# pierre-haessig/stodynprog

Measured on AMD Instinct MI355X. Metric: vi_sweeps_per_sec, higher is better.
Workload: dtype f64

## Files before the change

__graft_entry__.py:

```python
import os
import sys

ROOT = os.path.dirname(os.path.abspath(__file__))
if ROOT not in sys.path:
    sys.path.insert(0, ROOT)


def _prebuild_models(verbose=False):
    import numpy as np
    from stodynprog_amd import models, DPSolver, _native as nat
    sources = []
    specs = [
        ('inventory', {}, np.float64),
        ('nas_demo', {}, np.float64),
        ('storage_ar1', {}, np.float64),
        ('storage_ar1', dict(n_E=200, n_P=200, steps=(8. / 49, 0.1)), np.float64),
        ('searev', {}, np.float64),
        ('searev', dict(n_E=128, n_S=128, n_A=128, step=2.2 / 31), np.float64),
        ('synthetic3d', dict(N=20), np.float64),
        ('synthetic3d', dict(N=20), np.float32),
        ('synthetic3d', dict(N=48), np.float64),
        ('synthetic3d', dict(N=256), np.float64),
        ('synthetic3d', dict(N=256), np.float32),
        ('synthetic3d', dict(N=512), np.float32),
        ('synthetic3d', dict(N=256, stock_noise=0.07), np.float64),
        ('synthetic3d', dict(N=256, stock_noise=0.07, nested=True), np.float64),
        ('inventory_markov', {}, np.float64),
        ('inventory_fine', {}, np.float64),
        ('inventory_fine', dict(n_x=65536, n_u=4097, n_w=16), np.float64),
        ('two_reservoirs', dict(n_a=128, n_b=128, n_y=64, n_w=16, steps=(1. / 15, 1. / 15)), np.float64),
        ('synthetic3d_coupled', dict(N=256), np.float64),
        ('synthetic3d_coupled', dict(N=24), np.float64),
    ]
    for name, kw, dt in specs:
        sysd, ref = getattr(models, name)(**kw)
        for kernel in ('auto', 'staged', 'generic', 'long way'):
            solver = DPSolver(sysd, dtype=dt)
            solver.state_grid, solver.perturb_grid = ref.state_grid, ref.perturb_grid
            solver.perturb_proba, solver.control_steps = ref.perturb_proba, ref.control_steps
            if kernel == 'long way':
                solver.certified_filter = False
            else:
                solver.kernel = kernel
            sources.append(solver._kernel_plan()['source'])
    import importlib.util
    dont_write = sys.dont_write_bytecode
    sys.dont_write_bytecode = True
    try:
        spec = importlib.util.spec_from_file_location('column_forms', os.path.join(ROOT, 'tests', 'column_forms.py'))
        forms = importlib.util.module_from_spec(spec)
        spec.loader.exec_module(forms)
    finally:
        sys.dont_write_bytecode = dont_write
    saved = DPSolver.debug_defines
    try:
        for case, geometry in forms.PAIRS:
            DPSolver.debug_defines = dict(case.debug) or None
            for kw in (dict(), dict(certified_filter=False), dict(kernel='generic')):
                sources.append(case.solver(geometry, **kw)._kernel_plan()['source'])
    finally:
        DPSolver.debug_defines = saved
    sys.dont_write_bytecode = True
    sys.path.insert(0, os.path.join(ROOT, 'tests'))
    try:
        import policies
        import test_gpu_simulate_forms as simulate_forms
        for fam in policies.FAMILIES:
            for kernel in (None, 'generic'):
                sources.append(fam.solver(kernel)._kernel_plan()['source'])
        for make, _ in simulate_forms.UNITS.values():
            sources.append(make()._kernel_plan()['source'])
        sources.append(simulate_forms._deterministic(np.float32)._kernel_plan()['source'])
        sources.append(simulate_forms._deterministic(np.float64)._kernel_plan()['source'])
        for dt in (np.float64, np.float32):
            _, fh = models.finite_horizon()
            fh = policies.as_dtype(fh, dt)
            sources += [fh._kernel_plan(t0, fh._trace_now(t0))['source'] for t0 in (3, 11)]
        _, wec = models.searev(n_E=9, n_S=11, n_A=10)
        sources.append(policies.as_dtype(wec, np.float32)._kernel_plan()['source'])
        import test_horizon_plan
        sources += list(test_horizon_plan.units())
        import fp32_cases
        for case in fp32_cases.CASES + [fp32_cases.CONFIG5]:
            for run in case.runs:
                sources.append(fp32_cases.plan_of(case.solver(run))['source'])
        _, fh = models.finite_horizon()
        fh = policies.as_dtype(fh, np.float32)
        sources += [fh._kernel_plan(t, fh._trace_now(t))['source'] for T in (3, 11) for t in range(T)]
        import device_ops
        for dtkey in device_ops.DTYPES:
            for unit in device_ops.units(dtkey):
                sources.append(device_ops.unit_source(device_ops.unit_solver(unit, dtkey)))
        for seed in device_ops.WIDE_SEEDS:
            sources.append(device_ops.wide_model(seed)[0]._kernel_plan()['source'])
    finally:
        sys.path.remove(os.path.join(ROOT, 'tests'))
        sys.dont_write_bytecode = dont_write
    for kw in (dict(), dict(T=14 * 48, N_E=100)):
        _, pv = models.pv_storage(**kw)
        sources.append(pv._kernel_plan(0, pv._trace_now(0))['source'])
    from concurrent.futures import ThreadPoolExecutor
    unique = list(dict.fromkeys(sources))
    with ThreadPoolExecutor(max_workers=min(6, os.cpu_count() or 1)) as pool:
        return list(pool.map(lambda src: nat.compile_model(src, verbose=verbose), unique))


def build():
    from stodynprog_amd import _native as nat
    nat.build_library(verbose=True)
    from stodynprog_amd import codegen
    if os.path.isdir(nat.KCACHE):
        keep = set()
        for fn in os.listdir(nat.KCACHE):
            if fn.endswith('.hip'):
                try:
                    with open(os.path.join(nat.KCACHE, fn)) as f:
                        if codegen.source_key(f.read()) == fn[:-4]:
                            keep.add(fn[:-4])
                except OSError:
                    pass
        for fn in os.listdir(nat.KCACHE):
            stem = fn.split('.')[0]
            if '.tmp.' in fn or (fn.endswith(('.hsaco', '.hip')) and stem not in keep):
                os.unlink(os.path.join(nat.KCACHE, fn))
    import stodynprog_amd
    lib = nat.lib()
    assert lib is not None and nat.EXPORTS
    mods = _prebuild_models()
    print('built {} and {} model code objects'.format(nat.LIB_PATH, len(set(mods))))
    from oracle import c_oracle
    print('built', c_oracle.build())


def smoke():
    import numpy as np
    from stodynprog_amd import models, _native as nat
    nat.require_gpu()
    nat.check(nat.lib().sdp_set_device(0))
    print('device:', nat.device_info(0))
    _, solver = models.synthetic3d(N=20)
    V0 = models.synthetic3d_V0(solver.state_grid)
    J, pol = solver.value_iteration(V0, report_time=False)
    idx = solver.last_policy_index
    from oracle import c_oracle
    Jo, io, mo = c_oracle.vi_synth3d(solver.state_grid, V0, models.SYNTH_PAR, -1., 1., 64,
                                     solver.perturb_grid[0], solver.perturb_proba[0],
                                     n_nodes=V0.size)
    Jo = Jo.reshape(V0.shape)
    io = io.reshape(V0.shape)
    err = np.abs(J - Jo).max() / np.abs(Jo).max()
    print('smoke: max rel err J = {:.3e}; index mismatches = {}'.format(
        err, int((idx != io).sum())))
    assert err < 1e-12, err
    assert np.array_equal(idx, io)
    _, inv = models.inventory()
    J1, u1 = inv.value_iteration(np.zeros(10), report_time=False)
    assert np.allclose(J1, [9, 6, 3, 0, 0.5, 1, 1.5, 2, 2.5, 3], rtol=0, atol=1e-12), J1
    mcr = inv.monte_carlo(u1, np.zeros(1), 50, seed=1, n_burn=5, n_traj=100)
    _, w = inv.monte_carlo_draws(1, 100, 50)
    _, _, g = inv.simulate(u1, np.zeros((100, 1)), w)
    acc = np.zeros(100)
    for k in range(5, 50):
        acc = acc + g[k]
    assert np.array_equal(mcr.cost_sum, acc), (mcr.cost_sum, acc)
    print('smoke: Monte Carlo mean cost {:.4f} +- {:.4f}, same bits as the replay'.format(mcr.mean, mcr.stderr))
    print('smoke OK')


if __name__ == '__main__':
    build()
    if len(sys.argv) > 1 and sys.argv[1] == 'smoke':
        smoke()
```

stodynprog_amd/codegen.py:

```python
import hashlib
import re
import math
import os

import numpy as np

from .trace import TracedModel, DEP_X

CSRC = os.path.join(os.path.dirname(os.path.abspath(__file__)), 'csrc')


DEBUG_INT_MACROS = ('SDP_COL_MIN_WAVES', 'SDP_COL_BATCH', 'SDP_COL_UNROLL_U', 'SDP_COL_UNROLL_W',
                    'SDP_COL_A_GROUP', 'SDP_COL_FILTER_UNROLL', 'SDP_COL_FILTER_TOP2', 'SDP_COL_FILTER_RUNROLL',
                    'SDP_COL_A_WIDE_LOADS', 'SDP_COLU_WIDE_LOADS', 'SDP_COLU_A_GROUP',
                    'SDP_COL_TAIL_HOLD', 'SDP_SHORT_GROUP', 'SDP_BNB_CHUNK')
DEBUG_NAMES = frozenset(DEBUG_INT_MACROS + (
    'SDP_STAMP', 'SDP_NO_POW2', 'SDP_EXTRA_DEFINES', 'SDP_COL_FILTER_SCALE', 'SDP_LEAD_FILTER_SCALE',
    'SDP_LEAD_UNROLL', 'SDP_COL_A_LW', 'SDP_COL_FILTER', 'SDP_COL_SHIFT', 'SDP_COL_UTAB', 'SDP_LEAD_FILTER',
    'SDP_COL_THREADS', 'SDP_COL_WCHUNK', 'SDP_STG_CU', 'SDP_COL_WPAIR', 'SDP_COL_WRES', 'SDP_COL_LEAN2', 'SDP_COL_BNB',
    'SDP_LINE_FILTER', 'SDP_LINE_FILTER_SCALE', 'SDP_LINE_TOP2'))


def check_debug(debug):
    if not debug:
        return None
    unknown = sorted(set(debug) - DEBUG_NAMES)
    if unknown:
        raise ValueError('unknown debug define(s): {}'.format(', '.join(unknown)))
    return {k: str(v) for k, v in debug.items() if v is not None and str(v) != ''} or None


def _dbg(debug, name, default=None):
    if not debug:
        return default
    v = debug.get(name)
    return default if v is None or str(v) == '' else str(v)

_BIN_INFIX = {'add': '+', 'sub': '-', 'mul': '*', 'div': '/',
              'lt': '<', 'le': '<=', 'gt': '>', 'ge': '>=', 'eq': '==', 'ne': '!=',
              'and': '&&', 'or': '||', 'xor': '!='}
_FUNC1 = {'abs': 'fabs', 'sqrt': 'sqrt', 'floor': 'floor', 'ceil': 'ceil', 'trunc': 'trunc',
          'rint': 'rint', 'exp': 'exp', 'exp2': 'exp2', 'expm1': 'sdp_npexpm1', 'log': 'log',
          'log2': 'log2', 'log10': 'log10', 'log1p': 'sdp_nplog1p', 'sin': 'sin', 'cos': 'cos',
          'tan': 'tan', 'asin': 'asin', 'acos': 'acos', 'atan': 'atan', 'sinh': 'sinh',
          'cosh': 'cosh', 'tanh': 'tanh', 'cbrt': 'cbrt'}
_FUNC2 = {'pow': 'pow', 'atan2': 'atan2', 'hypot': 'hypot', 'fmod': 'fmod',
          'min': 'sdp_npmin', 'max': 'sdp_npmax', 'fmin': 'sdp_npfmin', 'fmax': 'sdp_npfmax',
          'pymod': 'sdp_nppymod', 'floordiv': 'sdp_npfloordiv'}


def real_literal(value):
    if math.isnan(value):
        return '(sdp_real)NAN'
    if math.isinf(value):
        return '(sdp_real)INFINITY' if value > 0 else '(-(sdp_real)INFINITY)'
    return '(sdp_real)({})'.format(float(value).hex())


def _emit_node(n, name, param_index=None):
    a = [name(x) for x in n.args]
    op = n.op
    if op == 'const':
        if param_index is not None and n.id in param_index:
            return 'sdp_model_prm[{}]'.format(param_index[n.id])
        return real_literal(n.value)
    if op == 'bconst':
        return 'true' if n.value else 'false'
    if op == 'var':
        v = n.value
        if v == 't':
            return 't'
        return '{}[{}]'.format(v[0], v[1:]) if v[0] in 'xu' else 'w'
    if op in _BIN_INFIX:
        return '({} {} {})'.format(a[0], _BIN_INFIX[op], a[1])
    if op in _FUNC1:
        return '{}({})'.format(_FUNC1[op], a[0])
    if op in _FUNC2:
        return '{}({}, {})'.format(_FUNC2[op], a[0], a[1])
    if op == 'neg':
        return '(-{})'.format(a[0])
    if op == 'square':
        return '({0} * {0})'.format(a[0])
    if op == 'recip':
        return '((sdp_real)1 / {})'.format(a[0])
    if op == 'sign':
        return 'sdp_npsign({})'.format(a[0])
    if op == 'not':
        return '(!{})'.format(a[0])
    if op == 'isnan':
        return '({0} != {0})'.format(a[0])
    if op == 'isinf':
        return '(fabs({}) == (sdp_real)INFINITY)'.format(a[0])
    if op == 'isfinite':
        return '(fabs({}) < (sdp_real)INFINITY)'.format(a[0])
    if op in ('select', 'bselect'):
        return '({} ? {} : {})'.format(a[0], a[1], a[2])
    if op == 'b2r':
        return '({} ? (sdp_real)1 : (sdp_real)0)'.format(a[0])
    if op == 'interp1':
        return 'sdp_interp1_{}({})'.format(n.value, a[0])
    raise NotImplementedError(op)


INTERP_SOURCE = '''SDP_DEV sdp_real sdp_np_interp(sdp_real x, const sdp_real *xp, const sdp_real *fp, int n,
                                sdp_real left, sdp_real right)
{
    if (n == 1) return x < xp[0] ? left : (x > xp[0] ? right : fp[0]);
    if (x != x) return x;
    if (x > xp[n - 1]) return right;
    if (x < xp[0]) return left;
    int imin = 0, imax = n;
    while (imin < imax) {
        const int imid = imin + ((imax - imin) >> 1);
        if (x >= xp[imid]) imin = imid + 1; else imax = imid;
    }
    const int j = imin - 1;
    if (j == n - 1) return fp[j];
    if (xp[j] == x) return fp[j];
    const sdp_real slope = (fp[j + 1] - fp[j]) / (xp[j + 1] - xp[j]);
    sdp_real r = slope * (x - xp[j]) + fp[j];
    if (r != r) {
        r = slope * (x - xp[j + 1]) + fp[j + 1];
        if (r != r && fp[j] == fp[j + 1]) r = fp[j];
    }
    return r;
}
'''


def interp_tables_source(model):
    used = sorted({n.value for n in model.live_nodes() if n.op == 'interp1'})
    if not used:
        return ''
    out = [INTERP_SOURCE]
    for tid in used:
        xp, fp, left, right = model.graph.tables[tid][:4]
        out.append('__constant__ sdp_real sdp_tabx_{}[{}] = {{{}}};'.format(
            tid, xp.size, ', '.join(real_literal(v) for v in xp)))
        out.append('__constant__ sdp_real sdp_tabf_{}[{}] = {{{}}};'.format(
            tid, fp.size, ', '.join(real_literal(v) for v in fp)))
        out.append('SDP_DEV sdp_real sdp_interp1_{0}(sdp_real x)\n{{\n    return sdp_np_interp('
                   'x, sdp_tabx_{0}, sdp_tabf_{0}, {1}, {2}, {3});\n}}'.format(
                       tid, xp.size, real_literal(left), real_literal(right)))
    return '\n'.join(out) + '\n'


def _emit_body(model, nodes, lines, names=None):
    names = dict(names or {})

    def name(n):
        return names[n.id]

    for n in nodes:
        expr = _emit_node(n, name, getattr(model, 'param_index', None))
        if n.op in ('const', 'bconst', 'var'):
            names[n.id] = expr
            continue
        var = 'v{}'.format(n.id)
        ctype = 'bool' if n.kind == 'b' else 'sdp_real'
        lines.append('    const {} {} = {};'.format(ctype, var, expr))
        names[n.id] = var
    return names


def model_function_source(model):
    assert isinstance(model, TracedModel)
    if model.n_perturb > 1:
        raise NotImplementedError('only 0 or 1 perturbation variable is supported '
                                  '(as reference stodynprog.py:679-683)')
    lines = ['SDP_DEV void sdp_model_cell(const sdp_real *x, const sdp_real *u, sdp_real w,',
             '                            sdp_real t, sdp_real *xn, sdp_real &g)',
             '{',
             '    (void)x; (void)u; (void)w; (void)t;']
# ... 67 lines not shown
    lines = ['SDP_DEV void sdp_model_leads(const sdp_real *x, const sdp_real *u, sdp_real t, sdp_real *xl)',
             '{', '    (void)x; (void)u; (void)t;']
    names = _emit_body(model, model.slice_nodes(leads), lines)
    for k, n in enumerate(leads):
        lines.append('    xl[{}] = {};'.format(k, names[n.id]))
    lines.append('}')
    out.append('\n'.join(lines))
    if m < d:
        lines = ['SDP_DEV void sdp_model_trails(const sdp_real *x, sdp_real w, sdp_real t, sdp_real *xt)',
                 '{', '    (void)x; (void)w; (void)t;']
        names = _emit_body(model, model.slice_nodes(trails), lines)
        for k, n in enumerate(trails):
            lines.append('    xt[{}] = {};'.format(k, names[n.id]))
        lines.append('}')
        out.append('\n'.join(lines))
    lines = ['SDP_DEV sdp_real sdp_model_cost(const sdp_real *x, const sdp_real *u, sdp_real w,',
             '                                sdp_real t)',
             '{', '    (void)x; (void)u; (void)w; (void)t;']
    names = _emit_body(model, model.slice_nodes([model.cost]), lines)
    lines += ['    return {};'.format(names[model.cost.id]), '}']
    out.append('\n'.join(lines))
    return '\n\n'.join(out)


def lead_filter_applies(model, dtype, min_axes=2, debug=None):
    if _dbg(debug, 'SDP_LEAD_FILTER', '1') == '0':
        return 0
    if model.n_perturb != 1 or np.dtype(dtype).itemsize != 8:
        return 0
    m = model.controlled_axes()
    return int(m) if m is not None and m >= min_axes else 0


def lead_order(model, dtype, debug=None):
    if _dbg(debug, 'SDP_LEAD_FILTER', '1') == '0' or model.n_perturb != 1 or np.dtype(dtype).itemsize != 8:
        return None
    co = model.controlled_order()
    if co is None or co[1] == tuple(range(model.n_state)) or co[0] >= model.n_state:
        return None
    return co


UTAB_MAX_VALUES = 4
UTAB_MAX_BYTES = 4096


def control_table_plan(model, dtype, per_node, max_controls, debug=None):
    if _dbg(debug, 'SDP_COL_UTAB', '1') == '0' or per_node or model.cost_depends_on_w:
        return None
    lead = None
    if model.lead_depends_on_w:
        split = model.lead_split()
        if split is None:
            return None
        lead = split[0]
    fr = model.control_uniform_frontier(lead)
    if fr is None or len(fr) > UTAB_MAX_VALUES:
        return None
    if len(fr) * int(max_controls) * np.dtype(dtype).itemsize > UTAB_MAX_BYTES:
        return None
    return fr


def control_table_source(model, frontier):
    slot = {n.id: k for k, n in enumerate(frontier)}
    out = []
    lines = ['SDP_DEV void sdp_model_utab(const sdp_real *x, const sdp_real *u, sdp_real t, sdp_real *tab)',
             '{', '    (void)x; (void)u; (void)t;']
    names = _emit_body(model, model.slice_nodes(frontier), lines)
    for n in frontier:
        lines.append('    tab[{}] = {};'.format(slot[n.id], names[n.id]))
    lines.append('}')
    out.append('\n'.join(lines))
    pre = {n.id: 'tab[{}]'.format(slot[n.id]) for n in frontier}
    split = model.lead_split() if model.lead_depends_on_w else None
    for fname, node in (('sdp_model_lead_tab', split[0] if split else model.x_next[0]),
                        ('sdp_model_cost_tab', model.cost)):
        lines = ['SDP_DEV sdp_real {}(const sdp_real *x, const sdp_real *tab, sdp_real t)'.format(fname),
                 '{', '    (void)x; (void)tab; (void)t;']
        names = _emit_body(model, model.slice_nodes_until([node], set(slot)), lines, pre)
        lines += ['    return {};'.format(names[node.id]), '}']
        out.append('\n'.join(lines))
    chain = model.lead_split_chain() if split else None
    if chain is not None:
        leaves = [n for n, _ in chain[0]]
        lines = ['SDP_DEV sdp_real sdp_model_lead_aabs_tab(const sdp_real *x, const sdp_real *tab, sdp_real t)',
                 '{', '    (void)x; (void)tab; (void)t;']
        names = _emit_body(model, model.slice_nodes_until(leaves, set(slot)), lines, pre)
        lines += ['    return {};'.format(' + '.join('fabs({})'.format(names[n.id]) for n in leaves)), '}']
        out.append('\n'.join(lines))
    return '\n\n'.join(out)


def short_pass_source(model, frontier, macro='SDP_COL_LEAN2'):
    sp = model.additive_control_split(frontier)
    if sp is None:
        return None
    (x_node, a_slot, a_form), (k_node, h_slot, h_form) = sp['lead'], sp['cost']
    out = ['#define {} 1          // x0\' = X(x) +- a(u), cost = K(x) +- h(u): the short first pass'.format(macro),
           '#define SDP_LEAN2_A_SLOT {}'.format(int(a_slot)),
           '#define SDP_LEAN2_H_SLOT {}'.format(-1 if h_slot is None else int(h_slot)),
           '#define SDP_LEAN2_LEAD(X, A) {}'.format({'add': '((X) + (A))', 'sub': '((X) - (A))', 'rsub': '((A) - (X))'}[a_form]),
           '#define SDP_LEAN2_FORM {}            // 0: X + a, 1: X - a, 2: a - X'.format({'add': 0, 'sub': 1, 'rsub': 2}[a_form]),
           '#define SDP_LEAN2_A_FIXED {}         // a depends on the control alone: the same lattice of positions in every column'.format(
               0 if (frontier[int(a_slot)].deps & DEP_X) else 1),
           '#define SDP_LEAN2_HNEG {}           // the part of the cost that depends on the control enters negated (K - h)'.format(
               1 if (h_slot is not None and h_form == 'sub') else 0)]
    for fname, node in (('sdp_model_lead_x', x_node), ('sdp_model_cost_x', k_node)):
        lines = ['SDP_DEV sdp_real {}(const sdp_real *x, sdp_real t)'.format(fname), '{', '    (void)x; (void)t;']
        if node is None:
            lines += ['    return (sdp_real)0;', '}']
        else:
            names = _emit_body(model, model.slice_nodes([node]), lines)
            lines += ['    return {};'.format(names[node.id]), '}']
        out.append('\n'.join(lines))
    return '\n'.join(out)


def lanes_for(max_controls):
    lanes = 1
    while lanes < max_controls and lanes < 64:
        lanes *= 2
    return lanes


def _prologue_lines(model, real, lanes, debug, peer_stores=False):
    lines = ['// generated by stodynprog_amd.codegen -- do not edit',
             '#define SDP_REAL {}'.format(real),
             '#define SDP_D {}'.format(model.n_state),
             '#define SDP_NU {}'.format(model.n_control),
             '#define SDP_HAS_W {}'.format(1 if model.n_perturb else 0),
             '#define SDP_LANES {}'.format(int(lanes)),
             '#define SDP_PEER_STORES {}     // the backup kernels also store J into other ranks (direct exchange)'.format(
                 1 if peer_stores else 0)]
    if _dbg(debug, 'SDP_STAMP') in ('1', '2', '3'):
        lines.append('#define SDP_STAMP {}     // diagnostic build: in-kernel clock stamps (tools/clock_probe.py, '
                     'tools/phase_probe.py)'.format(int(_dbg(debug, 'SDP_STAMP'))))
    if _dbg(debug, 'SDP_NO_POW2') == '1':
        lines.append('#define SDP_NO_POW2 1  // A/B: true division also for power-of-two spans')
    for kv in (_dbg(debug, 'SDP_EXTRA_DEFINES') or '').split(','):
        if '=' in kv:
            lines.append('#define {} {}   // SDP_EXTRA_DEFINES (diagnostic builds)'.format(*kv.split('=', 1)))
    lines += ['#include "sdp_device.h"', 'typedef SDP_REAL sdp_real;', '']
    if getattr(model, 'param_index', None):
        lines += ['#define SDP_NPARAMS {}'.format(len(model.param_index)),
                  'extern "C" { __constant__ sdp_real sdp_model_prm[SDP_NPARAMS]; }     // a definition', '']
    tables = interp_tables_source(model)
    if tables:
        lines.append(tables)
    lines += [model_function_source(model), '']
    return lines


def _column_lines(model, dtype, column, col_cfg, window, per_control, filtered, utab, debug, wres=0):
    rs = np.dtype(dtype).itemsize
    wpair = use_wpair(model, dtype, debug) and window is None
    shifted = bool(filtered and column_shift_applies(model, dtype, debug=debug))
    lines = ['#define SDP_COST_HAS_W {}'.format(1 if model.cost_depends_on_w else 0),
             '#define SDP_LEAD_HAS_W {}'.format(1 if model.lead_depends_on_w else 0),
             '#define SDP_TRAIL_HAS_U {}'.format(1 if model.trail_depends_on_u else 0),
             '#define SDP_COL_N0 {}'.format(int(column[0])),
             '#define SDP_COL_W {}'.format(max(int(column[1]), 1)),
             '#define SDP_COL_THREADS {}'.format(col_cfg[0]),
             '#define SDP_COL_WPAIR {}'.format(1 if wpair else 0)]
    if wres:
        lines.append('#define SDP_COL_WRES {}         // resident-chunk form: perturbation points the table holds at a time'.format(int(wres)))
        if rs == 8 and shifted and not _dbg(debug, 'SDP_COL_UNROLL_W'):
            lines.append('#define SDP_COL_UNROLL_W 1')
    if filtered and int(col_cfg[0]) <= 256 and not _dbg(debug, 'SDP_COL_MIN_WAVES'):
        if wres:
            lines.append('#define SDP_COL_MIN_WAVES {}    // as many waves per SIMD as the LDS image admits workgroups per CU, at most 4'.format(
                max(1, min(4, (COLUMN_LDS_MAX // int(col_cfg[1])) * int(col_cfg[0]) // 256))))
        else:
            lines.append('#define SDP_COL_MIN_WAVES 1    // small workgroups of the filtered kernel: no register cap')
    if filtered:
        lines.append('#define SDP_COL_FILTER 1')
        if shifted:
            lines += ['#define SDP_COL_SHIFT 1        // x0\' = a(x, u) +- b_1(x_1.., w) +- ..: first pass on the shifted lattice',
                      '#define SDP_COL_SHIFT_TERMS {}'.format(len(model.lead_split()[1])),
                      '#define SDP_COL_SHIFT_CHAIN {}        // additions of a chain of sums that was regrouped (0: the final-sum form)'.format(
                          model.lead_split_chain()[1] if model.lead_split_chain() is not None else 0),
                      '#define SDP_COL_SHIFT_ROWS {}'.format(int(col_cfg[2]))]
        if _dbg(debug, 'SDP_COL_FILTER_SCALE'):
            lines.append('#define SDP_COL_FILTER_SCALE {}'.format(float(_dbg(debug, 'SDP_COL_FILTER_SCALE'))))
    if per_control is None:
        wide = column_wide_loads(column[0], dtype, window, debug)
        order = column_build_order(int(col_cfg[0]), column[1], int(window[2]) if window is not None else column[0],
                                   (16 // rs) if wide else 1)
        if order[0] == 2:
            lw = int(_dbg(debug, 'SDP_COL_A_LW') or order[1])
            lines += ['#define SDP_COL_A_ORDER 2',
                      '#define SDP_COL_A_LW {}'.format(lw)]
            if rs == 4 and int(column[0]) >= 512 and not wres and window is None and not _dbg(debug, 'SDP_COL_A_GROUP'):
                lines.append('#define SDP_COL_A_GROUP 8      // table entries per thread whose vertex loads are issued together')
            if wide and not _dbg(debug, 'SDP_COL_A_WIDE_LOADS'):
                lines.append('#define SDP_COL_A_WIDE_LOADS 1')

                if wres and rs == 8 and not wpair and window is None and _dbg(debug, 'SDP_COL_TAIL_HOLD') is None:
                    tail, groups = int(column[1]) - int(wres), int(col_cfg[0]) // lw
                    if (tail > 0 and tail % groups == 0 and int(column[0]) % (2 * lw) == 0
                            and (tail // groups) * (int(column[0]) // (2 * lw)) * 4 <= 32):
                        lines.append('#define SDP_COL_TAIL_HOLD 1    // the tail of the table is built once and held in registers')
    if window is not None:
        lines.append('#define SDP_COL_ROWS {}'.format(int(window[2])))
    if per_control is not None:
        lines.append('#define SDP_COL_WCHUNK {}'.format(int(per_control[2])))
        if int(column[0]) % (16 // rs) == 0 and not _dbg(debug, 'SDP_COLU_WIDE_LOADS'):
            lines.append('#define SDP_COLU_WIDE_LOADS 1')
    for k in DEBUG_INT_MACROS:
        if _dbg(debug, k):
            lines.append('#define {} {}'.format(k, int(_dbg(debug, k))))
    lines += [separable_functions_source(model), '']
    if utab is not None and filtered:
        lines += ['#define SDP_COL_UTAB {}'.format(len(utab[0])),
                  '#define SDP_COL_UTAB_N {}'.format(int(utab[1])),
                  control_table_source(model, utab[0]), '']
        short = None
        if not model.cost_depends_on_w and window is None and per_control is None \
                and _dbg(debug, 'SDP_COL_LEAN2') != '0' and (not shifted or rs == 8):
            if rs == 8 and wres:
                short = short_pass_source(model, utab[0], 'SDP_COL_LEAN2')
                if short and _dbg(debug, 'SDP_COL_BNB') != '0':
                    short += ('\n#define SDP_COL_BNB 1          // the short first pass as a certified branch and bound over '
                              'blocks of controls (sdp_lean2_bnb)')

            elif rs == 4 and not wres and _dbg(debug, 'SDP_COL_FILTER_TOP2') in (None, '1'):
                short = short_pass_source(model, utab[0], 'SDP_COL_WIDE2')
                if short and _dbg(debug, 'SDP_COL_BNB') != '0':
                    short += ('\n#define SDP_COL_BNB 1          // the short wide first pass as a certified branch and bound over '
                              'blocks of controls (sdp_short_bnb)')
                    if int(column[0]) >= 512 and not _dbg(debug, 'SDP_BNB_CHUNK'):
                        short += '\n#define SDP_BNB_CHUNK 4        // blocks whose bounds are evaluated together (see SDP_COL_A_GROUP above)'
        if short:
            lines += [short, '']
    lines += ['#include "sdp_column_kernel.h"    // also brings in sdp_sweep_kernel.h', '']
    return lines


def line_filter_applies(model, dtype, W, debug=None):
    if _dbg(debug, 'SDP_LINE_FILTER', '1') == '0':
        return False
    return bool(model.n_state == 1 and model.n_perturb == 1 and 1 <= int(W) <= 1024 and np.dtype(dtype).itemsize == 8
                and not model.time_dep and model.lead_depends_on_w and not model.cost_depends_on_w
                and model.lead_split() is not None)


def line_functions_source(model):
    a_node, terms = model.lead_split()
    out = []
    lines = ['SDP_DEV sdp_real sdp_model_lead_a(const sdp_real *x, const sdp_real *u, sdp_real t)',
             '{', '    (void)x; (void)u; (void)t;']
    names = _emit_body(model, model.slice_nodes([a_node]), lines)
    lines += ['    return {};'.format(names[a_node.id]), '}']
    out.append('\n'.join(lines))
    chain = model.lead_split_chain()
    if chain is not None:
        leaves = [n for n, _ in chain[0]]
        lines = ['SDP_DEV sdp_real sdp_model_lead_aabs(const sdp_real *x, const sdp_real *u, sdp_real t)',
                 '{', '    (void)x; (void)u; (void)t;']
        names = _emit_body(model, model.slice_nodes(leaves), lines)
        lines += ['    return {};'.format(' + '.join('fabs({})'.format(names[n.id]) for n in leaves)), '}']
        out.append('\n'.join(lines))
    lines = ['SDP_DEV void sdp_model_lead_b(const sdp_real *x, sdp_real w, sdp_real t, sdp_real &b, sdp_real &babs)',
             '{', '    (void)x; (void)w; (void)t;']
    names = _emit_body(model, model.slice_nodes([b for b, _ in terms]), lines)
    b0, s0 = terms[0]
    lines.append('    b = {}{};'.format('-' if s0 < 0 else '', names[b0.id]))
    lines.append('    babs = fabs({});'.format(names[b0.id]))
    for bn, sg in terms[1:]:
        lines.append('    b = b {} {};'.format('+' if sg > 0 else '-', names[bn.id]))
        lines.append('    babs = babs + fabs({});'.format(names[bn.id]))
    lines.append('}')
    out.append('\n'.join(lines))
    lines = ['SDP_DEV sdp_real sdp_model_cost(const sdp_real *x, const sdp_real *u, sdp_real w,',
             '                                sdp_real t)',
             '{', '    (void)x; (void)u; (void)w; (void)t;']
    names = _emit_body(model, model.slice_nodes([model.cost]), lines)
    lines += ['    return {};'.format(names[model.cost.id]), '}']
    out.append('\n'.join(lines))
    return '\n\n'.join(out)


def translation_unit(model, dtype, lanes, column=None, staged=None, window=None,
                     per_control=None, filtered=False, utab=None, lead_axes=0, col_cfg=None, debug=None, wres=0,
                     lead_perm=None, line=0, peer_stores=False):
    debug = check_debug(debug)
    real = {'float64': 'double', 'float32': 'float'}[np.dtype(dtype).name]
    head = _prologue_lines(model, real, lanes, debug, peer_stores)
    if column is not None:
        assert model.column_shareable
        if per_control is not None:
            col_cfg = per_control
        elif window is not None:
            col_cfg = window
        elif col_cfg is None:
            col_cfg = column_config(column[0], column[1], model.n_state, dtype,
                                    use_wpair(model, dtype, debug), filtered,
                                    max_controls=column[2] if len(column) > 2 else None,
                                    n_columns=column[3] if len(column) > 3 else None,
                                    shift=filtered and column_shift_applies(model, dtype, debug=debug),
                                    utab_values=(utab_reals(len(utab[0]), utab[1]) if utab is not None and filtered else 0),
                                    debug=debug)
        if col_cfg is None:
            raise ValueError('the column kernel does not fit this grid (its table exceeds the LDS of a CU)')
        head += _column_lines(model, dtype, column, col_cfg, window, per_control, filtered, utab, debug,
                              wres if (window is None and per_control is None) else 0)
    elif staged is not None:
        tile = tuple(staged['tile']) + (1,) * (4 - len(staged['tile']))
        head += ['#define SDP_STG_THREADS {}'.format(int(staged['threads']))] + [
            '#define SDP_STG_T{} {}'.format(k, int(tile[k])) for k in range(4)] + [
            '#define SDP_STG_CU {}'.format(int(staged['cu'])),
            '#define SDP_STG_CW {}'.format(int(staged['cw'])),
            '#define SDP_STG_CAP {}'.format(int(staged['cap'])),
            '#include "sdp_staged_kernel.h"    // also brings in sdp_sweep_kernel.h',
            '']
    elif line:
        chain = model.lead_split_chain()
        head += ['#define SDP_LINE 1',
                 '#define SDP_LINE_W {}'.format(int(line)),
                 '#define SDP_LINE_CHAIN {}        // additions of a chain of sums that was regrouped (0: the final-sum form)'.format(
                     chain[1] if chain is not None else 0)]
        if _dbg(debug, 'SDP_LINE_FILTER_SCALE'):
            head.append('#define SDP_LINE_FILTER_SCALE {}'.format(float(_dbg(debug, 'SDP_LINE_FILTER_SCALE'))))
        if _dbg(debug, 'SDP_LINE_TOP2') is not None:
            head.append('#define SDP_LINE_TOP2 {}'.format(int(_dbg(debug, 'SDP_LINE_TOP2'))))
        head += [line_functions_source(model), '',
                 '#include "sdp_sweep_kernel.h"    // brings in sdp_line_kernel.h', '']
    elif lead_axes:
        head += ['#define SDP_LEAD_AXES {}'.format(int(lead_axes)),
                 '#define SDP_LEAD_COST_HAS_W {}'.format(1 if model.cost_depends_on_w else 0)]
        if lead_perm is not None and tuple(lead_perm) != tuple(range(model.n_state)):
            full = tuple(lead_perm) + tuple(range(model.n_state, 4))
            head.append('#define SDP_LEAD_PERM {{{}}}     // state variable of logical axis j: the stocks are not listed first'.format(
                ', '.join(str(int(k)) for k in full)))
        if _dbg(debug, 'SDP_LEAD_FILTER_SCALE'):
            head.append('#define SDP_LEAD_FILTER_SCALE {}'.format(float(_dbg(debug, 'SDP_LEAD_FILTER_SCALE'))))
        if _dbg(debug, 'SDP_LEAD_UNROLL'):
            head.append('#define SDP_LEAD_UNROLL {}'.format(int(_dbg(debug, 'SDP_LEAD_UNROLL'))))
        head += [lead_functions_source(model, int(lead_axes), lead_perm), '',
                 '#include "sdp_sweep_kernel.h"    // brings in sdp_lead_kernel.h', '']
    else:
        head += ['#include "sdp_sweep_kernel.h"', '']
    return '\n'.join(head)


STAGED_TILES = {1: (512,), 2: (16, 32), 3: (8, 8, 8), 4: (4, 4, 4, 8)}
STAGED_LDS_BYTES = 76 * 1024


def staged_row_stride(length, tile_last, d, rs):
    if d == 1 or tile_last >= 32 or rs != 8:
        return length | 1
    return (length + tile_last - 1) // (2 * tile_last) * (2 * tile_last) + tile_last


def staged_config(model, state_grid, perturb_grid, box, dtype, t_value=0.0, n_samples=24, debug=None):
    from .trace import evaluate
    d = model.n_state
    rs = np.dtype(dtype).itemsize
    shape = tuple(len(g) for g in state_grid)
    tile = STAGED_TILES[d]
    cap = STAGED_LDS_BYTES // rs
    W = len(perturb_grid[0]) if perturb_grid and model.n_perturb else 0
    wg = np.asarray(perturb_grid[0], dtype=float) if W else np.zeros(1)
    Wn = max(W, 1)
    nu = model.n_control
    lo, hi, n = box['lo'], box['hi'], box['n']
    S = int(np.prod(shape))
    rng = np.random.default_rng(2024)
    smin = np.array([g[0] for g in state_grid], dtype=float)
    span = np.array([g[-1] - g[0] for g in state_grid], dtype=float)
    nm1 = np.array([len(g) - 1 for g in state_grid], dtype=float)
    tiles_per = [-(-shape[k] // tile[k]) for k in range(d)]

    def control_values(flat_nodes, ci):
        col = flat_nodes if box['per_node'] else np.zeros_like(flat_nodes)
        nn = n[:, col].astype(np.int64)
        tot = np.prod(nn, axis=0)
        flat = np.minimum(ci, tot - 1)
        out = []
        for c in range(nu - 1, -1, -1):
            k = flat % nn[c]
            flat = flat // nn[c]
            l, h = lo[c, col], hi[c, col]
            step = np.where(nn[c] > 1, (h - l) / np.maximum(nn[c] - 1, 1), 0.0)
            out.append(np.where(k == nn[c] - 1, h, k * step + l))
        return out[::-1], tot

    def volume(cu, cw):
        vols = []
        for _ in range(n_samples):
            torg = [int(rng.integers(0, tiles_per[k])) * tile[k] for k in range(d)]
            idx = np.array(np.meshgrid(*[[torg[k], min(torg[k] + tile[k], shape[k]) - 1]
                                         for k in range(d)], indexing='ij')).reshape(d, -1)
            flat = np.ravel_multi_index(tuple(idx), shape)
            x = [np.asarray(state_grid[k], dtype=float)[idx[k]] for k in range(d)]
            _, tot = control_values(flat, 0)
            c0 = int(rng.integers(0, max(int(tot.max()) - cu, 0) + 1))
            w0 = int(rng.integers(0, max(Wn - cw, 0) + 1))
            qlo = np.full(d, np.inf)
            qhi = np.full(d, -np.inf)
            for ci in (c0, c0 + cu - 1):
                u, _ = control_values(flat, ci)
                for wi in (w0, min(w0 + cw, Wn) - 1):
                    with np.errstate(all='ignore'):
                        xn, _ = evaluate(model, x, u, [wg[wi]] if model.n_perturb else [], t_value)
                    for k in range(d):
                        p = (np.asarray(xn[k], dtype=float) - smin[k]) / span[k] * nm1[k]
                        q = np.clip(np.floor(np.nan_to_num(p, nan=0.0, posinf=1e9, neginf=-1e9)),
                                    0, shape[k] - 2)
                        qlo[k] = min(qlo[k], q.min())
                        qhi[k] = max(qhi[k], q.max())
            ext = [min(qhi[k] + 1, shape[k] - 2) + 2 - max(qlo[k] - 1, 0) for k in range(d)]
            ext[-1] = staged_row_stride(int(ext[-1]), tile[-1], d, rs)
            vols.append(float(np.prod(ext)))
        return float(np.percentile(vols, 80))

    cws = sorted({max(1, Wn >> s) for s in range(0, 8)}, reverse=True)
    best = None
    cus = (4, 2, 1)
    if _dbg(debug, 'SDP_STG_CU'):
        cus = (int(_dbg(debug, 'SDP_STG_CU')),)
    for cu in cus:
        for cw in cws:
            if best is not None and cu * cw <= best[0] * best[1]:
                continue
            if volume(cu, cw) <= cap:
                best = (cu, cw)
                break
    if best is None:
        best = (1, 1)
    return dict(threads=int(np.prod(tile)), tile=tile, cu=best[0], cw=best[1], cap=int(cap))


COLUMN_LDS_MAX = 160 * 1024


def use_wpair(model, dtype, debug=None):
    if _dbg(debug, 'SDP_COL_WPAIR'):
        return bool(int(_dbg(debug, 'SDP_COL_WPAIR')))
    return (np.dtype(dtype).itemsize == 4 and model.n_perturb > 0
            and not model.lead_depends_on_w and not model.trail_depends_on_u)


def column_shift_applies(model, dtype, table=None, debug=None):
    if _dbg(debug, 'SDP_COL_SHIFT', '1') == '0':
        return False
    ok = bool(model.n_perturb > 0 and model.lead_depends_on_w and model.lead_split() is not None
              and dtype is not None and np.dtype(dtype).itemsize == 8)
    if ok and table is not None:
        ok = column_config(table[0], table[1], table[2], dtype, False, True, shift=True,
                           utab_values=UTAB_MAX_BYTES // np.dtype(dtype).itemsize + 256,
                           debug=debug) is not None
    return ok


def column_filter_applies(model, window=None, per_control=None, dtype=None, table=None, debug=None):
    if _dbg(debug, 'SDP_COL_FILTER', '1') == '0':
        return False
    return bool(model.n_perturb > 0 and (not model.lead_depends_on_w or column_shift_applies(model, dtype, table, debug))
                and not model.trail_depends_on_u and window is None
                and per_control is None)


def column_config(n0, w, n_state, dtype, wpair=False, filtered=False, max_controls=None, n_columns=None,
                  shift=False, utab_values=0, debug=None, wres=0):
    rs = np.dtype(dtype).itemsize
    w = max(int(w), 1)
    tw = w + (w & 1) if wpair else w
    sizes = (512, 1024)
    if filtered and n0 <= 512:
        first = max(64, (int(n0) + 63) // 64 * 64)
        if max_controls:
            lanes = 1
            while lanes * 128 < int(max_controls) and lanes < 64:
                lanes *= 2
            cap = 1024 if (n_columns is not None and int(n_columns) < 256) else 512
            first = max(first, min(first * lanes, cap))
        sizes = (first,) + tuple(t for t in sizes if t > first)
    if _dbg(debug, 'SDP_COL_THREADS'):
        sizes = (int(_dbg(debug, 'SDP_COL_THREADS')),)
    if shift:
        for per_cu in ((3, 2, 1) if wres else (2, 1)):
            for threads in sizes:
                if per_cu >= 2 and threads > 512:
                    continue
                base = _column_lds(int(wres) or tw, w, n0, n_state, rs, threads, shift=True, shift_rows=0, utab_values=utab_values)
                rows = min(2 * int(n0) + 16, (COLUMN_LDS_MAX // per_cu - base - 1024) // (2 * rs))
                if rows >= int(n0) + max(8, int(n0) // 8):
                    return (threads, _column_lds(int(wres) or tw, w, n0, n_state, rs, threads, shift=True, shift_rows=rows,
                                                 utab_values=utab_values), int(rows))
        return None
    for threads in sizes:
        lds = _column_lds(int(wres) or tw, w, n0, n_state, rs, threads, reduced=filtered, utab_values=utab_values,
                          partial_minima=not filtered)
        if lds * (2 if threads <= 512 else 1) <= COLUMN_LDS_MAX:
            return threads, lds
    return None


def column_resident_points(model, n0, w, n_state, dtype, filtered, shift, wpair, threads, utab_values=0, debug=None):
    rs = np.dtype(dtype).itemsize
    w = int(w)
    ok = (filtered and rs == 8 and not wpair and not model.cost_depends_on_w and w >= 4
          and int(threads) >= int(n0))
    forced = _dbg(debug, 'SDP_COL_WRES')
    if forced is not None:
        k = int(forced)
        return k if (ok and 0 < k < w and 2 * k >= w) else 0
    if not ok:
        return 0
    half = (w + 1) // 2
    if shift:
        both = [column_config(n0, w, n_state, dtype, wpair, True, shift=True, utab_values=utab_values, debug=debug, wres=k)
                for k in (0, half)]
        if None in both:
            return 0
        whole, part = both[0][1], both[1][1]
    else:
        whole = _column_lds(w, w, n0, n_state, rs, threads, reduced=True, utab_values=utab_values)
        part = _column_lds(half, w, n0, n_state, rs, threads, reduced=True, utab_values=utab_values)
    if COLUMN_LDS_MAX // whole < 3 <= COLUMN_LDS_MAX // part:
        return half if RESIDENT_CHUNKS_DEFAULT else 0
    return 0


RESIDENT_CHUNKS_DEFAULT = True


def column_wide_loads(n0, dtype, window, debug=None):
    if _dbg(debug, 'SDP_COL_A_WIDE_LOADS', '1') == '0':
        return False
    rpl = 16 // np.dtype(dtype).itemsize
    if rpl != 2 and _dbg(debug, 'SDP_COL_A_WIDE_LOADS') != '1':
        return False
    return int(n0) % rpl == 0 and window is None


def column_build_order(threads, w, rows, rows_per_lane=1):
    w = max(int(w), 1)
    best = (0, 0, 0.0)
    for lw in ((32, 64, 16, 8) if rows_per_lane > 1 else (64, 32, 16, 8)):
        if lw * rows_per_lane > rows or threads % lw:
            continue
        groups = threads // lw
        util = w / float(-(-w // groups) * groups)
        if util > best[2] + 1e-9:
            best = (2, lw, util)
    return (best[0], best[1]) if best[2] >= 0.85 else (0, 0)


def bnb_words(n_controls):
    n = max(int(n_controls), 1)
    block = 8
    while (n + block - 1) // block > 64:
        block *= 2
    return 4 * ((n + block - 1) // block + 1)


def utab_reals(n_values, n_controls):
    return int(n_values) * int(n_controls) + bnb_words(n_controls) if n_values else 0


def _column_lds(tw, w, rows, n_state, rs, threads, reduced=False, shift=False, shift_rows=0, utab_values=0,
                partial_minima=False):
    dt = n_state - 1
    part = threads if partial_minima else 1
    members = [(rs, tw * rows, 16),
               (rs, w * dt, rs), (rs, w * dt, rs),
               (rs, 2, rs),
               (rs, part, rs), (4, part, 4),
               (4, w * dt, 4),
               (4, 4, 4), (4, 1, 4), (8, 2, 8),
               (rs, 2 * (int(utab_values) + 4 if utab_values else 2), 16)]
    if reduced or shift:
        per_row = 4 if rs == 4 else (2 if shift else 1)
        members.append((rs, per_row * int(shift_rows if shift else rows), 16))
    if shift:
        members += [(4, 2 * w, 4), (rs, 2 * w, rs), (rs, 2 * w, rs), (4, 8, 4)]
    off = 0
    for size, count, align in members:
        off = (off + align - 1) // align * align + size * int(count)
    return (off + 15) // 16 * 16


def column_percontrol_config(n0, w, n_state, dtype, debug=None):
    rs = np.dtype(dtype).itemsize
    w = max(int(w), 1)
    threads = min(512, max(64, (int(n0) + 63) // 64 * 64))
    wchunk = max(1, min(w, (32 * 1024) // (int(n0) * rs)))
    if _dbg(debug, 'SDP_COL_WCHUNK'):
        wchunk = max(1, min(w, int(_dbg(debug, 'SDP_COL_WCHUNK'))))
    lds = _column_lds(wchunk, w, n0, n_state, rs, threads)
    if lds > COLUMN_LDS_MAX:
        return None
    return threads, lds, wchunk


def column_window_config(n0, w, n_state, dtype, reach_rows):
    rs = np.dtype(dtype).itemsize
    w = max(int(w), 1)
    for threads, wgs in ((512, 2),):
        budget = COLUMN_LDS_MAX // wgs
        fixed = _column_lds(w, w, 0, n_state, rs, threads, partial_minima=True)
        rows = (budget - fixed) // (w * rs)
        rows = min(rows // 32 * 32, n0)
        seg = (rows - int(reach_rows) - 4) // 64 * 64
        if rows >= 128 and seg >= 64:
            return (threads, _column_lds(w, w, rows, n_state, rs, threads, partial_minima=True), int(rows),
                    int(min(seg, n0)))
    return None


def column_lds_bytes(n0, w, n_state, dtype):
    cfg = column_config(n0, w, n_state, dtype)
    return cfg[1] if cfg else COLUMN_LDS_MAX + 1


HIPCC_FLAGS = ['--genco', '--offload-arch=gfx950', '-O3', '-ffp-contract=off',
               '-fno-fast-math', '-std=c++17', '-I', CSRC]


_HEADERS = ('sdp_kernel_args.h', 'sdp_device.h', 'sdp_sweep_kernel.h', 'sdp_mc_kernel.h', 'sdp_column_kernel.h', 'sdp_colfilter_kernel.h', 'sdp_colres_kernel.h',
            'sdp_colfull_kernel.h', 'sdp_colu_kernel.h',
            'sdp_lead_kernel.h', 'sdp_staged_kernel.h')
_digest_cache = {}


def _headers_digest():
    stamp = tuple(os.stat(os.path.join(CSRC, fn)).st_mtime_ns for fn in _HEADERS)
    h = _digest_cache.get(stamp)
    if h is None:
        h = hashlib.sha256()
        for fn in _HEADERS:
            with open(os.path.join(CSRC, fn), 'rb') as f:
                h.update(f.read())
        _digest_cache.clear()
        _digest_cache[stamp] = h
    return h.copy()


_compiler_id = None
HIPCC_PATH = '/opt/rocm/bin/hipcc'


def compiler_identity():
    global _compiler_id
    if _compiler_id is None:
        import subprocess
        try:
            out = subprocess.run([HIPCC_PATH, '--version'], stdout=subprocess.PIPE, stderr=subprocess.DEVNULL,
                                 timeout=60).stdout.decode(errors='replace')
            keep = [ln.strip() for ln in out.splitlines() if ln.startswith(('HIP version', 'AMD clang version', 'clang version'))]
            _compiler_id = '\n'.join(keep) or 'hipcc without a version'
        except (OSError, subprocess.SubprocessError):
            _compiler_id = 'no hipcc'
    return _compiler_id


BUILD_RULES = 'spill fence 1'


def source_key(source):
    h = _headers_digest()
    if '#define SDP_LINE ' in source:
        with open(os.path.join(CSRC, 'sdp_line_kernel.h'), 'rb') as f:
            h.update(f.read())
    h.update(source.encode())
    h.update(' '.join(HIPCC_FLAGS[:-1]).encode())
    h.update(compiler_identity().encode())
    h.update(BUILD_RULES.encode())
    return h.hexdigest()[:24]


_ASM_FUNC = re.compile(r'^([A-Za-z_]\w*):\s*; @')
_ASM_BLOCK = re.compile(r'^(\.LBB\d+_\d+):|^; %bb\.(\d+):')
_ASM_SPILL = re.compile(r'^\s+(?:scratch_(?:store|load)\w*|buffer_(?:store|load)\w*|v_accvgpr_(?:write|read)\w*)\b.*;.*\b(?:Spill|Reload)\b')
_ASM_END_CF = re.compile(r'^\s+s_or_b64\s+exec,\s*exec,')
_ASM_EXEC_WRITE = re.compile(r'^\s+s_\w+\s+exec(?:_lo|_hi)?\b|^\s+s_\w*saveexec\w*\b|^\s+v_cmpx')


def spill_hazards(asm):
    out, func, block, pending, at_top = [], None, None, [], False
    for n, line in enumerate(asm.splitlines(), 1):
        m = _ASM_FUNC.match(line)
        if m:
            func, block, pending, at_top = m.group(1), 'entry', [], False
            continue
        m = _ASM_BLOCK.match(line)
        if m:
            block, pending, at_top = m.group(1) or '%bb.' + m.group(2), [], True
            continue
        if not at_top:
            continue
        if _ASM_SPILL.match(line):
            pending.append(line.strip())
        elif _ASM_END_CF.match(line):
            if pending:
                out.append((func, block, n, pending))
            at_top = False
        elif _ASM_EXEC_WRITE.match(line):
            at_top = False
    return out


def _msgpack_ints_after(blob, key):
    out, i = [], blob.find(key)
    while i >= 0:
        j = i + len(key)
        b = blob[j] if j < len(blob) else 0
        out.append(b if b <= 0x7f else int.from_bytes(blob[j + 1:j + 1 + {0xcc: 1, 0xcd: 2, 0xce: 4}.get(b, 0)], 'big') if b in (0xcc, 0xcd, 0xce) else -1)
        i = blob.find(key, j)
    return out


def code_object_may_spill(blob):
    scratch = _msgpack_ints_after(blob, b'.private_segment_fixed_size')
    agprs = _msgpack_ints_after(blob, b'.agpr_count')
    if not scratch or len(agprs) != len(scratch):
        return True
    return any(v != 0 for v in scratch) or any(v != 0 for v in agprs)
```

stodynprog_amd/csrc/sdp_colfilter_kernel.h:

```cpp
#pragma once

SDP_DEV double sdp_vmin(double a, double b) { double r; asm("v_min_f64 %0, %1, %2" : "=v"(r) : "v"(a), "v"(b)); return r; }
SDP_DEV double sdp_vmax(double a, double b) { double r; asm("v_max_f64 %0, %1, %2" : "=v"(r) : "v"(a), "v"(b)); return r; }
SDP_DEV float sdp_vmin(float a, float b) { float r; asm("v_min_f32 %0, %1, %2" : "=v"(r) : "v"(a), "v"(b)); return r; }
SDP_DEV float sdp_vmax(float a, float b) { float r; asm("v_max_f32 %0, %1, %2" : "=v"(r) : "v"(a), "v"(b)); return r; }
SDP_DEV double sdp_vmax_abs(double a, double b) { double r; asm("v_max_f64 %0, %1, |%2|" : "=v"(r) : "v"(a), "v"(b)); return r; }
SDP_DEV float sdp_vmax_abs(float a, float b) { float r; asm("v_max_f32 %0, %1, |%2|" : "=v"(r) : "v"(a), "v"(b)); return r; }

struct SdpColFilter {
    sdp_real psum;
    sdp_real pcap;
    sdp_real cu;
    sdp_real floor;
    sdp_real ratio;
    const sdp_cst_real *p, *wg;
    double psum64;
    sdp_real gc;
    sdp_real glimit;
    bool ok;
    sdp_real k_rows, x_cap;
};
constexpr bool SDP_COL_LEAN_ON = sizeof(sdp_real) == 8;
constexpr bool SDP_COL_WIDE_ON = sizeof(sdp_real) == 4;
static_assert(!SDP_COL_SHIFT || SDP_COL_LEAN_ON, "the shifted lattice is a form of the lean first pass (8-byte reals)");
// ... 205 lines not shown
#pragma unroll
                for (int i = 0; i < CH; ++i) {
                    const sdp_real t0 = tv[i][0], t1 = tv[i][1], t2 = tv[i][2];
                    acc = fma(tp[i], fma(tf[i], t1 - t0, t0), acc);
                    bnd = fma(tc[i], fabs((t2 - t1) - (t1 - t0)), bnd);
                    big = sdp_vmax_abs(big, t1);
                }
            } else {
#pragma unroll
                for (int i = 0; i < CH; ++i) {
                    const int wq = w_lo + wave + (i0 + i) * waves;
                    const int trow = (wq < w_lo + w_cnt ? wq : w_lo + wave) - w_lo;
                    const int j = k + (tq[i] - trow * N0);
                    const int q = max(min(j, N0 - 2), 0);
                    const sdp_real lam = (sdp_real)(j - q) + tf[i];
                    const sdp_real *row = m.T + trow * N0 + q;
                    const sdp_real t0 = row[0], t1 = row[1], t2 = row[q + 2 < N0 ? 2 : 1];
                    acc = fma(tp[i], fma(lam, t1 - t0, t0), acc);
                    const sdp_real d2 = (t2 - t1) - (t1 - t0);
                    const bool kink = (unsigned)j <= (unsigned)(N0 - 3);
                    bnd = fma(tc[i], kink ? fabs(d2) : (sdp_real)0, bnd);
                    big = sdp_vmax_abs(sdp_vmax_abs(big, t0), t1);
                }
            }
            if (ki < c.rows) {
                __hip_atomic_fetch_add(&m.ad[2 * ki], acc, __ATOMIC_RELAXED, __HIP_MEMORY_SCOPE_WORKGROUP);
                __hip_atomic_fetch_add(&m.ad[2 * ki + 1], bnd, __ATOMIC_RELAXED, __HIP_MEMORY_SCOPE_WORKGROUP);
            }
            dmax = sdp_vmax(dmax, acc == acc ? f.pcap * big + f.floor : (sdp_real)INFINITY);
        }
    }
    dmax = sdp_wave_max(dmax);
    if (lane == 0)
        atomicMax(&m.dcol[parity], (unsigned long long)__double_as_longlong((double)dmax));
}
#endif

SDP_DEV int sdp_col_axis_mode(const SdpLeadAxis &l)
{
    if (!l.pow2) return 0;
    return (l.smin == (sdp_real)0 && l.span == (sdp_real)1) ? 2 : 1;
}

#if SDP_COST_HAS_W
template <bool WIDE, typename ACC>
SDP_DEV void sdp_col_cost_expect(const SdpColFilter &f, const sdp_real *x, const sdp_real *u, sdp_real t,
                                 ACC &G, sdp_real &Gabs)
{
    G = (ACC)0;
    Gabs = (sdp_real)0;
    sdp_real graw = (sdp_real)0;
#pragma unroll 4
    for (int w = 0; w < SDP_COL_W; ++w) {
        const sdp_real pw = f.p[w];
        const sdp_real gw = sdp_model_cost(x, u, f.wg[w], t);
        G = fma((ACC)pw, (ACC)gw, G);
        Gabs = fma((WIDE ? sdp_col_wide_nw(w) : (sdp_real)1) * fabs(pw), fabs(gw), Gabs);
        graw = sdp_vmax_abs(graw, gw);
    }
    Gabs = sdp_vmax(Gabs, graw);
}
#endif

template <int AXIS>
SDP_DEV void sdp_col_lean_core(const sdp_real *A, const SdpColFilter &f, const SdpLeadAxis &l,
                               sdp_real xn0, sdp_real g, sdp_real &F, sdp_real &lmax, sdp_real &bmax)
{
    const sdp_real sn = AXIS == 2 ? xn0 : (AXIS == 1 ? (xn0 - l.smin) * l.rspan : (xn0 - l.smin) / l.span);
    const sdp_real p = sn * l.nm1;
#if SDP_COL_SHIFT
    const sdp_real pk = p - l.koff;
    int q0 = (int)pk;
    asm("v_med3_i32 %0, %0, 0, %1" : "+v"(q0) : "s"(l.ordm2));
    const sdp_real lam0 = pk - (sdp_real)q0;
    lmax = sdp_vmax_abs(lmax, lam0);
    const sdp_real a0 = A[2 * q0], a1 = A[2 * q0 + 2];
    bmax = sdp_vmax(bmax, A[2 * q0 + 1]);
#else
    (void)bmax;
    int q0 = (int)p;
    asm("v_med3_i32 %0, %0, 0, %1" : "+v"(q0) : "s"(l.ordm2));
    const sdp_real lam0 = p - (sdp_real)q0;
    lmax = sdp_vmax_abs(lmax, lam0);
    const sdp_real a0 = A[q0], a1 = A[q0 + 1];
#endif
#if SDP_COST_HAS_W
    F = g + fma(lam0, a1 - a0, a0);
#else
    F = fma(g, f.psum, fma(lam0, a1 - a0, a0));
#endif
}
template <int AXIS>
SDP_DEV void sdp_col_lean_eval(const sdp_real *A, const SdpColFilter &f, const SdpLeadAxis &l,
                               const sdp_real *x, const sdp_real *u, sdp_real t, sdp_real &F, sdp_real &lmax,
                               sdp_real &gmax, sdp_real &bmax)
{
#if SDP_COL_SHIFT
    const sdp_real xn0 = sdp_model_lead_a(x, u, t);
#if SDP_COL_SHIFT_CHAIN
    lmax = sdp_vmax_abs(lmax, sdp_model_lead_aabs(x, u, t) * (fabs(l.nm1 * l.rspan) * (sdp_real)1.002));
#endif
#else
    const sdp_real xn0 = sdp_model_lead(x, u, (sdp_real)0, t);
#endif
#if SDP_COST_HAS_W
    sdp_real g, gabs;
    sdp_col_cost_expect<false>(f, x, u, t, g, gabs);
    gmax = sdp_vmax(gmax, gabs);
#else
    (void)gmax;
    const sdp_real g = sdp_model_cost(x, u, (sdp_real)0, t);
#endif
    sdp_col_lean_core<AXIS>(A, f, l, xn0, g, F, lmax, bmax);
}
#if SDP_COL_UTAB
template <int AXIS>
SDP_DEV void sdp_col_lean_eval_tab(const sdp_real *A, const sdp_real *utab, const SdpColFilter &f,
                                   const SdpLeadAxis &l, const sdp_real *x, int ci, sdp_real t,
                                   sdp_real &F, sdp_real &lmax, sdp_real &bmax)
{
    sdp_real tab[SDP_COL_UTAB];
#pragma unroll
    for (int k = 0; k < SDP_COL_UTAB; ++k) tab[k] = utab[ci * SDP_COL_UTAB + k];
    const sdp_real xn0 = sdp_model_lead_tab(x, tab, t);
    const sdp_real g = sdp_model_cost_tab(x, tab, t);
#if SDP_COL_SHIFT && SDP_COL_SHIFT_CHAIN
    lmax = sdp_vmax_abs(lmax, sdp_model_lead_aabs_tab(x, tab, t) * (fabs(l.nm1 * l.rspan) * (sdp_real)1.002));
#endif
    sdp_col_lean_core<AXIS>(A, f, l, xn0, g, F, lmax, bmax);
}
SDP_DEV void sdp_col_phase_u(const SdpSweepArgs &a, sdp_real *utab, const sdp_real *x, sdp_real t, int first = 0,
                             int count = 0, const SdpBox *box_c = nullptr, sdp_real psum = (sdp_real)0,
                             sdp_real k_rows = (sdp_real)0, sdp_real x_cap = (sdp_real)0, double psum_d = 0.0,
                             bool a_known = false)
{
    (void)psum; (void)k_rows; (void)x_cap; (void)psum_d; (void)a_known;
    if (count == 0) count = (int)blockDim.x - first;
    const int tid = sdp_col_tid();
    if (tid < first || tid >= first + count) return;
    SdpBox box;
    if (box_c) box = *box_c;
    else sdp_load_box(a, 0, box);
    const int n_tab = min(box.total, SDP_COL_UTAB_N);
#if SDP_COL_SHORT
    sdp_real a_lo = INFINITY, a_hi = -INFINITY, h_abs = (sdp_real)0, fin = (sdp_real)0;
#endif
#if SDP_COL_BNB
    constexpr sdp_real BNB_DELTA = sizeof(sdp_real) == 8 ? (sdp_real)0x1p-20 : (sdp_real)0x1p-8;
    constexpr bool BNB_WIDE = sizeof(sdp_real) == 4;
    sdp_real *rec = utab + SDP_COL_UTAB * SDP_COL_UTAB_N + 4;
    const int lane_u = tid - first;
    bool bnb_fine = count == 64 && SDP_BNB_BLOCK <= 64;
    sdp_real bnb_prev_hi = -INFINITY, bnb_prev_lo = (sdp_real)NAN, bnb_between = (sdp_real)0, bnb_amax = (sdp_real)0;
    for (int c0 = 0; c0 < n_tab; c0 += 64) {
        int ci = c0 + lane_u;
        asm volatile("" : "+v"(ci));
        sdp_real u[SDP_NU], tab[SDP_COL_UTAB];
        sdp_controls_at(box, min(ci, n_tab - 1), u);
        sdp_model_utab(x, u, t, tab);
        if (ci < n_tab) {
#pragma unroll
            for (int k = 0; k < SDP_COL_UTAB; ++k) utab[ci * SDP_COL_UTAB + k] = tab[k];
            if (!a_known) {
                a_lo = sdp_vmin(a_lo, tab[SDP_LEAN2_A_SLOT]);
                a_hi = sdp_vmax(a_hi, tab[SDP_LEAN2_A_SLOT]);
                fin = fin + fabs(tab[SDP_LEAN2_A_SLOT]);
            }
            if (SDP_LEAN2_H_SLOT >= 0) {
                h_abs = sdp_vmax_abs(h_abs, tab[SDP_LEAN2_H_SLOT < 0 ? 0 : SDP_LEAN2_H_SLOT]);
                fin = fin + fabs(tab[SDP_LEAN2_H_SLOT < 0 ? 0 : SDP_LEAN2_H_SLOT]);
            }
        }
        const sdp_real av = tab[SDP_LEAN2_A_SLOT];
        const sdp_real hv = SDP_LEAN2_H_SLOT < 0 ? (sdp_real)0 : tab[SDP_LEAN2_H_SLOT < 0 ? 0 : SDP_LEAN2_H_SLOT];
        const double hpv = (double)(SDP_LEAN2_HNEG ? -hv : hv) * psum_d;
        const bool have = ci < n_tab;
        double hp = have ? hpv : (double)INFINITY;
        constexpr int SEG = SDP_BNB_BLOCK < 64 ? SDP_BNB_BLOCK : 64;
        const bool head = have && (lane_u % SEG) == 0;
        if (a_known) {
            if (SEG == 8) {
                hp = sdp_vmin(hp, sdp_dpp_f64<0xB1>(hp)); hp = sdp_vmin(hp, sdp_dpp_f64<0x4E>(hp)); hp = sdp_vmin(hp, sdp_dpp_f64<0x141>(hp));
            } else {
#pragma unroll
                for (int d = 1; d < SEG; d <<= 1) hp = sdp_vmin(hp, __shfl_xor(hp, d, 64));
            }
            if (head) {
                const int b = ci / SDP_BNB_BLOCK;
                if (BNB_WIDE) *(double *)(rec + 4 * b + 2) = hp;
                else rec[2 * b + 1] = (sdp_real)hp;
            }
            continue;
        }
        const sdp_real pa = (SDP_LEAN2_FORM == 1 ? -av : av) * k_rows;
        bnb_fine = bnb_fine && (!have || (pa == pa && hpv == hpv && fabs(pa) < (sdp_real)INFINITY));
        bnb_amax = sdp_vmax_abs(bnb_amax, have ? av : (sdp_real)0);
        sdp_real lo = have ? pa : (sdp_real)INFINITY, hi = have ? pa : -(sdp_real)INFINITY;
        if (SEG == 8) {
            lo = sdp_vmin(lo, sdp_dpp_f64<0xB1>(lo)); hi = sdp_vmax(hi, sdp_dpp_f64<0xB1>(hi)); hp = sdp_vmin(hp, sdp_dpp_f64<0xB1>(hp));
            lo = sdp_vmin(lo, sdp_dpp_f64<0x4E>(lo)); hi = sdp_vmax(hi, sdp_dpp_f64<0x4E>(hi)); hp = sdp_vmin(hp, sdp_dpp_f64<0x4E>(hp));
            lo = sdp_vmin(lo, sdp_dpp_f64<0x141>(lo)); hi = sdp_vmax(hi, sdp_dpp_f64<0x141>(hi)); hp = sdp_vmin(hp, sdp_dpp_f64<0x141>(hp));
        } else {
#pragma unroll
            for (int d = 1; d < SEG; d <<= 1) {
                lo = sdp_vmin(lo, __shfl_xor(lo, d, 64));
                hi = sdp_vmax(hi, __shfl_xor(hi, d, 64));
                hp = sdp_vmin(hp, __shfl_xor(hp, d, 64));
            }
        }
        const sdp_real next_lo = __shfl_down(lo, SEG, 64);
        const bool has_next = lane_u + SEG < 64 && ci + SEG < n_tab;
        if (head) {
            const int b = ci / SDP_BNB_BLOCK;
            if (BNB_WIDE) { rec[4 * b] = lo - BNB_DELTA; *(double *)(rec + 4 * b + 2) = hp; }
            else { rec[2 * b] = lo - BNB_DELTA; rec[2 * b + 1] = (sdp_real)hp; }
            if (has_next) {
                bnb_fine = bnb_fine && hi + 2 * BNB_DELTA <= next_lo;
                bnb_between = sdp_vmax(bnb_between, next_lo - lo);
            }
            if (lane_u == 0 && c0 > 0) {
                bnb_fine = bnb_fine && bnb_prev_hi + 2 * BNB_DELTA <= lo;
                bnb_between = sdp_vmax(bnb_between, lo - bnb_prev_lo);
            }
            if (ci + SDP_BNB_BLOCK >= n_tab) {
                rec[(BNB_WIDE ? 4 : 2) * (b + 1)] = hi + BNB_DELTA;
                bnb_between = sdp_vmax(bnb_between, hi - lo);
            }
        }
        if (c0 + 64 < n_tab) {
            bnb_prev_hi = __shfl(hi, 64 - SEG, 64);
            bnb_prev_lo = __shfl(lo, 64 - SEG, 64);
        }
    }
    if (!a_known)
    {
        const bool sorted = __all(bnb_fine);
        bnb_between = sdp_wave_max(bnb_between);
        bnb_amax = sdp_wave_max(bnb_amax);
        if (lane_u == 0) {
            const int n_blocks = (n_tab + SDP_BNB_BLOCK - 1) / SDP_BNB_BLOCK;
            const int extra = (bnb_between == bnb_between && bnb_between < (sdp_real)SDP_COL_N0)
                                  ? max((int)(bnb_between + 4 * BNB_DELTA) - 1, 0) : SDP_COL_N0;
            if (BNB_WIDE) rec[4 * n_blocks + 1] = (sdp_real)__int_as_float(extra);
            else rec[2 * n_blocks + 1] = (sdp_real)__hiloint2double(0, extra);
            sdp_real *st = utab + SDP_COL_UTAB * SDP_COL_UTAB_N;
            const sdp_real cap = x_cap - bnb_amax;
            st[3] = (sorted && cap == cap && extra < SDP_COL_N0) ? cap : (sdp_real)-1;
        }
    }
#else
    for (int ci_ = tid - first; ci_ < n_tab; ci_ += count) {
        int ci = ci_;
        asm volatile("" : "+v"(ci));
        sdp_real u[SDP_NU], tab[SDP_COL_UTAB];
        sdp_controls_at(box, ci, u);
        sdp_model_utab(x, u, t, tab);
#pragma unroll
        for (int k = 0; k < SDP_COL_UTAB; ++k) utab[ci * SDP_COL_UTAB + k] = tab[k];
#if SDP_COL_SHORT
        a_lo = sdp_vmin(a_lo, tab[SDP_LEAN2_A_SLOT]);
        a_hi = sdp_vmax(a_hi, tab[SDP_LEAN2_A_SLOT]);
        fin = fin + fabs(tab[SDP_LEAN2_A_SLOT]);
        if (SDP_LEAN2_H_SLOT >= 0) {
            h_abs = sdp_vmax_abs(h_abs, tab[SDP_LEAN2_H_SLOT < 0 ? 0 : SDP_LEAN2_H_SLOT]);
            fin = fin + fabs(tab[SDP_LEAN2_H_SLOT < 0 ? 0 : SDP_LEAN2_H_SLOT]);
        }
#endif
    }
#endif
#if SDP_COL_SHORT
    h_abs = sdp_wave_max(h_abs);
    fin = sdp_wave_sum(fin);
    if (a_known) {
        if (tid == first) {
            sdp_real *st = utab + SDP_COL_UTAB * SDP_COL_UTAB_N;
            const sdp_real before = st[2];
            st[2] = (count == 64 && fin < SDP_COL_FILTER_LIMIT && before == before) ? h_abs : (sdp_real)NAN;
        }
        return;
    }
    a_lo = sdp_wave_min(a_lo);
    a_hi = sdp_wave_max(a_hi);
    if (tid == first) {
        sdp_real *st = utab + SDP_COL_UTAB * SDP_COL_UTAB_N;
        st[0] = a_lo;
        st[1] = a_hi;
        st[2] = (count == 64 && fin < SDP_COL_FILTER_LIMIT) ? h_abs : (sdp_real)NAN;
    }
#endif
}
#endif

template <int AXIS>
SDP_DEV void sdp_col_wide_core(const sdp_real *ad, const SdpColFilter &f, const SdpLeadAxis &l,
                               sdp_real xn0, double g64, sdp_real gabs, double &F, sdp_real &bound, sdp_real &pmax)
{
    const sdp_real sn = AXIS == 2 ? xn0 : (AXIS == 1 ? (xn0 - l.smin) * l.rspan : (xn0 - l.smin) / l.span);
    const sdp_real p = sn * l.nm1;
    pmax = sdp_vmax_abs(pmax, p);
    int q0 = (int)p;
    asm("v_med3_i32 %0, %0, 0, %1" : "+v"(q0) : "s"(l.ordm2));
    const sdp_real lam0 = p - (sdp_real)q0;
    const sdp_real oml0 = (sdp_real)1 - lam0;
    const sdp_real *row = ad + 4 * q0;
    const double a0 = *(const double *)row, a1 = *(const double *)(row + 4);
    const sdp_real b0 = row[2], b1 = row[6];
#if SDP_COST_HAS_W
    F = g64 + fma((double)oml0, a0, (double)lam0 * a1);
    bound = gabs + fma(fabs(oml0), b0, fabs(lam0) * b1);
#else
    F = fma(g64, f.psum64, fma((double)oml0, a0, (double)lam0 * a1));
    bound = fma(gabs, f.gc, fma(fabs(oml0), b0, fabs(lam0) * b1));
#endif
}
template <int AXIS>
SDP_DEV void sdp_col_wide_eval(const sdp_real *ad, const SdpColFilter &f, const SdpLeadAxis &l,
                               const sdp_real *x, const sdp_real *u, sdp_real t, double &F, sdp_real &bound, sdp_real &pmax)
{
    const sdp_real xn0 = sdp_model_lead(x, u, (sdp_real)0, t);
#if SDP_COST_HAS_W
    double g64;
    sdp_real gabs;
    sdp_col_cost_expect<true>(f, x, u, t, g64, gabs);
    sdp_col_wide_core<AXIS>(ad, f, l, xn0, g64, gabs, F, bound, pmax);
#else
    const sdp_real g = sdp_model_cost(x, u, (sdp_real)0, t);
    sdp_col_wide_core<AXIS>(ad, f, l, xn0, (double)g, fabs(g), F, bound, pmax);
#endif
}
#if SDP_COL_UTAB
template <int AXIS>
SDP_DEV void sdp_col_wide_eval_tab(const sdp_real *ad, const sdp_real *utab, const SdpColFilter &f,
                                   const SdpLeadAxis &l, const sdp_real *x, int ci, sdp_real t,
                                   double &F, sdp_real &bound, sdp_real &pmax)
{
    sdp_real tab[SDP_COL_UTAB];
#pragma unroll
    for (int k = 0; k < SDP_COL_UTAB; ++k) tab[k] = utab[ci * SDP_COL_UTAB + k];
    const sdp_real g = sdp_model_cost_tab(x, tab, t);
    sdp_col_wide_core<AXIS>(ad, f, l, sdp_model_lead_tab(x, tab, t), (double)g, fabs(g), F, bound, pmax);
}
#endif

#ifndef SDP_COL_FILTER_TOP2
#define SDP_COL_FILTER_TOP2 -1
#endif
constexpr bool SDP_COL_TOP2 = SDP_COL_FILTER_TOP2 < 0 ? (sizeof(sdp_real) == 4 || SDP_COL_SHIFT) : SDP_COL_FILTER_TOP2 != 0;
struct SdpColBounds {
    sdp_fkey f1, f2, f3, s_sum;
    sdp_real s_max, p_max;
    sdp_real b_max;
    int i1, i2;
};
SDP_DEV void sdp_col_bounds_insert(SdpColBounds &b, sdp_fkey F, int ci)
{
    if (SDP_COL_TOP2) {
        b.f3 = sdp_vmin(b.f3, sdp_vmax(b.f2, F));
        const bool c1 = F < b.f1, c2 = F < b.f2;
        b.i2 = c1 ? b.i1 : (c2 ? ci : b.i2);
    }
    b.f2 = sdp_vmin(b.f2, sdp_vmax(b.f1, F));
    b.i1 = F < b.f1 ? ci : b.i1;
    b.f1 = sdp_vmin(b.f1, F);
}

template <bool PLAIN, int AXIS>
SDP_DEV void sdp_col_filter_pass1(const sdp_real *ad_tab, const sdp_real *utab, const SdpColFilter &f,
                                  const SdpLeadAxis &l, const SdpBox &box, sdp_real *x, sdp_real t,
                                  int c_lo, int c_hi, SdpColBounds &b)
{
#if SDP_COL_UTAB
    {
        (void)box;
        auto one = [&](int ci) {
            sdp_fkey F;
            if (SDP_COL_WIDE_ON) {
                double Fw;
                sdp_real bound;
                sdp_col_wide_eval_tab<AXIS>(ad_tab, utab, f, l, x, ci, t, Fw, bound, b.p_max);
                b.s_max = sdp_vmax(b.s_max, bound);
                F = (sdp_fkey)Fw;
            } else {
                sdp_real Fl;
                sdp_col_lean_eval_tab<AXIS>(ad_tab, utab, f, l, x, ci, t, Fl, b.p_max, b.b_max);
                F = (sdp_fkey)Fl;
            }
            b.s_sum = b.s_sum + fabs(F);
            sdp_col_bounds_insert(b, F, ci);
        };
        constexpr int K = SDP_COL_FILTER_UNROLL;
        int ci = c_lo;
        for (; ci + K <= c_hi; ci += K) {
#pragma unroll
            for (int j = 0; j < K; ++j) one(ci + j);
        }
        for (; ci < c_hi; ++ci) one(ci);
        return;
    }
#endif
    (void)utab;
    auto eval = [&](int ci, const sdp_real *u) {
        if (SDP_COL_WIDE_ON) {
            double Fw;
            sdp_real bound;
            sdp_col_wide_eval<AXIS>(ad_tab, f, l, x, u, t, Fw, bound, b.p_max);
            b.s_max = sdp_vmax(b.s_max, bound);
            b.s_sum = b.s_sum + (sdp_fkey)fabs(Fw);
            sdp_col_bounds_insert(b, (sdp_fkey)Fw, ci);
            return;
        }
        sdp_real F;
        sdp_col_lean_eval<AXIS>(ad_tab, f, l, x, u, t, F, b.p_max, b.s_max, b.b_max);
        b.s_sum = b.s_sum + fabs(F);
        sdp_col_bounds_insert(b, F, ci);
    };
    auto one = [&](int ci) {
        sdp_real u[SDP_NU];
        if (PLAIN) u[0] = (sdp_real)ci * box.step[0] + box.lo[0];
        else sdp_controls_at(box, ci, u);
        eval(ci, u);
    };
    const int last = PLAIN ? box.n[0] - 1 : INT_MAX;
    const int c_main = min(c_hi, last);
    constexpr int K = SDP_COL_FILTER_UNROLL;
    int ci = c_lo;
    for (; ci + K <= c_main; ci += K) {
#pragma unroll
        for (int j = 0; j < K; ++j) one(ci + j);
    }
    for (; ci < c_main; ++ci) one(ci);
    if (PLAIN && c_hi > last && c_lo <= last) eval(last, box.hi);
}

#if SDP_COL_SHORT
template <int AXIS>
SDP_DEV void sdp_lean2_cell(const SdpLeadAxis &l, sdp_real xn0, int &q0, sdp_real &lam0)
{
    const sdp_real sn = AXIS == 2 ? xn0 : (AXIS == 1 ? (xn0 - l.smin) * l.rspan : (xn0 - l.smin) / l.span);
    const sdp_real p = sn * l.nm1;
    q0 = (int)p;
    asm("v_med3_i32 %0, %0, 0, %1" : "+v"(q0) : "s"(l.ordm2));
    lam0 = p - (sdp_real)q0;
}
#if SDP_COL_SHIFT
template <int AXIS>
SDP_DEV void sdp_lean2s_cell(const SdpLeadAxis &l, sdp_real xn0, int &q0, sdp_real &lam0)
{
    const sdp_real sn = AXIS == 2 ? xn0 : (AXIS == 1 ? (xn0 - l.smin) * l.rspan : (xn0 - l.smin) / l.span);
    const sdp_real pk = sn * l.nm1 - l.koff;
    q0 = (int)pk;
    asm("v_med3_i32 %0, %0, 0, %1" : "+v"(q0) : "s"(l.ordm2));
    lam0 = pk - (sdp_real)q0;
}
#endif
#endif
#if SDP_COL_WIDE2
template <int AXIS>
SDP_DEV double sdp_wide2_value(const sdp_real *ad, const sdp_real *utab, const SdpColFilter &f, const SdpLeadAxis &l,
                               sdp_real X, int ci)
{
    int q0;
    sdp_real lam0;
    sdp_lean2_cell<AXIS>(l, SDP_LEAN2_LEAD(X, utab[ci * SDP_COL_UTAB + SDP_LEAN2_A_SLOT]), q0, lam0);
    const double a0 = SDP_AD_A_CONST(ad, q0), a1 = SDP_AD_A_CONST(ad, q0 + 1);
    const double h = fma((double)lam0, a1 - a0, a0);
    if (SDP_LEAN2_H_SLOT < 0) return h;
    const sdp_real hv = utab[ci * SDP_COL_UTAB + (SDP_LEAN2_H_SLOT < 0 ? 0 : SDP_LEAN2_H_SLOT)];
    return fma((double)(SDP_LEAN2_HNEG ? -hv : hv), f.psum64, h);
}
struct SdpShortBounds { double f1, f2, f3; };
SDP_DEV void sdp_short_insert(SdpShortBounds &b, double F)
{
    b.f3 = sdp_vmin(b.f3, sdp_vmax(b.f2, F));
    b.f2 = sdp_vmin(b.f2, sdp_vmax(b.f1, F));
    b.f1 = sdp_vmin(b.f1, F);
}
#ifndef SDP_WIDE2_GROUP
#define SDP_WIDE2_GROUP 4
#endif
template <int AXIS>
SDP_DEV void sdp_wide2_pass1(const sdp_real *ad, const sdp_real *utab, const SdpColFilter &f, const SdpLeadAxis &l,
                             sdp_real X, int c_lo, int c_hi, int mask, SdpShortBounds &b)
{
    auto insert = [&](double F, int ci) {
        sdp_short_insert(b, __hiloint2double(__double2hiint(F), (__double2loint(F) & ~mask) | ci));
    };
    constexpr int K = SDP_WIDE2_GROUP;
    constexpr int HS = SDP_LEAN2_H_SLOT < 0 ? 0 : SDP_LEAN2_H_SLOT;
    int ci = c_lo;
    for (; ci + K <= c_hi; ci += K) {
        int q0[K];
        sdp_real av[K], hv[K], lam0[K];
        double a0[K], a1[K];
#pragma unroll
        for (int j = 0; j < K; ++j) {
            av[j] = utab[(ci + j) * SDP_COL_UTAB + SDP_LEAN2_A_SLOT];
            hv[j] = SDP_LEAN2_H_SLOT < 0 ? (sdp_real)0 : utab[(ci + j) * SDP_COL_UTAB + HS];
        }
#pragma unroll
        for (int j = 0; j < K; ++j) sdp_lean2_cell<AXIS>(l, SDP_LEAN2_LEAD(X, av[j]), q0[j], lam0[j]);
#pragma unroll
        for (int j = 0; j < K; ++j) {
            a0[j] = SDP_AD_A_CONST(ad, q0[j]);
            a1[j] = SDP_AD_A_CONST(ad, q0[j] + 1);
        }
#pragma unroll
        for (int j = 0; j < K; ++j) {
            const double h = fma((double)lam0[j], a1[j] - a0[j], a0[j]);
            insert(SDP_LEAN2_H_SLOT < 0 ? h : fma((double)(SDP_LEAN2_HNEG ? -hv[j] : hv[j]), f.psum64, h), ci + j);
        }
    }
    for (; ci < c_hi; ++ci) insert(sdp_wide2_value<AXIS>(ad, utab, f, l, X, ci), ci);
}
#endif

#if SDP_COL_BNB
#ifndef SDP_SHORT_GROUP
#define SDP_SHORT_GROUP 4
#endif
#ifndef SDP_BNB_CHUNK
#define SDP_BNB_CHUNK (sizeof(SDP_REAL) == 8 ? 4 : 2)
#endif
template <int AXIS, bool WIDE, typename INSERT>
SDP_DEV void sdp_short_bnb(const sdp_real *A, const sdp_real *utab, const SdpColFilter &f, const SdpLeadAxis &l,
                           sdp_real X, sdp_real k_rows, int c_lo, int n, int mask, double slack, int guess, INSERT &insert,
                           sdp_real &sdp_diag_cnt, sdp_real *b_seen = nullptr)
{
    (void)sdp_diag_cnt; (void)c_lo; (void)b_seen;
    constexpr bool SHIFT = SDP_COL_SHIFT != 0;
    static_assert(!(SHIFT && WIDE), "branch and bound on the shifted lattice: 8-byte reals");
    constexpr double BSCALE = (double)(SDP_COL_FILTER_SCALE);
    constexpr int BS = SDP_BNB_BLOCK, NB = SDP_BNB_BLOCKS;
    constexpr int HS = SDP_LEAN2_H_SLOT < 0 ? 0 : SDP_LEAN2_H_SLOT;
    static_assert(NB <= 64, "branch and bound: at most 64 blocks");
    const sdp_real *rec = utab + SDP_COL_UTAB * SDP_COL_UTAB_N + 4;
    const double psum = WIDE ? f.psum64 : (double)f.psum;
    auto pack = [&](double F, int ci) { return __hiloint2double(__double2hiint(F), (__double2loint(F) & ~mask) | ci); };
    auto row = [&](int q) -> double { return WIDE ? SDP_AD_A_CONST(A, q) : (double)A[SHIFT ? 2 * q : q]; };
    auto brow = [&](int q) -> double { return SHIFT ? (double)A[2 * q + 1] : 0.0; };
    auto cell = [&](sdp_real xn0, int &q0, sdp_real &lam0) {
#if SDP_COL_SHIFT
        sdp_lean2s_cell<AXIS>(l, xn0, q0, lam0);
#else
        sdp_lean2_cell<AXIS>(l, xn0, q0, lam0);
#endif
    };
    auto start = [&](int b) -> sdp_real { return WIDE ? rec[4 * b] : rec[2 * b]; };
    auto least = [&](int b) -> double { return WIDE ? *(const double *)(rec + 4 * b + 2) : (double)rec[2 * b + 1]; };
    const int n_blocks = (n + BS - 1) / BS;
    const int g = guess < 0 ? (n >> 1) : min(guess, n - 1);
    const sdp_real ga = utab[g * SDP_COL_UTAB + SDP_LEAN2_A_SLOT];
    const sdp_real gh = SDP_LEAN2_H_SLOT < 0 ? (sdp_real)0 : utab[g * SDP_COL_UTAB + HS];
    const sdp_real pX = (SDP_LEAN2_FORM == 2 ? -((X + l.smin) * k_rows) : (X - l.smin) * k_rows) - (SHIFT ? l.koff : (sdp_real)0);
    const int extra = __builtin_amdgcn_readfirstlane(WIDE ? __float_as_int((float)rec[4 * n_blocks + 1]) : __double2loint((double)rec[2 * n_blocks + 1]));
    int gq;
    sdp_real glam;
    cell(SDP_LEAN2_LEAD(X, ga), gq, glam);
    const double gA0 = row(gq), gA1 = row(gq + 1), gB = brow(gq);
    unsigned long long need = 0ull;
    double thresh = 0.0;
    constexpr int CB = NB < SDP_BNB_CHUNK ? NB : SDP_BNB_CHUNK;
    for (int b0 = 0; b0 < n_blocks; b0 += CB) {
        int q[CB + 1];
        double P[CB + 1], hp[CB], Aq[CB + 1], Aq1[CB + 1], m[CB], Bq[SHIFT ? CB + 1 : 1], bm[SHIFT ? CB : 1];
#pragma unroll
        for (int j = 0; j <= CB; ++j) {
            const int b = min(b0 + j, n_blocks);
            P[j] = (double)(pX + start(b));
            if (j < CB) hp[j] = least(min(b, n_blocks - 1));
        }
#pragma unroll
        for (int j = 0; j <= CB; ++j) {
            q[j] = (int)P[j];
            asm("v_med3_i32 %0, %0, 0, %1" : "+v"(q[j]) : "s"(l.ordm2));
        }
#pragma unroll
        for (int j = 0; j <= CB; ++j) {
            Aq[j] = row(q[j]);
            Aq1[j] = row(q[j] + 1);
            if (SHIFT) Bq[j] = brow(q[j]);
        }
        if (SHIFT) {
#pragma unroll
            for (int j = 0; j < CB; ++j) bm[j] = sdp_vmax(sdp_vmax(Bq[j], brow(q[j] + 1)), Bq[j + 1]);
        }
        if (b0 == 0) {
            const double h = fma((double)glam, gA1 - gA0, gA0);
            const double Fg = pack(SDP_LEAN2_H_SLOT < 0 ? h : fma((double)(SDP_LEAN2_HNEG ? -gh : gh), psum, h), g);
            thresh = (SHIFT ? fma(BSCALE, gB, Fg) : Fg) + slack;
        }
#pragma unroll
        for (int j = 0; j <= CB; ++j) {
            const double lam = P[j] - (double)q[j];
            P[j] = fma(lam, Aq1[j] - Aq[j], Aq[j]);
        }
#pragma unroll
        for (int j = 0; j < CB; ++j) m[j] = sdp_vmin(sdp_vmin(P[j], P[j + 1]), sdp_vmin(Aq1[j], Aq[j + 1]));
        for (int k = 0; k < extra; ++k) {
            double more[CB];
#pragma unroll
            for (int j = 0; j < CB; ++j) more[j] = row(max(min(q[j] + 2 + k, q[j + 1] - 1), 0));
#pragma unroll
            for (int j = 0; j < CB; ++j) m[j] = sdp_vmin(m[j], more[j]);
            if (SHIFT) {
#pragma unroll
                for (int j = 0; j < CB; ++j) bm[j] = sdp_vmax(bm[j], brow(max(min(q[j] + 2 + k, q[j + 1] - 1), 0)));
            }
        }
#pragma unroll
        for (int j = 0; j < CB; ++j) {
            if (q[j + 1] - q[j] - 2 > extra) m[j] = -(double)INFINITY;
            const double lbv = SHIFT ? fma(-BSCALE, bm[j], hp[j] + m[j]) : hp[j] + m[j];
            if ((!(lbv > thresh) || b0 + j == g / BS) && b0 + j < n_blocks) need |= 1ull << (b0 + j);
        }
    }
#ifdef SDP_DIAG_BNB_COUNT
    sdp_diag_cnt = (sdp_real)(__popcll(need) + 100 * (g / BS));
#endif
    while (__any(need != 0ull)) {
        const bool on = need != 0ull;
        const int b = on ? __ffsll((long long)need) - 1 : 0;
        need &= need - 1ull;
        constexpr int K = SDP_SHORT_GROUP;
        static_assert(BS % K == 0, "branch and bound: whole groups per block");
        for (int j0 = 0; j0 < BS; j0 += K) {
            int q0[K], ci[K];
            sdp_real av[K], lam0[K], hv[K];
            double a0[K], a1[K], bq[SHIFT ? K : 1];
#pragma unroll
            for (int j = 0; j < K; ++j) {
                ci[j] = min(b * BS + j0 + j, n - 1);
                av[j] = utab[ci[j] * SDP_COL_UTAB + SDP_LEAN2_A_SLOT];
                hv[j] = SDP_LEAN2_H_SLOT < 0 ? (sdp_real)0 : utab[ci[j] * SDP_COL_UTAB + HS];
            }
#pragma unroll
            for (int j = 0; j < K; ++j) cell(SDP_LEAN2_LEAD(X, av[j]), q0[j], lam0[j]);
#pragma unroll
            for (int j = 0; j < K; ++j) {
                a0[j] = row(q0[j]);
                a1[j] = row(q0[j] + 1);
                if (SHIFT) bq[j] = brow(q0[j]);
            }
            if (SHIFT) {
#pragma unroll
                for (int j = 0; j < K; ++j)
                    if (on && b * BS + j0 + j < n) *b_seen = sdp_vmax(*b_seen, (sdp_real)bq[j]);
            }
#pragma unroll
            for (int j = 0; j < K; ++j) {
                const double h = fma((double)lam0[j], a1[j] - a0[j], a0[j]);
                const double Fp = pack(SDP_LEAN2_H_SLOT < 0 ? h : fma((double)(SDP_LEAN2_HNEG ? -hv[j] : hv[j]), psum, h), ci[j]);
                insert(on && b * BS + j0 + j < n ? Fp : 0x1.fffffffffffffp+1023);
            }
        }
    }
}
#endif

SDP_DEV void sdp_col_bounds_merge(SdpColBounds &b, int d)
{
    const sdp_fkey o_f1 = sdp_shfl_xor(b.f1, d), o_f2 = sdp_shfl_xor(b.f2, d);
    const sdp_real o_max = sdp_shfl_xor(b.s_max, d);
    const sdp_fkey o_sum = sdp_shfl_xor(b.s_sum, d);
    const int o_i1 = __shfl_xor(b.i1, d, 64);
    if (SDP_COL_TOP2) {
        const sdp_fkey o_f3 = sdp_shfl_xor(b.f3, d);
        const int o_i2 = __shfl_xor(b.i2, d, 64);
        sdp_col_bounds_insert(b, o_f1, o_i1);
        sdp_col_bounds_insert(b, o_f2, o_i2);
        sdp_col_bounds_insert(b, o_f3, INT_MAX);
    } else {
        const sdp_fkey mx = o_f1 > b.f1 ? o_f1 : b.f1;
        b.f2 = o_f2 < b.f2 ? o_f2 : b.f2;
        b.f2 = mx < b.f2 ? mx : b.f2;
        if (o_f1 < b.f1) { b.f1 = o_f1; b.i1 = o_i1; }
    }
    b.s_max = o_max > b.s_max ? o_max : b.s_max;
    b.s_sum = b.s_sum + o_sum;
    const sdp_real o_p = sdp_shfl_xor(b.p_max, d);
    b.p_max = o_p > b.p_max ? o_p : b.p_max;
    if (SDP_COL_SHIFT) {
        const sdp_real o_b = sdp_shfl_xor(b.b_max, d);
        b.b_max = o_b > b.b_max ? o_b : b.b_max;
    }
}


SDP_DEV void sdp_col_filter_nodes(const SdpSweepArgs &a, const SdpGrid<sdp_real, SDP_DT> &tg,
                                  const SdpColShared &s, const SdpColWeights &wts, const SdpLeadAxis &lead,
                                  const SdpColFilter &filt, int axis_mode, const sdp_real *ad_tab,
                                  const sdp_real *utab, sdp_real dcol,
                                  int64_t col, int i_lo, int i_hi, int wave, int waves,
                                  sdp_real *x, sdp_real t, SdpColDiag &diag,
                                  const SdpBox *box_c, int i_pre, sdp_real x0_pre
#if SDP_COL_SHIFT
                                  , const SdpColShiftCol &shc
#endif
                                  , int *guess_p = nullptr
                                  )
{
    (void)guess_p;
    constexpr int N0 = SDP_COL_N0;
    const int lane = threadIdx.x & 63;
    SdpLeadAxis lead1 = lead;
#if SDP_COL_SHIFT
    lead1.koff = (sdp_real)shc.kmin;
    lead1.ordm2 = shc.ok ? shc.rows - 2 : 0;
#endif
    const sdp_real *__restrict__ axis0 = (const sdp_real *)a.axes + a.axis_off[0];
    (void)diag;
    const int n_nodes = i_hi - i_lo;
    const int groups = (n_nodes + 63) >> 6;
    int chunks = groups < waves ? waves / groups : 1;
    chunks = 1 << (31 - __builtin_clz(chunks < 64 ? chunks : 64));
    const int npw = 64 / chunks;
    const int items = (n_nodes + npw - 1) / npw;
    __builtin_amdgcn_s_setprio(SDP_COL_B_PRIO);
    for (int item = wave; item < items; item += waves) {
        const int chunk = lane / npw;
        const int i_raw = i_lo + item * npw + (lane - chunk * npw);
        const bool live = i_raw < i_hi;
        const int i = live ? i_raw : i_hi - 1;
        const int64_t node = col * N0 + i;
        SdpBox box;
        x[0] = i == i_pre ? x0_pre : axis0[i];
        if (box_c) box = *box_c;
        else sdp_load_box(a, node, box);
        const int c_lo = (int)((int64_t)box.total * chunk / chunks);
        const int c_hi = (int)((int64_t)box.total * (chunk + 1) / chunks);
        SDP_COL_MARK(diag.m1);
#if SDP_COL_WIDE2
        static_assert(SDP_COL_WIDE_ON && SDP_COL_TOP2 && !SDP_COST_HAS_W && !SDP_COL_SHIFT && SDP_COL_UTAB,
                      "short first pass of the full-table kernel: the wide form of 4-byte reals");
        struct { double f1, f2, f3; int i1, i2; } bd;
        bool bad;
        sdp_fkey radius;
        const sdp_real X = sdp_model_lead_x(x, t);
        {
            const sdp_real *ust = utab + SDP_COL_UTAB * SDP_COL_UTAB_N;
            const sdp_real K = sdp_model_cost_x(x, t);
            const int bits = 32 - __clz(max(box.total - 1, 1));
            const int mask = (1 << bits) - 1;
            SdpShortBounds sb;
            sb.f1 = sb.f2 = sb.f3 = INFINITY;
            int q_e;
            sdp_real lam_lo, lam_hi;
            if (axis_mode == 2) {
                sdp_lean2_cell<2>(lead, SDP_LEAN2_LEAD(X, ust[0]), q_e, lam_lo);
                sdp_lean2_cell<2>(lead, SDP_LEAN2_LEAD(X, ust[1]), q_e, lam_hi);
            } else if (axis_mode == 1) {
                sdp_lean2_cell<1>(lead, SDP_LEAN2_LEAD(X, ust[0]), q_e, lam_lo);
                sdp_lean2_cell<1>(lead, SDP_LEAN2_LEAD(X, ust[1]), q_e, lam_hi);
            } else {
                sdp_lean2_cell<0>(lead, SDP_LEAN2_LEAD(X, ust[0]), q_e, lam_lo);
                sdp_lean2_cell<0>(lead, SDP_LEAN2_LEAD(X, ust[1]), q_e, lam_hi);
            }
            const sdp_real l_cap = sdp_vmax_abs(sdp_vmax_abs((sdp_real)1, lam_lo), lam_hi);
            const sdp_real s_node = (filt.gc + filt.pcap) * ((fabs(K) + ust[2]) + ((sdp_real)1 + (sdp_real)2 * l_cap) * dcol);
            bad = !filt.ok || !(s_node < SDP_COL_FILTER_LIMIT) || !(fabs(lam_lo) + fabs(lam_hi) < (sdp_real)1073741824.0) ||
                  bits > 24 || box.total > SDP_COL_UTAB_N;
            radius = (sdp_fkey)(SDP_COL_FILTER_SCALE) * (sdp_fkey)(1.001 * 0x1p-24) * ((sdp_fkey)s_node + (sdp_fkey)filt.floor) +
                     ldexp((sdp_fkey)s_node, bits - 51);
            bool full_pass = true;
#if SDP_COL_BNB
            if (__all(chunks == 1 && fabs(X) < ust[3] && !bad)) {
                full_pass = false;
                sdp_real cnt_unused = (sdp_real)0;
                const double slack = fma(2.0, (double)radius, 0x1p-40 * (double)s_node);
// ... 130 lines not shown
```

stodynprog_amd/csrc/sdp_colres_kernel.h:

```cpp
#pragma once

static_assert(SDP_COL_LEAN_ON && !SDP_COL_WIDE_ON, "resident chunks: the lean first pass of 8-byte reals");
static_assert(!SDP_COL_TOP2 || SDP_COL_SHIFT, "resident chunks: two carried survivors only on the shifted lattice");
static_assert(SDP_COL_WRES >= 1 && 2 * SDP_COL_WRES >= SDP_COL_W, "resident chunks: at least half of the points resident");
constexpr int SDP_COLRES_K = SDP_COL_TOP2 ? 2 : 1;

#ifndef SDP_COL_TAIL_HOLD
#define SDP_COL_TAIL_HOLD 0
#endif
#if SDP_COL_TAIL_HOLD && (!SDP_COL_A_WIDE_LOADS || SDP_COL_A_ORDER != 2 || SDP_COL_WPAIR || \
                          (SDP_COL_W - SDP_COL_WRES) % (SDP_COL_THREADS / SDP_COL_A_LW) != 0 || SDP_COL_ROWS % (2 * SDP_COL_A_LW) != 0)
#error "SDP_COL_TAIL_HOLD: the plain resident-chunk kernel with 16-byte build loads, whole rounds of points and rows"
#endif
#if SDP_COL_TAIL_HOLD
typedef sdp_real sdp_held_rows __attribute__((ext_vector_type(2)));
constexpr int SDP_HOLD_WP = SDP_COL_THREADS / SDP_COL_A_LW;
constexpr int SDP_HOLD_NW = (SDP_COL_W - SDP_COL_WRES) / SDP_HOLD_WP;
constexpr int SDP_HOLD_NJ = SDP_COL_ROWS / (2 * SDP_COL_A_LW);
template <bool BUILD>
SDP_DEV void sdp_colres_tail(const SdpSweepArgs &a, const SdpGrid<sdp_real, SDP_DT> &tg, const SdpColShared &s,
                             sdp_held_rows (&held)[SDP_HOLD_NW][SDP_HOLD_NJ])
{
    constexpr int N0 = SDP_COL_ROWS, C = SDP_COL_WRES, LW = SDP_COL_A_LW, NV = 1 << SDP_DT;
    const sdp_real *__restrict__ V = (const sdp_real *)a.V + s.r0;
// ... 74 lines not shown
    constexpr int B = SDP_COL_BATCH;
    const volatile sdp_lds_real *tab = (const volatile sdp_lds_real *)T;
#pragma unroll SDP_COL_UNROLL_W
    for (int w0 = w_lo; w0 < w_hi; w0 += B) {
        sdp_real lo[B][K], hi[B][K];
#if SDP_LEAD_HAS_W
        sdp_real lam_b[B][K], oml_b[B][K];
#endif
#pragma unroll
        for (int b = 0; b < B; ++b)
            if (w0 + b < w_hi) {
#pragma unroll
                for (int j = 0; j < K; ++j) {
#if SDP_LEAD_HAS_W
                    sdp_colres_cell(l, x, c.u[j], SDP_COL_GW(k, w0 + b), t, c.q0[j], lam_b[b][j], oml_b[b][j]);
#endif
                    lo[b][j] = tab[(w0 + b - t_base) * N0 + c.q0[j]];
                    hi[b][j] = tab[(w0 + b - t_base) * N0 + c.q0[j] + 1];
                }
            }
#pragma unroll
        for (int b = 0; b < B; ++b)
            if (w0 + b < w_hi) {
                const sdp_real pw = SDP_COL_PW(k, w0 + b);
#pragma unroll
                for (int j = 0; j < K; ++j) {
#if SDP_LEAD_HAS_W
                    const sdp_real val = oml_b[b][j] * lo[b][j] + lam_b[b][j] * hi[b][j];
#else
                    const sdp_real val = c.oml0[j] * lo[b][j] + c.lam0[j] * hi[b][j];
#endif
                    const sdp_real jc = c.g[j] + val;
                    c.acc[j] = c.acc[j] + jc * pw;
                }
            }
    }
}

#if SDP_COL_LEAN2
static_assert(!SDP_COST_HAS_W && (SDP_COL_SHIFT ? !SDP_COL_SHIFT_CHAIN : !SDP_COL_TOP2) && SDP_COL_UTAB && sizeof(sdp_real) == 8,
              "short first pass: 8-byte reals, control table, a perturbation that does not reach the cost and reaches the stock "
              "through final sums at most");
template <int AXIS>
SDP_DEV sdp_real sdp_lean2_value(const sdp_real *A, const sdp_real *utab, const SdpColFilter &f, const SdpLeadAxis &l,
                                 sdp_real X, int ci)
{
    int q0;
    sdp_real lam0;
    sdp_lean2_cell<AXIS>(l, SDP_LEAN2_LEAD(X, utab[ci * SDP_COL_UTAB + SDP_LEAN2_A_SLOT]), q0, lam0);
    const sdp_real a0 = A[q0], a1 = A[q0 + 1];
    const sdp_real h = fma(lam0, a1 - a0, a0);
    if (SDP_LEAN2_H_SLOT < 0) return h;
    const sdp_real hv = utab[ci * SDP_COL_UTAB + (SDP_LEAN2_H_SLOT < 0 ? 0 : SDP_LEAN2_H_SLOT)];
    return fma(SDP_LEAN2_HNEG ? -hv : hv, f.psum, h);
}
#ifndef SDP_LEAN2_GROUP
#define SDP_LEAN2_GROUP 4
#endif
template <int AXIS>
SDP_DEV void sdp_lean2_pass1(const sdp_real *A, const sdp_real *utab, const SdpColFilter &f, const SdpLeadAxis &l,
                             sdp_real X, int n, int mask, sdp_real &f1, sdp_real &f2)
{
    auto insert = [&](sdp_real F, int ci) {
        const sdp_real Fp = __hiloint2double(__double2hiint(F), (__double2loint(F) & ~mask) | ci);
        f2 = sdp_vmin(f2, sdp_vmax(f1, Fp));
        f1 = sdp_vmin(f1, Fp);
    };
    constexpr int K = SDP_LEAN2_GROUP;
    constexpr int HS = SDP_LEAN2_H_SLOT < 0 ? 0 : SDP_LEAN2_H_SLOT;
    int ci = 0;
    for (; ci + K <= n; ci += K) {
        int q0[K];
        sdp_real av[K], lam0[K], hv[K], a0[K], a1[K];
#pragma unroll
        for (int j = 0; j < K; ++j) {
            av[j] = utab[(ci + j) * SDP_COL_UTAB + SDP_LEAN2_A_SLOT];
            hv[j] = SDP_LEAN2_H_SLOT < 0 ? (sdp_real)0 : utab[(ci + j) * SDP_COL_UTAB + HS];
        }
#pragma unroll
        for (int j = 0; j < K; ++j) sdp_lean2_cell<AXIS>(l, SDP_LEAN2_LEAD(X, av[j]), q0[j], lam0[j]);
#pragma unroll
        for (int j = 0; j < K; ++j) {
            a0[j] = A[q0[j]];
            a1[j] = A[q0[j] + 1];
        }
#pragma unroll
        for (int j = 0; j < K; ++j) {
            const sdp_real h = fma(lam0[j], a1[j] - a0[j], a0[j]);
            insert(SDP_LEAN2_H_SLOT < 0 ? h : fma(SDP_LEAN2_HNEG ? -hv[j] : hv[j], f.psum, h), ci + j);
        }
    }
    for (; ci < n; ++ci) insert(sdp_lean2_value<AXIS>(A, utab, f, l, X, ci), ci);
}

#if SDP_COL_SHIFT
typedef sdp_real sdp_ab_pair __attribute__((ext_vector_type(2)));
template <int AXIS>
SDP_DEV sdp_real sdp_lean2s_value(const sdp_real *A, const sdp_real *utab, const SdpColFilter &f, const SdpLeadAxis &l,
                                  sdp_real X, int ci, sdp_real &bmax)
{
    int q0;
    sdp_real lam0;
    sdp_lean2s_cell<AXIS>(l, SDP_LEAN2_LEAD(X, utab[ci * SDP_COL_UTAB + SDP_LEAN2_A_SLOT]), q0, lam0);
    const sdp_ab_pair ab = *(const sdp_ab_pair *)(A + 2 * q0);
    const sdp_real a1 = A[2 * q0 + 2];
    bmax = sdp_vmax(bmax, ab.y);
    const sdp_real h = fma(lam0, a1 - ab.x, ab.x);
    if (SDP_LEAN2_H_SLOT < 0) return h;
    const sdp_real hv = utab[ci * SDP_COL_UTAB + (SDP_LEAN2_H_SLOT < 0 ? 0 : SDP_LEAN2_H_SLOT)];
    return fma(SDP_LEAN2_HNEG ? -hv : hv, f.psum, h);
}
template <int AXIS>
SDP_DEV void sdp_lean2s_pass1(const sdp_real *A, const sdp_real *utab, const SdpColFilter &f, const SdpLeadAxis &l,
                              sdp_real X, int n, int mask, sdp_real &f1, sdp_real &f2, sdp_real &f3, sdp_real &bmax)
{
    auto insert = [&](sdp_real F, int ci) {
        const sdp_real Fp = __hiloint2double(__double2hiint(F), (__double2loint(F) & ~mask) | ci);
        f3 = sdp_vmin(f3, sdp_vmax(f2, Fp));
        f2 = sdp_vmin(f2, sdp_vmax(f1, Fp));
        f1 = sdp_vmin(f1, Fp);
    };
    constexpr int K = SDP_LEAN2_GROUP;
    constexpr int HS = SDP_LEAN2_H_SLOT < 0 ? 0 : SDP_LEAN2_H_SLOT;
    int ci = 0;
    for (; ci + K <= n; ci += K) {
        int q0[K];
        sdp_real av[K], lam0[K], hv[K], a1[K];
        sdp_ab_pair ab[K];
#pragma unroll
        for (int j = 0; j < K; ++j) {
            av[j] = utab[(ci + j) * SDP_COL_UTAB + SDP_LEAN2_A_SLOT];
            hv[j] = SDP_LEAN2_H_SLOT < 0 ? (sdp_real)0 : utab[(ci + j) * SDP_COL_UTAB + HS];
        }
#pragma unroll
        for (int j = 0; j < K; ++j) sdp_lean2s_cell<AXIS>(l, SDP_LEAN2_LEAD(X, av[j]), q0[j], lam0[j]);
#pragma unroll
        for (int j = 0; j < K; ++j) {
            ab[j] = *(const sdp_ab_pair *)(A + 2 * q0[j]);
            a1[j] = A[2 * q0[j] + 2];
        }
#pragma unroll
        for (int j = 0; j < K; ++j) {
            bmax = sdp_vmax(bmax, ab[j].y);
            const sdp_real h = fma(lam0[j], a1[j] - ab[j].x, ab[j].x);
            insert(SDP_LEAN2_H_SLOT < 0 ? h : fma(SDP_LEAN2_HNEG ? -hv[j] : hv[j], f.psum, h), ci + j);
        }
    }
    for (; ci < n; ++ci) insert(sdp_lean2s_value<AXIS>(A, utab, f, l, X, ci, bmax), ci);
}
#endif

#endif

extern "C" __global__ void __launch_bounds__(SDP_COL_THREADS, SDP_COL_MIN_WAVES) sdp_sweep_col(SdpSweepArgs a)
{
    __shared__ SdpColLds sdp_lds;
    SDP_STAMP_BEGIN(a);
    const int lane = threadIdx.x & 63;
    const int wave = threadIdx.x >> 6;
    const int waves = blockDim.x >> 6;
    constexpr int N0 = SDP_COL_N0;
    constexpr int Wn = SDP_COL_W;
    constexpr int C = SDP_COL_WRES, R = Wn - C;
    sdp_trap_unless(a.n_lead == N0 && a.W == Wn && (int)blockDim.x == SDP_COL_THREADS);
    const sdp_real t = (sdp_real)a.t_k;
    const sdp_real *__restrict__ axis0 = (const sdp_real *)a.axes + a.axis_off[0];

    SdpColShared s;
    sdp_col_carve(sdp_lds, s);
    SdpGrid<sdp_real, SDP_DT> tg;
    sdp_col_trailing_grid(a, tg);
    SdpLeadAxis lead;
    sdp_col_lead_axis(a, lead);
    SdpColWalk walk;
    sdp_col_walk(a, walk);
    SdpColWeights wts;
    sdp_col_load_weights(a, wts);
    SdpColFilter filt;
    sdp_col_filter_setup(a, filt);
    const int axis_mode = __builtin_amdgcn_readfirstlane(sdp_col_axis_mode(lead));
    const sdp_cst_real *pw = (const sdp_cst_real *)a.proba;
    lead.smin = sdp_uniform(lead.smin); lead.span = sdp_uniform(lead.span); lead.nm1 = sdp_uniform(lead.nm1); lead.rspan = sdp_uniform(lead.rspan);
    filt.psum = sdp_uniform(filt.psum); filt.pcap = sdp_uniform(filt.pcap); filt.cu = sdp_uniform(filt.cu);
    filt.floor = sdp_uniform(filt.floor); filt.ratio = sdp_uniform(filt.ratio);
    const sdp_real k_rows = sdp_uniform(lead.nm1 / lead.span);
    const sdp_real x_cap = sdp_uniform((sdp_real)(SDP_COL_SHIFT ? 0x1p29 : 0x1p30) / k_rows - fabs(lead.smin));
    (void)k_rows; (void)x_cap;
    if (threadIdx.x < 2) sdp_lds.dcol[threadIdx.x] = 0ull;
    int parity = 0;

    const int64_t u_base = walk.unit - (blockIdx.x >> 3), u_end = walk.end;
    unsigned int *claim = a.claim + 32 * (blockIdx.x & 7);
    if (threadIdx.x == 0) sdp_lds.next_unit = (int)atomicAdd(claim, 1u);
    __syncthreads();
    int64_t unit = u_base + sdp_lds.next_unit;
    int upar = 0;
#if SDP_STAMP == 2
    unsigned long long tm_build = 0, tm_p1 = 0, tm_all = 0, tm_top = 0, tm0 = 0, tm1 = 0, tm_start = __builtin_amdgcn_s_memtime();
#define SDP_RES_MARK(v) v = __builtin_amdgcn_s_memtime()
#else
#define SDP_RES_MARK(v)
#endif
    int guess = -1;
    int tables_made = 1;
    (void)tables_made;
    (void)guess;
#if SDP_COL_UTAB
    sdp_trap_unless(!a.box_per_node);
#endif
    SdpBox box_hold;
    const SdpBox *box_c = nullptr;
    const sdp_real *w_mine = nullptr;
    sdp_real w_hold = (sdp_real)0;
    if (!a.box_per_node) {
        sdp_load_box(a, 0, box_hold);
#pragma unroll
        for (int c = 0; c < SDP_NU; ++c) {
            box_hold.lo[c] = sdp_uniform(box_hold.lo[c]); box_hold.hi[c] = sdp_uniform(box_hold.hi[c]);
            box_hold.step[c] = sdp_uniform(box_hold.step[c]); box_hold.delta[c] = sdp_uniform(box_hold.delta[c]);
            box_hold.n[c] = sdp_uniform(box_hold.n[c]);
        }
        box_hold.total = sdp_uniform(box_hold.total);
        box_c = &box_hold;
    }
    if (lane < Wn && !SDP_COL_TAIL_HOLD) { w_hold = ((const sdp_real *)a.wgrid)[lane]; w_mine = &w_hold; }
#if SDP_COL_SHIFT
    if (threadIdx.x < 2) sdp_col_shift_reset(sdp_lds, threadIdx.x);
    __syncthreads();
#endif
    if (unit < u_end) {
        sdp_real xn[SDP_D];
        sdp_col_coords(a, sdp_col_of_unit(a, unit), xn);
        sdp_col_phase_w(a, tg, s, xn, nullptr, t);
#if SDP_COL_UTAB
        sdp_col_phase_u(a, sdp_lds.utab[0], xn, t, 0, 64, box_c, filt.psum, k_rows, x_cap, (double)filt.psum);
#endif
#if SDP_COL_SHIFT
        sdp_col_phase_shift(a, sdp_lds, lead, xn, t, 0);
#endif
    }
    while (unit < u_end) {
        const int64_t col = sdp_col_of_unit(a, unit);
        const int part = (int)((unsigned)unit % (unsigned)a.col_splits);
        const int i_lo = (int)((unsigned)(N0 * part) / (unsigned)a.col_splits);
        const int i_hi = (int)((unsigned)(N0 * (part + 1)) / (unsigned)a.col_splits);
        sdp_real x[SDP_D];
        sdp_col_coords(a, col, x);
        const int r = sdp_col_tid();
        SDP_RES_MARK(tm0);
        __syncthreads();
#if SDP_STAMP == 2
        { const unsigned long long tmb = __builtin_amdgcn_s_memtime(); tm_top += tmb - tm0; tm0 = tmb; }
#endif
        int nx = 0;
        if (wave == waves - 1 && lane == 0) nx = (int)atomicAdd(claim, 1u);
#if SDP_COL_SHIFT
        if (threadIdx.x == 0) sdp_col_shift_reset(sdp_lds, upar ^ 1);
        SdpColShiftCol shc;
        sdp_col_shift_col(sdp_lds, lead, upar, shc);
        sdp_col_shift_zero(sdp_lds, shc);
#endif
#if SDP_COL_TAIL_HOLD
        sdp_held_rows held[SDP_HOLD_NW][SDP_HOLD_NJ];
        sdp_colres_tail<true>(a, tg, s, held);
#else
        if (!(SDP_DIAG_SKIP & 1)) sdp_col_phase_a<false>(a, tg, s, C, R);
#endif
        __syncthreads();
#if SDP_COL_SHIFT
        sdp_col_shift_reduce(a, sdp_lds, filt, shc, parity, upar, C, R);
#else
        sdp_real acc_t = (sdp_real)0, big = (sdp_real)0;
        if (r < N0 && !(SDP_DIAG_SKIP & 1)) {
#pragma unroll SDP_COL_FILTER_RUNROLL
            for (int w = 0; w < R; ++w) {
                const sdp_real v = sdp_lds.T[w * N0 + r];
                acc_t = acc_t + pw[C + w] * v;
                big = sdp_vmax_abs(big, v);
            }
        }
#endif
        __syncthreads();
        if (!(SDP_DIAG_SKIP & 2)) sdp_col_phase_a<false>(a, tg, s, 0, C);
        if (wave == waves - 1 && lane == 0) sdp_lds.next_unit = nx;
        __syncthreads();
        __builtin_amdgcn_s_setprio(SDP_COL_B_PRIO);
#if SDP_COL_SHIFT
        sdp_col_shift_reduce(a, sdp_lds, filt, shc, parity, upar, 0, C);
#else
        {
            sdp_real dmax = (sdp_real)0;
            if (r < N0) {
                sdp_real acc = (sdp_real)0;
#pragma unroll SDP_COL_FILTER_RUNROLL
                for (int w = 0; w < ((SDP_DIAG_SKIP & 2) ? 0 : C); ++w) {
                    const sdp_real v = sdp_lds.T[w * N0 + r];
                    acc = acc + pw[w] * v;
                    big = sdp_vmax_abs(big, v);
                }
                acc = acc + acc_t;
                dmax = acc == acc ? filt.pcap * big + filt.floor : (sdp_real)INFINITY;
                sdp_lds.ad[r] = acc;
            }
            dmax = sdp_wave_max(dmax);
            if (lane == 0) atomicMax(&sdp_lds.dcol[parity], (unsigned long long)__double_as_longlong((double)dmax));
        }
#endif
        (void)r;
        __syncthreads();
        SDP_RES_MARK(tm1);
#if SDP_STAMP == 2
        tm_build += tm1 - tm0;
#endif
        const sdp_real dcol = sdp_col_filter_dcol(sdp_lds, parity);
        parity ^= 1;
        const int64_t next_unit = u_base + sdp_lds.next_unit;
        SdpLeadAxis lead1 = lead;
#if SDP_COL_SHIFT
        lead1.koff = (sdp_real)shc.kmin;
        lead1.ordm2 = shc.ok ? shc.rows - 2 : 0;
#endif
        const int i = i_lo + (int)threadIdx.x;
        const bool live = i < i_hi;
        const int64_t node = col * N0 + (live ? i : i_hi - 1);
        SdpBox box;
        if (box_c) box = *box_c;
        else sdp_load_box(a, node, box);
        sdp_real best = INFINITY;
        sdp_real diag_cnt = (sdp_real)-1;
        (void)diag_cnt;
        int ibest = INT_MAX;
        SdpColresCand cd;
        cd.n = 0;
#pragma unroll
        for (int j = 0; j < SDP_COLRES_K; ++j) {
            cd.acc[j] = cd.g[j] = cd.lam0[j] = cd.oml0[j] = (sdp_real)0;
            cd.q0[j] = 0;
            cd.idx[j] = INT_MAX;
#pragma unroll
            for (int c = 0; c < SDP_NU; ++c) cd.u[j][c] = (sdp_real)0;
        }
        if (live && (SDP_DIAG_SKIP & 4)) {
            x[0] = axis0[i];
            cd.n = 1; cd.idx[0] = 3; ibest = 3;
            sdp_controls_at(box, 3, cd.u[0]);
            cd.g[0] = sdp_model_cost(x, cd.u[0], (sdp_real)0, t);
            sdp_colres_cell(lead, x, cd.u[0], (sdp_real)0, t, cd.q0[0], cd.lam0[0], cd.oml0[0]);
        } else
        if (live) {
            x[0] = axis0[i];
#if SDP_COL_LEAN2 && SDP_COL_SHIFT
            const sdp_real *utab = sdp_lds.utab[upar];
            const sdp_real *ust = utab + SDP_COL_UTAB * SDP_COL_UTAB_N;
            const sdp_real X = sdp_model_lead_x(x, t), K = sdp_model_cost_x(x, t);
            const int bits = 32 - __clz(max(box.total - 1, 1));
            const int mask = (1 << bits) - 1;
            struct { sdp_real f1, f2, f3; int i1, i2; } bd;
            bd.f1 = bd.f2 = bd.f3 = INFINITY;
            int q_e;
            sdp_real lam_lo, lam_hi, b_max = (sdp_real)0;
            if (axis_mode == 2) {
                sdp_lean2s_cell<2>(lead1, SDP_LEAN2_LEAD(X, ust[0]), q_e, lam_lo);
                sdp_lean2s_cell<2>(lead1, SDP_LEAN2_LEAD(X, ust[1]), q_e, lam_hi);
            } else if (axis_mode == 1) {
                sdp_lean2s_cell<1>(lead1, SDP_LEAN2_LEAD(X, ust[0]), q_e, lam_lo);
                sdp_lean2s_cell<1>(lead1, SDP_LEAN2_LEAD(X, ust[1]), q_e, lam_hi);
            } else {
                sdp_lean2s_cell<0>(lead1, SDP_LEAN2_LEAD(X, ust[0]), q_e, lam_lo);
                sdp_lean2s_cell<0>(lead1, SDP_LEAN2_LEAD(X, ust[1]), q_e, lam_hi);
            }
            const sdp_real l_cap = sdp_vmax_abs(sdp_vmax_abs((sdp_real)1, lam_lo), lam_hi);
            const sdp_real h_cap = (((sdp_real)1 + (sdp_real)2 * (l_cap + shc.lc)) * ((sdp_real)3 + shc.es)) * dcol;
            const sdp_real s_node = fma(filt.pcap, fabs(K) + ust[2], h_cap);
            const bool bad = !filt.ok || !shc.ok || !(s_node < SDP_COL_FILTER_LIMIT) ||
                             !(fabs(lam_lo) + fabs(lam_hi) + shc.lc < (sdp_real)1073741824.0) || bits > 24 || box.total > SDP_COL_UTAB_N;
            const sdp_real radius0 = (filt.cu + (sdp_real)(SDP_COL_FILTER_SCALE) * ldexp(SDP_COL_FILTER_EPS, bits + 1)) * s_node;
#if SDP_COL_BNB
            const sdp_real slack = fma((sdp_real)2, radius0, ((sdp_real)12 * SDP_COL_FILTER_EPS) * s_node);
            const bool bnb = fabs(X) < ust[3] && shc.ok;
            if (__all(bnb)) {
                auto ins = [&](double Fq) {
                    bd.f3 = sdp_vmin(bd.f3, sdp_vmax(bd.f2, Fq));
                    bd.f2 = sdp_vmin(bd.f2, sdp_vmax(bd.f1, Fq));
                    bd.f1 = sdp_vmin(bd.f1, Fq);
                };
                if (axis_mode == 2) sdp_short_bnb<2, false>(sdp_lds.ad, utab, filt, lead1, X, k_rows, 0, box.total, mask, slack, guess, ins, diag_cnt, &b_max);
                else if (axis_mode == 1) sdp_short_bnb<1, false>(sdp_lds.ad, utab, filt, lead1, X, k_rows, 0, box.total, mask, slack, guess, ins, diag_cnt, &b_max);
                else sdp_short_bnb<0, false>(sdp_lds.ad, utab, filt, lead1, X, k_rows, 0, box.total, mask, slack, guess, ins, diag_cnt, &b_max);
            } else
#endif
            {
                if (axis_mode == 2) sdp_lean2s_pass1<2>(sdp_lds.ad, utab, filt, lead1, X, box.total, mask, bd.f1, bd.f2, bd.f3, b_max);
                else if (axis_mode == 1) sdp_lean2s_pass1<1>(sdp_lds.ad, utab, filt, lead1, X, box.total, mask, bd.f1, bd.f2, bd.f3, b_max);
                else sdp_lean2s_pass1<0>(sdp_lds.ad, utab, filt, lead1, X, box.total, mask, bd.f1, bd.f2, bd.f3, b_max);
            }
            const sdp_real radius = fma((sdp_real)(SDP_COL_FILTER_SCALE), b_max, radius0);
            bd.i1 = bd.f1 < (sdp_real)INFINITY ? (__double2loint(bd.f1) & mask) : INT_MAX;
            bd.i2 = bd.f2 < (sdp_real)INFINITY ? (__double2loint(bd.f2) & mask) : INT_MAX;
#elif SDP_COL_LEAN2
            const sdp_real *utab = sdp_lds.utab[upar];
            const sdp_real *ust = utab + SDP_COL_UTAB * SDP_COL_UTAB_N;
            const sdp_real X = sdp_model_lead_x(x, t), K = sdp_model_cost_x(x, t);
            const int bits = 32 - __clz(max(box.total - 1, 1));
            const int mask = (1 << bits) - 1;
            struct { sdp_real f1, f2; int i1, i2; } bd;
            bd.f1 = bd.f2 = INFINITY;
            bd.i2 = INT_MAX;
            int q_e;
            sdp_real lam_lo, lam_hi;
            if (axis_mode == 2) {
                sdp_lean2_cell<2>(lead, SDP_LEAN2_LEAD(X, ust[0]), q_e, lam_lo);
                sdp_lean2_cell<2>(lead, SDP_LEAN2_LEAD(X, ust[1]), q_e, lam_hi);
            } else if (axis_mode == 1) {
                sdp_lean2_cell<1>(lead, SDP_LEAN2_LEAD(X, ust[0]), q_e, lam_lo);
                sdp_lean2_cell<1>(lead, SDP_LEAN2_LEAD(X, ust[1]), q_e, lam_hi);
            } else {
                sdp_lean2_cell<0>(lead, SDP_LEAN2_LEAD(X, ust[0]), q_e, lam_lo);
                sdp_lean2_cell<0>(lead, SDP_LEAN2_LEAD(X, ust[1]), q_e, lam_hi);
            }
            const sdp_real l_cap = sdp_vmax_abs(sdp_vmax_abs((sdp_real)1, lam_lo), lam_hi);
            const sdp_real s_node = fma(filt.pcap, fabs(K) + ust[2], ((sdp_real)1 + (sdp_real)2 * l_cap) * dcol);
            const bool bad = !filt.ok || !(s_node < SDP_COL_FILTER_LIMIT) || !(fabs(lam_lo) + fabs(lam_hi) < (sdp_real)1073741824.0) ||
                             bits > 24 || box.total > SDP_COL_UTAB_N;
            const sdp_real radius = (filt.cu + (sdp_real)(SDP_COL_FILTER_SCALE) * ldexp(SDP_COL_FILTER_EPS, bits + 1)) * s_node;
#if SDP_COL_BNB
            const sdp_real slack = fma((sdp_real)2, radius, ((sdp_real)8 * SDP_COL_FILTER_EPS) * s_node);
            const bool bnb = fabs(X) < ust[3];
            if (__all(bnb)) {
                auto ins = [&](double Fq) {
                    bd.f2 = sdp_vmin(bd.f2, sdp_vmax(bd.f1, Fq));
                    bd.f1 = sdp_vmin(bd.f1, Fq);
                };
                if (axis_mode == 2) sdp_short_bnb<2, false>(sdp_lds.ad, utab, filt, lead, X, k_rows, 0, box.total, mask, slack, guess, ins, diag_cnt);
                else if (axis_mode == 1) sdp_short_bnb<1, false>(sdp_lds.ad, utab, filt, lead, X, k_rows, 0, box.total, mask, slack, guess, ins, diag_cnt);
                else sdp_short_bnb<0, false>(sdp_lds.ad, utab, filt, lead, X, k_rows, 0, box.total, mask, slack, guess, ins, diag_cnt);
            } else
#endif
            {
                if (axis_mode == 2) sdp_lean2_pass1<2>(sdp_lds.ad, utab, filt, lead, X, box.total, mask, bd.f1, bd.f2);
                else if (axis_mode == 1) sdp_lean2_pass1<1>(sdp_lds.ad, utab, filt, lead, X, box.total, mask, bd.f1, bd.f2);
                else sdp_lean2_pass1<0>(sdp_lds.ad, utab, filt, lead, X, box.total, mask, bd.f1, bd.f2);
            }
            bd.i1 = bd.f1 < (sdp_real)INFINITY ? (__double2loint(bd.f1) & mask) : INT_MAX;
#else
            SdpColBounds bd;
            bd.f1 = bd.f2 = bd.f3 = INFINITY;
            bd.s_max = bd.s_sum = bd.p_max = bd.b_max = (sdp_real)0;
            bd.i1 = bd.i2 = INT_MAX;
            const sdp_real *utab = sdp_lds.utab[upar];
            const bool plain = SDP_NU == 1 && box.n[0] > 1 && box.step[0] != (sdp_real)0;
            if (plain) {
                if (axis_mode == 2) sdp_col_filter_pass1<true, 2>(sdp_lds.ad, utab, filt, lead1, box, x, t, 0, box.total, bd);
                else if (axis_mode == 1) sdp_col_filter_pass1<true, 1>(sdp_lds.ad, utab, filt, lead1, box, x, t, 0, box.total, bd);
                else sdp_col_filter_pass1<true, 0>(sdp_lds.ad, utab, filt, lead1, box, x, t, 0, box.total, bd);
            } else {
                if (axis_mode == 2) sdp_col_filter_pass1<false, 2>(sdp_lds.ad, utab, filt, lead1, box, x, t, 0, box.total, bd);
                else if (axis_mode == 1) sdp_col_filter_pass1<false, 1>(sdp_lds.ad, utab, filt, lead1, box, x, t, 0, box.total, bd);
                else sdp_col_filter_pass1<false, 0>(sdp_lds.ad, utab, filt, lead1, box, x, t, 0, box.total, bd);
            }
#if SDP_COL_SHIFT
            const sdp_real h_cap = (((sdp_real)1 + (sdp_real)2 * (bd.p_max + shc.lc)) * ((sdp_real)3 + shc.es)) * dcol;
            const sdp_real s_node = fma(filt.ratio, bd.s_sum + h_cap, h_cap);
            const bool bad = !filt.ok || !shc.ok || !(s_node < SDP_COL_FILTER_LIMIT) || !(bd.p_max + shc.lc < (sdp_real)1073741824.0);
            const sdp_real radius = fma(filt.cu, s_node, (sdp_real)(SDP_COL_FILTER_SCALE) * bd.b_max);
#else
            const sdp_real h_cap = ((sdp_real)1 + (sdp_real)2 * bd.p_max) * dcol;
            const sdp_real s_node = fma(filt.ratio, bd.s_sum + h_cap, h_cap);
            const bool bad = !filt.ok || !(s_node < SDP_COL_FILTER_LIMIT) || !(bd.p_max < (sdp_real)1073741824.0);
            const sdp_real radius = filt.cu * s_node;
#endif
#endif
            const sdp_real m_hi = bd.f1 + radius;
            const bool single = !bad && bd.i1 != INT_MAX && bd.f2 - radius > m_hi;
#if SDP_COL_LEAN2 && !SDP_COL_SHIFT
            const bool pair = false;
#else
            const bool pair = SDP_COL_TOP2 && !bad && !single && bd.i2 != INT_MAX && bd.f3 - radius > m_hi;
#endif
            if (single || pair) {
                cd.n = single ? 1 : 2;
                cd.idx[0] = single ? bd.i1 : min(bd.i1, bd.i2);
                if (SDP_COLRES_K > 1) cd.idx[SDP_COLRES_K - 1] = single ? bd.i1 : max(bd.i1, bd.i2);
                else ibest = bd.i1;
#pragma unroll
                for (int j = 0; j < SDP_COLRES_K; ++j) {
                    sdp_controls_at(box, cd.idx[j], cd.u[j]);
                    cd.g[j] = sdp_model_cost(x, cd.u[j], (sdp_real)0, t);
#if !SDP_LEAD_HAS_W
                    sdp_colres_cell(lead, x, cd.u[j], (sdp_real)0, t, cd.q0[j], cd.lam0[j], cd.oml0[j]);
#endif
                }
            } else {
                for (int ci = 0; ci < box.total; ++ci) {
                    sdp_real u[SDP_NU];
                    sdp_controls_at(box, ci, u);
                    bool cand = bad;
                    if (!cand) {
#if SDP_COL_LEAN2 && SDP_COL_SHIFT
                        sdp_real b_unused = (sdp_real)0;
                        const sdp_real F = lead.pow2 ? sdp_lean2s_value<1>(sdp_lds.ad, utab, filt, lead1, X, ci, b_unused)
                                                     : sdp_lean2s_value<0>(sdp_lds.ad, utab, filt, lead1, X, ci, b_unused);
#elif SDP_COL_LEAN2
                        const sdp_real F = lead.pow2 ? sdp_lean2_value<1>(sdp_lds.ad, utab, filt, lead, X, ci)
                                                     : sdp_lean2_value<0>(sdp_lds.ad, utab, filt, lead, X, ci);
#else
                        sdp_real F, pm = (sdp_real)0, gm = (sdp_real)0, bm = (sdp_real)0;
                        if (lead.pow2) sdp_col_lean_eval<1>(sdp_lds.ad, filt, lead1, x, u, t, F, pm, gm, bm);
                        else sdp_col_lean_eval<0>(sdp_lds.ad, filt, lead1, x, u, t, F, pm, gm, bm);
#endif
                        cand = !(F - radius > m_hi);
                    }
                    if (cand) {
                        const sdp_real jc = sdp_col_cost_global<false>(a, tg, s, wts, lead, x, u, t);
                        if (ibest == INT_MAX || sdp_better_seq(jc, best)) { best = jc; ibest = ci; }
                    }
                }
            }
        }
#if SDP_STAMP == 2
        tm_p1 += __builtin_amdgcn_s_memtime() - tm1;
#endif
        const bool two = SDP_COLRES_K > 1 && __any(cd.n == 2);
        if (SDP_DIAG_SKIP & 8) {}
        else if (SDP_COLRES_K > 1 && two) sdp_colres_partial<SDP_COLRES_K>(sdp_lds.T, wts, lead, x, t, 0, C, 0, cd);
        else if (cd.n) sdp_colres_partial<1>(sdp_lds.T, wts, lead, x, t, 0, C, 0, cd);
        __syncthreads();
        __builtin_amdgcn_s_setprio(0);
#if SDP_COL_TAIL_HOLD
        sdp_colres_tail<false>(a, tg, s, held);
#else
        if (!(SDP_DIAG_SKIP & 16)) sdp_col_phase_a<false>(a, tg, s, C, R);
#endif
        __syncthreads();
        __builtin_amdgcn_s_setprio(SDP_COL_B_PRIO);
        if (SDP_DIAG_SKIP & 32) {}
        else if (SDP_COLRES_K > 1 && two) sdp_colres_partial<SDP_COLRES_K>(sdp_lds.T, wts, lead, x, t, C, Wn, C, cd);
        else if (cd.n) sdp_colres_partial<1>(sdp_lds.T, wts, lead, x, t, C, Wn, C, cd);
        if (live) {
#pragma unroll
            for (int j = 0; j < SDP_COLRES_K; ++j) {
                if (SDP_COLRES_K == 1) { if (cd.n) best = cd.acc[0]; }
                else if (j < cd.n && (ibest == INT_MAX || sdp_better_seq(cd.acc[j], best))) { best = cd.acc[j]; ibest = cd.idx[j]; }
            }
#ifdef SDP_DIAG_BNB_COUNT
            best = diag_cnt;
#endif
            if (!(SDP_DIAG_SKIP & 128)) sdp_col_store(a, node, box, best, ibest);
            if (ibest != INT_MAX) guess = ibest;
        }
        {
            const int nxu = __builtin_amdgcn_readfirstlane(sdp_lds.next_unit);
            if (u_base + nxu < u_end && !(SDP_DIAG_SKIP & 64)) {
                sdp_real xn[SDP_D];
                sdp_col_coords(a, sdp_col_of_unit(a, u_base + nxu), xn);
                sdp_col_phase_w(a, tg, s, xn, nullptr, t, (waves - 1) * 64, 64, w_mine);
#if SDP_COL_UTAB
                sdp_col_phase_u(a, sdp_lds.utab[upar ^ 1], xn, t, max(waves - 2, 0) * 64, 64, box_c, filt.psum, k_rows, x_cap, (double)filt.psum,
                                SDP_LEAN2_A_FIXED_ON && tables_made >= 2);
                ++tables_made;
#endif
#if SDP_COL_SHIFT
                sdp_col_phase_shift(a, sdp_lds, lead, xn, t, upar ^ 1, max(waves - 3, 0) * 64, 64);
#endif
            }
        }
        __builtin_amdgcn_s_setprio(0);
        upar ^= 1;
        unit = next_unit;
    }
    if (threadIdx.x == 0) {
        __threadfence();
        if (atomicAdd(a.claim + 256, 1u) == gridDim.x - 1) {
            for (int k = 0; k < 8; ++k) atomicExch(a.claim + 32 * k, 0u);
            atomicExch(a.claim + 256, 0u);
        }
    }
#if SDP_STAMP == 2
    if (a.stamps && (threadIdx.x & 63) == 0) {
        tm_all = __builtin_amdgcn_s_memtime() - tm_start;
        unsigned long long *o = a.stamps + ((size_t)blockIdx.x * (blockDim.x >> 6) + (threadIdx.x >> 6)) * 4;
        o[0] = tm_build; o[1] = tm_p1; o[2] = tm_top; o[3] = tm_all;
    }
#else
    SDP_STAMP_END(a);
#endif
}

extern "C" __global__ void __launch_bounds__(SDP_COL_THREADS) sdp_evalpol_col(SdpSweepArgs a)
{
    __shared__ SdpColLds sdp_lds;
    constexpr int N0 = SDP_COL_N0;
    constexpr int Wn = SDP_COL_W;
    constexpr int C = SDP_COL_WRES;
    sdp_trap_unless(a.n_lead == N0 && a.W == Wn);
    const sdp_real t = (sdp_real)a.t_k;
    const sdp_real *__restrict__ axis0 = (const sdp_real *)a.axes + a.axis_off[0];
    SdpColShared s;
    sdp_col_carve(sdp_lds, s);
    SdpGrid<sdp_real, SDP_DT> tg;
    sdp_col_trailing_grid(a, tg);
    tg.shift = a.shift_index >= 0 ? ((const sdp_real *)a.V)[a.shift_index] : (sdp_real)0;
    if (a.ref_out && blockIdx.x == 0 && threadIdx.x == 0) *a.ref_out = (double)tg.shift;
    SdpLeadAxis lead;
    sdp_col_lead_axis(a, lead);
    SdpColWalk walk;
    sdp_col_walk(a, walk);
    SdpColWeights wts;
    sdp_col_load_weights(a, wts);
    for (int64_t unit = walk.unit; unit < walk.end; unit += walk.stride) {
        const int64_t col = sdp_col_of_unit(a, unit);
        const int part = (int)((unsigned)unit % (unsigned)a.col_splits);
        const int i_lo = (int)((unsigned)(N0 * part) / (unsigned)a.col_splits);
        const int i_hi = (int)((unsigned)(N0 * (part + 1)) / (unsigned)a.col_splits);
        sdp_real x[SDP_D];
        sdp_col_coords(a, col, x);
        __syncthreads();
        sdp_col_phase_w(a, tg, s, x, nullptr, t);
        for (int i0 = i_lo; i0 < i_hi; i0 += (int)blockDim.x) {
            const int i = i0 + (int)threadIdx.x;
            const bool live = i < i_hi;
            const int64_t node = col * N0 + (live ? i : i_hi - 1);
            SdpColresCand cd;
            cd.n = 1;
            cd.acc[0] = (sdp_real)0;
            cd.idx[0] = 0;
            x[0] = axis0[live ? i : i_hi - 1];
#pragma unroll
            for (int c = 0; c < SDP_NU; ++c) cd.u[0][c] = ((const sdp_real *)a.pol_in)[node * SDP_NU + c];
            cd.g[0] = sdp_model_cost(x, cd.u[0], (sdp_real)0, t);
            cd.q0[0] = 0; cd.lam0[0] = cd.oml0[0] = (sdp_real)0;
#if !SDP_LEAD_HAS_W
            sdp_colres_cell(lead, x, cd.u[0], (sdp_real)0, t, cd.q0[0], cd.lam0[0], cd.oml0[0]);
#endif
            for (int w0 = 0; w0 < Wn; w0 += C) {
                const int cnt = min(C, Wn - w0);
                __syncthreads();
                sdp_col_phase_a<true>(a, tg, s, w0, cnt);
                __syncthreads();
                sdp_colres_partial<1>(sdp_lds.T, wts, lead, x, t, w0, w0 + cnt, w0, cd);
            }
            const sdp_real acc = cd.acc[0];
            if (live) sdp_store_J<sdp_real>(a, node, col, acc);
        }
    }
}
```

stodynprog_amd/csrc/sdp_column_kernel.h:

```cpp
#pragma once
#include "sdp_sweep_kernel.h"
#include <type_traits>

#if SDP_D >= 2

#ifndef SDP_COL_THREADS
#define SDP_COL_THREADS 512
#endif
#ifndef SDP_COL_UNROLL_W
#define SDP_COL_UNROLL_W 4
#endif
#ifndef SDP_COL_A_GROUP
#define SDP_COL_A_GROUP 4
#endif
#ifndef SDP_COL_A_ORDER
#define SDP_COL_A_ORDER 0
#endif
#ifndef SDP_COL_A_LW
#define SDP_COL_A_LW 16
#endif
#ifndef SDP_COLU_WIDE_LOADS
#define SDP_COLU_WIDE_LOADS 0
#endif
#ifndef SDP_COLU_A_GROUP
#define SDP_COLU_A_GROUP (SDP_COLU_WIDE_LOADS ? 2 : SDP_COL_A_GROUP)
#endif
#ifndef SDP_COL_A_WIDE_LOADS
#define SDP_COL_A_WIDE_LOADS 0
#endif
#ifndef SDP_COL_MIN_WAVES
#define SDP_COL_MIN_WAVES 4
#endif
#if defined(SDP_WAVES_CAP) && SDP_COL_MIN_WAVES > SDP_WAVES_CAP
#undef SDP_COL_MIN_WAVES
#define SDP_COL_MIN_WAVES SDP_WAVES_CAP
#endif
#ifndef SDP_COL_WPAIR
#define SDP_COL_WPAIR 0
#endif
#ifndef SDP_COL_BATCH
#if SDP_COL_WPAIR || SDP_LEAD_HAS_W
#define SDP_COL_BATCH 2
#else
#define SDP_COL_BATCH 4
#endif
#endif
#ifndef SDP_COL_UNROLL_U
#if SDP_COL_WPAIR
#define SDP_COL_UNROLL_U 4
#else
#define SDP_COL_UNROLL_U 2
#endif
#endif
#if SDP_COL_WPAIR && (!SDP_HAS_W || SDP_LEAD_HAS_W)
#error "SDP_COL_WPAIR needs a perturbation and an x0' that does not depend on it"
#endif
#ifndef SDP_TRAIL_HAS_U
#define SDP_TRAIL_HAS_U 0
#endif
#ifndef SDP_COL_ROWS
#define SDP_COL_ROWS SDP_COL_N0
#endif
#ifndef SDP_COL_FILTER
#define SDP_COL_FILTER 0
#endif
#ifndef SDP_COL_FILTER_UNROLL
#define SDP_COL_FILTER_UNROLL (sizeof(SDP_REAL) == 8 ? 8 : 4)
#endif
#define SDP_COL_B_PRIO 3
#ifndef SDP_COL_FILTER_RUNROLL
#define SDP_COL_FILTER_RUNROLL 16
#endif
#ifndef SDP_COL_UTAB
#define SDP_COL_UTAB 0
#endif
#ifndef SDP_COL_UTAB_N
#define SDP_COL_UTAB_N 1
#endif
#ifndef SDP_COL_FILTER_SCALE
#define SDP_COL_FILTER_SCALE 1
#endif
#ifndef SDP_COL_SHIFT
#define SDP_COL_SHIFT 0
#endif
#ifndef SDP_COL_SHIFT_CHAIN
#define SDP_COL_SHIFT_CHAIN 0
#endif
#ifndef SDP_COL_SHIFT_ROWS
#define SDP_COL_SHIFT_ROWS (2 * SDP_COL_N0)
#endif
#ifndef SDP_COL_WRES
#define SDP_COL_WRES SDP_COL_W
#endif
#if SDP_COL_WRES < SDP_COL_W && (!SDP_COL_FILTER || SDP_COL_WPAIR || SDP_COST_HAS_W || \
                                 SDP_COL_ROWS < SDP_COL_N0 || SDP_COL_THREADS < SDP_COL_N0 || 2 * SDP_COL_WRES < SDP_COL_W)
#error "SDP_COL_WRES: lean filtered kernel, plain full-column table, one lane per node, at least half of the points resident"
#endif
#ifndef SDP_COL_LEAN2
#define SDP_COL_LEAN2 0
#endif
#ifndef SDP_COL_WIDE2
#define SDP_COL_WIDE2 0
#endif
#define SDP_COL_SHORT (SDP_COL_LEAN2 || SDP_COL_WIDE2)
#ifndef SDP_COL_BNB
#define SDP_COL_BNB 0
#endif
#ifndef SDP_LEAN2_A_FIXED
#define SDP_LEAN2_A_FIXED 0
#endif
constexpr bool SDP_LEAN2_A_FIXED_ON = SDP_LEAN2_A_FIXED && SDP_COL_BNB;
constexpr int sdp_bnb_block(int n) { int b = 8; while ((n + b - 1) / b > 64) b *= 2; return b; }
template <typename T>
SDP_DEV T sdp_col_opaque(T v)
{
#if defined(SDP_COL_TAIL_HOLD) && SDP_COL_TAIL_HOLD
    asm volatile("" : "+v"(v));
#endif
    return v;
}
SDP_DEV int sdp_col_tid() { return sdp_col_opaque((int)threadIdx.x); }
#if SDP_COL_FILTER && (!SDP_HAS_W || (SDP_LEAD_HAS_W && !SDP_COL_SHIFT) || SDP_TRAIL_HAS_U || SDP_COL_ROWS < SDP_COL_N0)
#error "SDP_COL_FILTER needs a perturbation that reaches x0' through a final sum at most, and the plain full-column table"
#endif
#if SDP_COL_SHIFT && (!SDP_COL_FILTER || !SDP_LEAD_HAS_W || SDP_COL_WPAIR)
#error "SDP_COL_SHIFT is a form of the certified filter for a perturbation that reaches x0'"
#endif
#if SDP_COL_FILTER && SDP_COST_HAS_W && SDP_COL_UTAB
#error "the control table holds sub-expressions without the perturbation: not with a cost that depends on it"
#endif
#if SDP_TRAIL_HAS_U && (SDP_COL_WPAIR || SDP_COL_ROWS < SDP_COL_N0)
#error "control-dependent trailing dynamics: plain full table, exact arithmetic only"
#endif
#if SDP_COL_ROWS < SDP_COL_N0 && SDP_COL_WPAIR
#error "the row window is built for the plain table layout with exact arithmetic"
#endif
constexpr bool SDP_COL_WINDOW = SDP_COL_ROWS < SDP_COL_N0;
constexpr int SDP_DT = SDP_D - 1;
constexpr int SDP_COL_TW = SDP_COL_WPAIR ? (SDP_COL_W + 1) / 2 * 2 : SDP_COL_W;

struct SdpColShared {
    sdp_real *T;
    int *w_off;
    sdp_real *w_lam;
    sdp_real *w_oml;
    sdp_real *part_J;
    int *part_i;
    int r0;
};

#ifndef SDP_COL_WCHUNK
#define SDP_COL_WCHUNK SDP_COL_W
#endif
constexpr int SDP_COL_LDS_PART = (SDP_COL_FILTER || SDP_TRAIL_HAS_U) ? 1 : SDP_COL_THREADS;
constexpr int SDP_BNB_BLOCK = sdp_bnb_block(SDP_COL_UTAB_N);
constexpr int SDP_BNB_BLOCKS = (SDP_COL_UTAB_N + SDP_BNB_BLOCK - 1) / SDP_BNB_BLOCK;
constexpr int SDP_BNB_WORDS = SDP_COL_UTAB ? 4 * (SDP_BNB_BLOCKS + 1) : 0;
#define SDP_AD_A(ad, r) (SDP_COL_WIDE2 ? ((double *)(ad))[(r)] : *(double *)((ad) + 4 * (r)))
#define SDP_AD_A_CONST(ad, r) (SDP_COL_WIDE2 ? ((const double *)(ad))[(r)] : *(const double *)((ad) + 4 * (r)))
constexpr int SDP_COL_LDS_AD = sizeof(SDP_REAL) == 4 ? 4 : (!SDP_COL_SHIFT ? 1 : 2);
struct __attribute__((aligned(16))) SdpColLds {
    sdp_real T[(SDP_TRAIL_HAS_U ? SDP_COL_WCHUNK : (SDP_COL_WRES < SDP_COL_W ? SDP_COL_WRES : SDP_COL_TW)) * SDP_COL_ROWS];
    sdp_real w_lam[SDP_COL_W * SDP_DT];
    sdp_real w_oml[SDP_COL_W * SDP_DT];
    sdp_real reserve_[2];
    sdp_real part_J[SDP_COL_LDS_PART];
    int part_i[SDP_COL_LDS_PART];
    int w_off[SDP_COL_W * SDP_DT];
    int win[2][2];
    int next_unit;
    unsigned long long dcol[2];
    sdp_real utab[2][SDP_COL_UTAB ? SDP_COL_UTAB * SDP_COL_UTAB_N + 4 + SDP_BNB_WORDS : 2] __attribute__((aligned(16)));
#if SDP_COL_FILTER
    sdp_real ad[SDP_COL_LDS_AD * (SDP_COL_SHIFT ? SDP_COL_SHIFT_ROWS : SDP_COL_ROWS)] __attribute__((aligned(16)));
#endif
#if SDP_COL_SHIFT
    int sh_q[2][SDP_COL_W];
    sdp_real sh_f[2][SDP_COL_W];
    sdp_real sh_c[2][SDP_COL_W];
    int sh_k[2][4];
#endif
};
static_assert(sizeof(SdpColLds) <= 160 * 1024, "column table exceeds the 160 KiB LDS of a CU");

struct SdpColDiag {
    unsigned long long m1 = 0, m2 = 0, tp1 = 0, tp2 = 0, n_slow = 0, n_exact = 0, n_all = 0;
};
#if SDP_STAMP == 2
#define SDP_COL_MARK(v) v = __builtin_amdgcn_s_memtime()
#else
#define SDP_COL_MARK(v)
#endif

SDP_DEV void sdp_col_carve(SdpColLds &m, SdpColShared &s)
{
    s.T = m.T;
    s.w_lam = m.w_lam;
    s.w_oml = m.w_oml;
    s.w_off = m.w_off;
    s.part_J = m.part_J;
    s.part_i = m.part_i;
    s.r0 = 0;
}

SDP_DEV double sdp_uniform_real(double v) { return __hiloint2double(__builtin_amdgcn_readfirstlane(__double2hiint(v)), __builtin_amdgcn_readfirstlane(__double2loint(v))); }
SDP_DEV float sdp_uniform_real(float v) { return __int_as_float(__builtin_amdgcn_readfirstlane(__float_as_int(v))); }
SDP_DEV void sdp_col_trailing_grid(const SdpSweepArgs &a, SdpGrid<sdp_real, SDP_DT> &g)
{
    const sdp_real *axes = (const sdp_real *)a.axes;
    int m = SDP_COL_N0;
    g.pow2 = 0;
#pragma unroll
    for (int k = SDP_DT - 1; k >= 0; --k) {
        const int ax = k + 1;
        g.smin[k] = axes[a.axis_off[ax]];
        g.span[k] = axes[a.axis_off[ax] + a.orders[ax] - 1] - g.smin[k];
        g.rspan[k] = (sdp_real)1 / g.span[k];
        if (sdp_is_pow2(g.span[k])) g.pow2 |= 1 << k;
        g.nm1[k] = (sdp_real)(a.orders[ax] - 1);
        g.ordm2[k] = a.orders[ax] - 2;
        g.M[k] = m;
        m *= a.orders[ax];
    }
    g.pow2 = __builtin_amdgcn_readfirstlane(g.pow2);
    g.shift = (sdp_real)0;
#pragma unroll
    for (int k = 0; k < SDP_DT; ++k) {
        g.smin[k] = sdp_uniform_real(g.smin[k]); g.span[k] = sdp_uniform_real(g.span[k]);
        g.rspan[k] = sdp_uniform_real(g.rspan[k]); g.nm1[k] = sdp_uniform_real(g.nm1[k]);
    }
}

template <int K>
struct SdpColGather {
    static SDP_DEV void run(const sdp_real *__restrict__ V, const SdpGrid<sdp_real, SDP_DT> &g,
                            const int *off, int base, sdp_real *vals)
    {
        SdpColGather<K + 1>::run(V, g, off, base + off[K], vals);
        SdpColGather<K + 1>::run(V, g, off, base + off[K] + g.M[K], vals + (1 << (SDP_DT - K - 1)));
    }
};
template <>
struct SdpColGather<SDP_DT> {
    static SDP_DEV void run(const sdp_real *__restrict__ V, const SdpGrid<sdp_real, SDP_DT> &,
                            const int *, int base, sdp_real *vals)
    {
        vals[0] = V[base];
    }
};
template <int K, bool SHIFT>
struct SdpColNest {
    static SDP_DEV sdp_real run(const sdp_real *vals, const sdp_real *lam, const sdp_real *oml,
                                sdp_real shift)
    {
        const sdp_real lo = SdpColNest<K + 1, SHIFT>::run(vals, lam, oml, shift);
        const sdp_real hi = SdpColNest<K + 1, SHIFT>::run(vals + (1 << (SDP_DT - K - 1)), lam, oml, shift);
        return oml[K] * lo + lam[K] * hi;
    }
};
template <bool SHIFT>
struct SdpColNest<SDP_DT - 1, SHIFT> {
    static SDP_DEV sdp_real run(const sdp_real *vals, const sdp_real *lam, const sdp_real *oml,
                                sdp_real shift)
    {
        sdp_real lo = vals[0], hi = vals[1];
        if (SHIFT) { lo = lo - shift; hi = hi - shift; }
        return oml[SDP_DT - 1] * lo + lam[SDP_DT - 1] * hi;
    }
};

SDP_DEV void sdp_col_phase_w(const SdpSweepArgs &a, const SdpGrid<sdp_real, SDP_DT> &tg,
                             const SdpColShared &s, const sdp_real *x, const sdp_real *u, sdp_real t,
                             int first = 0, int count = 0, const sdp_real *w_mine = nullptr)
{
    constexpr int Wn = SDP_COL_W;
#if SDP_HAS_W
    const sdp_real *__restrict__ wgrid = (const sdp_real *)a.wgrid;
#endif
    if (count == 0) count = (int)blockDim.x - first;
    const int tid = sdp_col_tid();
    if (tid < first || tid >= first + count) return;
    for (int w = tid - first; w < Wn; w += count) {
        sdp_real xn[SDP_D];
#if SDP_HAS_W
        sdp_model_trail(x, u, (w_mine && w == tid - first) ? *w_mine : wgrid[w], t, xn);
#else
        sdp_model_trail(x, u, (sdp_real)0, t, xn);
#endif
        SdpCell<sdp_real, SDP_DT, sdp_real> c;
#pragma unroll
        for (int k = 0; k < SDP_DT; ++k) {
            sdp_locate_axis<sdp_real, SDP_DT, sdp_real>(tg, k, xn[k + 1], c);
            s.w_off[w * SDP_DT + k] = c.off[k];
            s.w_lam[w * SDP_DT + k] = c.lam[k];
            s.w_oml[w * SDP_DT + k] = c.oml[k];
        }
    }
}

extern "C" __device__ double __ockl_wfred_max_f64(double);
extern "C" __device__ double __ockl_wfred_min_f64(double);
extern "C" __device__ double __ockl_wfred_add_f64(double);
extern "C" __device__ float __ockl_wfred_max_f32(float);
extern "C" __device__ float __ockl_wfred_min_f32(float);
extern "C" __device__ float __ockl_wfred_add_f32(float);
SDP_DEV double sdp_wave_max(double v) { return __ockl_wfred_max_f64(v); }
SDP_DEV double sdp_uniform(double v) { return __hiloint2double(__builtin_amdgcn_readfirstlane(__double2hiint(v)), __builtin_amdgcn_readfirstlane(__double2loint(v))); }
SDP_DEV float sdp_uniform(float v) { return __int_as_float(__builtin_amdgcn_readfirstlane(__float_as_int(v))); }
SDP_DEV int sdp_uniform(int v) { return __builtin_amdgcn_readfirstlane(v); }
template <int CTRL>
SDP_DEV double sdp_dpp_f64(double v)
{
    const int lo = __builtin_amdgcn_update_dpp(0, __double2loint(v), CTRL, 0xF, 0xF, false);
    const int hi = __builtin_amdgcn_update_dpp(0, __double2hiint(v), CTRL, 0xF, 0xF, false);
    return __hiloint2double(hi, lo);
}
template <int CTRL>
SDP_DEV float sdp_dpp_f64(float v) { return __int_as_float(__builtin_amdgcn_update_dpp(0, __float_as_int(v), CTRL, 0xF, 0xF, false)); }
SDP_DEV float sdp_wave_max(float v) { return __ockl_wfred_max_f32(v); }
SDP_DEV double sdp_wave_min(double v) { return __ockl_wfred_min_f64(v); }
SDP_DEV float sdp_wave_min(float v) { return __ockl_wfred_min_f32(v); }
SDP_DEV double sdp_wave_sum(double v) { return __ockl_wfred_add_f64(v); }
SDP_DEV float sdp_wave_sum(float v) { return __ockl_wfred_add_f32(v); }

template <bool SHIFT = false>
SDP_DEV void sdp_col_phase_a(const SdpSweepArgs &a, const SdpGrid<sdp_real, SDP_DT> &tg,
                             const SdpColShared &s, const int w_begin = 0, const int w_count = SDP_COL_W)
// ... 583 lines not shown
```

stodynprog_amd/solver.py:

```python
from __future__ import division, print_function
import ctypes as C
import itertools
from datetime import datetime

import numpy as np

from . import _native as nat
from . import codegen
from . import convergence as conv
from . import montecarlo as mc
from .interp import MlinInterpolator
from .trace import TraceError, trace_model, trace_box, callable_fingerprint, _fp_value, _NoFingerprint

__all__ = ['DPSolver']


class _DeviceProblem(object):

    def __init__(self, desc_arrays, module_path, dtype, shape, nu, W, lanes, box_per_node,
                 node_range, comm=None, slab_bounds=None, layout=0, staged=None, col_seg_nodes=0):
        self._keep = desc_arrays
        self.layout = int(layout)
        self.dtype = np.dtype(dtype)
        self.shape = tuple(shape)
# ... 396 lines not shown
        fp = callable_fingerprint(s.dyn, s.cost, s.params) if self.trace_cache else None
        key = ('trace now', s.stationnary)
        if fp is not None:
            kept = self._cache.get(key)
            if kept is not None and kept[0] == fp:
                return kept[1]
        model = self._trace_now_uncached(t_k)
        if fp is not None and (s.stationnary or (not isinstance(model, TraceError) and model.t_value is None)):
            self._cache[key] = (fp, model)
        return model

    def _trace_now_uncached(self, t_k=None):
        s = self.sys
        try:
            model = trace_model(s.dyn, s.cost, len(s.state), len(s.control), len(s.perturb),
                                s.params, s.stationnary)
            key = ('struct', model.structure_key())
            bits = np.asarray(model.param_values(), dtype=float).tobytes()
            seen = self._cache.setdefault(key, dict(bits=bits, lifted=False))
            if not seen['lifted'] and seen['bits'] != bits:
                seen['lifted'] = True
            if seen['lifted']:
                model.lift_constants()
            return model
        except TraceError as e:
            if s.stationnary or t_k is None:
                return e
            try:
                model = trace_model(s.dyn, s.cost, len(s.state), len(s.control),
                                    len(s.perturb), s.params, s.stationnary, t_value=int(t_k))
            except TraceError:
                return e
            model.lift_constants()
            return model

    def _check_supported(self):
        if len(self.perturb_grid) > 1:
            raise NotImplementedError('only one perturbation variable is supported '
                                      '(as in the reference, sdp.py:664-666)')
        d = len(self.state_grid)
        if d > 5:
            raise NotImplementedError('interpolation for state dimension >5'
                                      ' is not implemented.')
        if d > 4:
            raise Exception("Can't interpolate in dimension strictly greater than 5")

    def _box_plan(self, box_t=None):
        key = ('box', self._fingerprint(box_t))
        bp = self._cache.get(key)
        fp = callable_fingerprint(self.sys.control_box, self.sys.params) if self.trace_cache else None
        if bp is not None and fp is not None and bp.get('fp') == fp and bp.get('sig') is not None:
            return bp
        tb = self._trace_box_now(box_t)
        if bp is not None:
            if not isinstance(tb, TraceError):
                if bp.get('sig') != tb.signature():
                    bp = None
                else:
                    bp['fp'] = fp
            elif bp.get('sig') is not None or self.box_recheck == 'every node' or not self._box_still_valid(bp, box_t):
                bp = None
        if bp is None:
            lo, hi, n = self._box_table(box_t, traced=tb)
            per_node = not (np.all(lo == lo[:, :1]) and np.all(hi == hi[:, :1])
                            and np.all(n == n[:, :1]))
            max_u = int(np.prod(n.astype(np.int64), axis=0).max())
            if max_u >= 2 ** 31:
                raise ValueError('control lattice too large')
            if not per_node:
                lo, hi, n = lo[:, :1], hi[:, :1], n[:, :1]
            lo, hi, n = (np.ascontiguousarray(a) for a in (lo, hi, n))
            digest = hash((lo.tobytes(), hi.tobytes(), n.tobytes()))
            bp = dict(lo=lo, hi=hi, n=n, per_node=per_node, max_u=max_u,
                      lanes=codegen.lanes_for(max_u), digest=digest, mode=getattr(self, '_box_mode', None),
                      sig=getattr(self, '_box_sig', None), fp=fp)
            if box_t is not None:
                for k in [k for k in self._cache if k[0] == 'box']:
                    del self._cache[k]
            self._cache[key] = bp
        return bp

    def _box_still_valid(self, bp, box_t, n_probe=21):
        shape = self._shape()
        S = int(np.prod(shape))
        lo, hi, n = bp['lo'], bp['hi'], bp['n']
        self._box_probe_round = getattr(self, '_box_probe_round', 0) + 1
        rng = np.random.default_rng(self._box_probe_round)
        probe = set(rng.integers(0, S, size=min(S, n_probe)).tolist())
        probe.update([0, S - 1, S // 2])
        lead = () if box_t is None else (box_t,)
        try:
            for flat in probe:
                ind = np.unravel_index(flat, shape)
                x = tuple(g[i] for g, i in zip(self.state_grid, ind))
                box = self.sys.control_box(*(lead + x), **self.sys.params)
                col = flat if bp['per_node'] else 0
                for c, (a, b) in enumerate(box):
                    a, b = float(a), float(b)
                    with np.errstate(all='ignore'):
                        n_interv = (b - a) / self.control_steps[c]
                    if n_interv < 0.1:
                        a = b = (a + b) / 2
                        npts = 1
                    else:
                        npts = int(np.ceil(n_interv) + 1)
                    if not (_same(lo[c, col], a) and _same(hi[c, col], b) and n[c, col] == npts):
                        return False
        except Exception:
            return False
        return True

    def _kernel_plan(self, box_t=None, model=None):
        if model is None:
            model = self._traced()
        if isinstance(model, TraceError):
            raise model
        shape = self._shape()
        dt = self.dtype
        bp = self._box_plan(box_t)
        lanes = bp['lanes']
        debug = codegen.check_debug(self.debug_defines)
        W = len(self.perturb_grid[0]) if self.perturb_grid else 0
        mk = getattr(model, '_plan_key', None)
        if mk is None or mk[0] != (model.param_index is not None):
            mk = (model.param_index is not None, model.structure_key(), np.asarray(model.param_values(), dtype=float).tobytes())
            try:
                model._plan_key = mk
            except AttributeError:
                pass
        memo = ('plan', self._fingerprint(None), bp['digest'], None if box_t is None else float(box_t),
                mk[1], mk[2], model.param_index is not None, model.t_value, bool(self._cache.get('no_lead')))
        kept = self._cache.get(memo)
        if kept is not None:
            return dict(kept, model=model)
        plan = self._kernel_plan_now(box_t, model, bp, lanes, debug, W)
        plan['_memo'] = memo
        for k in [k for k in self._cache if k[0] == 'plan' and k[1:4] != memo[1:4]]:
            del self._cache[k]
        self._cache[memo] = plan
        return plan

    def _plans_direct_exchange(self):
        return bool(self.comm is not None and self.comm.is_device and 1 < self.comm.nranks <= 8
                    and self.comm_exchange == 'direct')

    def _kernel_plan_now(self, box_t, model, bp, lanes, debug, W):
        shape = self._shape()
        dt = self.dtype
        if self.kernel not in ('auto', 'generic', 'column', 'staged', 'lead', 'line'):
            raise ValueError("kernel must be 'auto', 'column', 'lead', 'line', 'staged' or 'generic'")
        may_filter = (getattr(self, 'certified_filter', True)
                      and codegen.column_filter_applies(model, dtype=dt, table=(shape[0], W, len(shape)), debug=debug))
        n_controls = bp['max_u'] if box_t is None else 1 << max(int(bp['max_u']) - 1, 0).bit_length()
        col_cfg, utab, wres = None, None, 0
        if self.kernel in ('auto', 'column') and model.storage_separable:
            wpair = codegen.use_wpair(model, dt, debug)
            shift = bool(may_filter and codegen.column_shift_applies(model, dt, debug=debug))
            fr = codegen.control_table_plan(model, dt, bp['per_node'], n_controls, debug) if may_filter else None
            for frontier in ((fr, None) if fr is not None else (None,)):
                kw = dict(max_controls=n_controls, n_columns=int(np.prod(shape[1:])), shift=shift,
                          utab_values=codegen.utab_reals(len(frontier), n_controls) if frontier else 0, debug=debug)
                col_cfg = codegen.column_config(shape[0], W, len(shape), dt, wpair, may_filter, **kw)
                if col_cfg is not None:
                    utab = (frontier, n_controls) if frontier is not None else None
                    wres = codegen.column_resident_points(model, shape[0], W, len(shape), dt, may_filter, shift, wpair,
                                                          col_cfg[0], kw['utab_values'], debug)
                    if wres:
                        col_cfg = codegen.column_config(shape[0], W, len(shape), dt, wpair, may_filter, wres=wres, **kw)
                    break
        column = col_cfg is not None
        lead_axes = 0
        if (not column and self.kernel in ('auto', 'lead') and W > 0 and not self._cache.get('no_lead')
                and (self.comm is None or self.comm.is_device)
                and getattr(self, 'certified_filter', True)):
            lead_axes = codegen.lead_filter_applies(
                model, dt, 1 if (self.kernel == 'lead' or model.storage_separable) else 2, debug)
        lead_perm = None
        if (not column and not lead_axes and self.kernel in ('auto', 'lead') and W > 0 and not self._cache.get('no_lead')
                and (self.comm is None or self.comm.is_device)
                and getattr(self, 'certified_filter', True)):
            co = codegen.lead_order(model, dt, debug)
            if co is not None:
                lead_axes, lead_perm = co
        if self.kernel == 'lead' and not lead_axes:
            raise ValueError("kernel = 'lead' needs controlled state variables next to an exogenous process, "
                             'a perturbation that reaches only that process, 8-byte reals and the certified '
                             'filter (several GPUs: a device communicator)')
        if lead_axes:
            lanes = 1
        per_control = (not column and not lead_axes and self.kernel in ('auto', 'column') and model.column_shareable
                       and model.trail_depends_on_u
                       and (self.kernel == 'column' or int(np.prod(shape)) >= self.PERCONTROL_MIN_NODES)
                       and self._box_constant_along_axis0(bp, shape))
        per_control_cfg = None
        if per_control:
            per_control_cfg = codegen.column_percontrol_config(shape[0], W, len(shape), dt, debug)
            column = per_control = per_control_cfg is not None
        window = None
        if (not column and not per_control and not lead_axes and self.kernel in ('auto', 'column')
                and model.storage_separable):
            window = codegen.column_window_config(shape[0], W, len(shape), dt,
                                                  self._lead_reach_rows(model, bp, box_t))
            column = window is not None
        if (not column or per_control) and not lead_perm and self.kernel in ('auto', 'column'):
            k = model.separable_axis_hint()
            if k is not None and not self._cache.get('hinted'):
                self._cache['hinted'] = True
                import warnings
                warnings.warn('state variable "{}" is the only one driven by the control: listing it '
                              'FIRST in dyn/cost/control_box (and in discretize_state) lets the fast '
                              'column kernel run this model'.format(self.sys.state[k]))
        if self.kernel == 'column' and not column:
            raise ValueError('the column kernel needs a storage-separable model whose '
                             'table fits in LDS')
        staged = None
        S_nodes = int(np.prod(shape))
        small = (len(shape) == 1 or S_nodes <= self.STAGED_MIN_NODES
                 or (S_nodes <= 4 * self.STAGED_MIN_NODES and bp['max_u'] * max(W, 1) >= self.STAGED_MIN_WORK))
        if not column and not lead_axes and (self.kernel == 'staged' or (self.kernel == 'auto' and not small)):
            key = ('staged', model.structure_key(), bp['digest'], str(dt), shape, W, _dbg_key(debug))
            staged = self._cache.get(key)
            if staged is None:
                staged = codegen.staged_config(model, self.state_grid, self.perturb_grid, bp, dt,
                                               0.0 if box_t is None else float(box_t), debug=debug)
                self._cache[key] = staged
        line = 0
        if (len(shape) == 1 and self.kernel in ('auto', 'line') and self.comm is None and W > 0 and staged is None
                and getattr(self, 'certified_filter', True) and box_t is None
                and model.t_value is None and model.param_index is None
                and (self.kernel == 'line' or S_nodes * int(bp['max_u']) * W >= self.LINE_MIN_CELLS)
                and codegen.line_filter_applies(model, dt, W, debug)):
            line = W
            pow2 = lambda v: 1 << max(int(np.ceil(np.log2(max(v, 1)))), 0)
            need = pow2(W * 64 / 2048.)
            want = min(pow2(131072. / S_nodes), max(1 << int(np.floor(np.log2(max(bp['max_u'] / 32., 1)))), 1))
            lanes = int(min(64, max(need, want)))
        if self.kernel == 'line' and not line:
            raise ValueError("kernel = 'line' needs one state variable whose perturbation enters x' through final sums "
                             "(x + u - w), a cost that does not see it, 8-byte reals, a stationary system, the certified "
                             'filter, one GPU')
        filtered = bool(column and getattr(self, 'certified_filter', True) and codegen.column_filter_applies(
            model, window, per_control_cfg if per_control else None, dtype=dt,
            table=(shape[0], W, len(shape)), debug=debug))
        if not filtered or window is not None or per_control:
            utab = None
        source = codegen.translation_unit(model, dt, lanes,
                                          column=(shape[0], W, n_controls, int(np.prod(shape[1:]))) if column else None,
                                          staged=staged,
                                          window=window, per_control=per_control_cfg if per_control else None,
                                          filtered=filtered, utab=utab, lead_axes=lead_axes,
                                          col_cfg=col_cfg, debug=debug, wres=wres if filtered else 0,
                                          lead_perm=lead_perm, line=line, peer_stores=self._plans_direct_exchange())
        filtered = filtered or bool(lead_axes) or bool(line)
        return dict(model=model, source=source, column=column, lanes=lanes, staged=staged, filtered=filtered,
                    lead_axes=lead_axes, lead_perm=lead_perm, line=bool(line),
                    window=window, per_control=per_control,
                    col_seg_nodes=(window[3] if window else (per_control_cfg[0] if per_control else 0)),
                    per_node=bp['per_node'], lo=bp['lo'], hi=bp['hi'], n=bp['n'],
                    max_u=bp['max_u'], W=W, box_digest=bp['digest'], box_mode=bp.get('mode'))

    @staticmethod
    def _box_constant_along_axis0(bp, shape):
        if not bp['per_node']:
            return True
        n0 = shape[0]
        for arr in (bp['lo'], bp['hi'], bp['n']):
            a = arr.reshape(arr.shape[0], n0, -1)
            if not (a == a[:, :1, :]).all():
                return False
        return True

    def _lead_reach_rows(self, model, bp, box_t=None, n_samples=4096, around=False):
        from .trace import evaluate
        shape = self._shape()
        S = int(np.prod(shape))
        rng = np.random.default_rng(7)
        flat = np.unique(np.concatenate([rng.integers(0, S, size=min(S, n_samples)), [0, S - 1]]))
        idx = np.unravel_index(flat, shape)
        x = [np.asarray(g, dtype=float)[i] for g, i in zip(self.state_grid, idx)]
        col = flat if bp['per_node'] else np.zeros_like(flat)
        nu = len(self.sys.control)
        ends = []
        for first in (True, False):
            ends.append([bp['lo'][c, col] if first else bp['hi'][c, col] for c in range(nu)])
        wg = np.asarray(self.perturb_grid[0], dtype=float) if (self.perturb_grid and model.n_perturb) else None
        ws = [None] if wg is None else ([wg[0], wg[-1]] if model.lead_depends_on_w else [wg[0]])
        g0 = np.asarray(self.state_grid[0], dtype=float)
        rows = []
        for u in ends:
            for w in ws:
                with np.errstate(all='ignore'):
                    xn, _ = evaluate(model, x, u, [] if w is None else [w],
                                     0.0 if box_t is None else float(box_t))
                p = (np.asarray(xn[0], dtype=float) - g0[0]) / (g0[-1] - g0[0]) * (len(g0) - 1)
                rows.append(np.clip(np.nan_to_num(p, nan=0.0, posinf=1e9, neginf=-1e9), 0, len(g0) - 2))
        rows = np.array([np.broadcast_to(r, flat.shape) for r in rows])
        if around:
            return int(np.ceil(np.abs(rows - idx[0][None, :]).max())) + 1
        return int(np.ceil((rows.max(axis=0) - rows.min(axis=0)).max())) + 1

    def _problem(self, t_k=None, model=None):
        self._check_supported()
        box_t = None if self.sys.stationnary else t_k
        if model is None:
            model = self._trace_now(t_k)
        if isinstance(model, TraceError):
            raise model
        plan = self._kernel_plan(box_t, model)
        skey = plan.get('_source_key')
        if skey is None:
            skey = codegen.source_key(plan['source'])
            kept_plan = self._cache.get(plan.get('_memo'))
            if kept_plan is not None:
                kept_plan['_source_key'] = skey
        fp = ('problem', self._fingerprint(None), plan['box_digest'], skey)
        prob = self._cache.get(fp)
        if prob is None:
            try:
                prob = self._create_problem(fp, plan)
            except MemoryError:
                if not plan.get('lead_axes') or self.kernel == 'lead':
                    raise
                import warnings
                warnings.warn('not enough device memory for the reduced-array sweep (2 extra arrays of the grid\'s '
                              'size): using the kernels that need none')
                self._cache['no_lead'] = True
                plan = self._kernel_plan(box_t, model)
                fp = ('problem', self._fingerprint(None), plan['box_digest'], codegen.source_key(plan['source']))
                prob = self._create_problem(fp, plan)
        if model.param_index is not None:
            prob.set_params(model.param_values())
            if prob.lists_of is not None and prob.lists_of != np.asarray(model.param_values(), dtype=float).tobytes():
                self._set_exchange_lists(prob, model, plan)
        self.backend_info = dict(prob.info, time_specialized=model.t_value is not None,
                                 lifted_constants=len(model.param_index or ()),
                                 box_mode=plan.get('box_mode') or 'node by node')
        return prob

    def _create_problem(self, fp, plan):
        nat.require_gpu()
        model, source, column, lanes = plan['model'], plan['source'], plan['column'], plan['lanes']
        per_node, lo, hi, n, max_u, W = (plan[k] for k in ('per_node', 'lo', 'hi', 'n', 'max_u', 'W'))
        shape = self._shape()
        S = int(np.prod(shape))
        dt = self.dtype
        layout = nat.LAYOUT_COLUMNS if column else nat.LAYOUT_NODES
        arrays = dict(
            axes=[np.ascontiguousarray(g, dtype=dt) for g in self.state_grid],
            box_lo=np.ascontiguousarray(lo, dtype=dt),
            box_hi=np.ascontiguousarray(hi, dtype=dt),
            box_n=np.ascontiguousarray(n, dtype=np.int32))
        if W:
            arrays['wgrid'] = np.ascontiguousarray(self.perturb_grid[0], dtype=dt)
            arrays['proba'] = np.ascontiguousarray(self.perturb_proba[0], dtype=dt)
        module = nat.compile_model(source)
        dev_shape = (shape[1:] + shape[:1]) if column else shape
        if self.comm is not None and self.comm.is_device:
            from .dist import phase_partition, slab_partition
            unit = shape[0] if column else 1
            bounds = phase_partition(S // unit, unit, self.comm.nranks, self.comm_phases,
                                     self.comm_taper)
            sparse = ((getattr(self, 'comm_sparse', False) or self.comm_exchange == 'sendrecv')
                      and self.comm_exchange in ('peer', 'direct', 'sendrecv')
                      and self.comm.nranks > 1 and column and not plan['per_control']
                      and not plan['window'] and model.storage_separable and self.sys.stationnary
                      and len(shape) >= 2)
            if sparse:
                dense_bounds = bounds
                bounds = slab_partition(S // unit, unit, self.comm.nranks, self.comm_phases)
            elif plan.get('lead_axes'):
                row = int(np.prod(shape[1:])) if shape[0] >= self.comm.nranks else 1
                bounds = slab_partition(S // row, row, self.comm.nranks, self.comm_phases)
            node_range = (0, S)
        elif self.comm is not None:
            bounds = self.comm.slab_bounds(dev_shape)
            node_range = (int(bounds[self.comm.rank]), int(bounds[self.comm.rank + 1]))
        else:
            bounds, node_range = None, (0, S)
        if self._idx_source is not None:
            self.last_policy_index
        old = [k for k in self._cache if k[0] == 'problem']
        if old and self.comm is not None and self.comm.is_device and self.comm.nranks > 1:
            for k in old:
                if self._cache[k].h:
                    nat.check(nat.lib().sdp_problem_attach_comm(self._cache[k].h, None, 0, None))
            self.comm.barrier()
        for k in old:
            self._cache.pop(k).close()
        prob = _DeviceProblem(arrays, module, dt, shape, len(self.sys.control), W, lanes,
                              per_node, node_range,
                              self.comm if (self.comm is not None and self.comm.is_device) else None,
                              bounds, layout, plan['staged'], plan['col_seg_nodes'])
        self._cache[fp] = prob
        if self._debug_after_create is not None:
            self._debug_after_create(prob)
        exchange = None
        if self.comm is not None and self.comm.is_device and self.comm.nranks > 1:
            exchange = 'rccl'
            if self.comm_exchange in ('peer', 'direct'):
                try:
                    nat.check(nat.lib().sdp_problem_enable_peer_exchange(prob.h))
                    exchange = 'peer'
                except RuntimeError as e:
                    if 'peer exchange not available' not in str(e):
                        raise
# ... 771 lines not shown
```

Before: 943.2.

## Add uniform-stock-axis branch and bound using precomputed block row offsets and padded table

When the stock axis is uniformly spaced and the control enters additively on x0, the planner pads the reduced LDS table with linearly extrapolated rows on both sides. It also precomputes, per control block, an integer row offset and a fractional phase shared by all lanes. The branch-and-bound lower bounds then become direct LDS loads at fixed offsets, with no per-block index computation or clamping. This adds LDS space and a check that the planner only enables the path when occupancy does not change, and it adds setup work per column.

```diff
diff --git a/__graft_entry__.py b/__graft_entry__.py
--- a/__graft_entry__.py
+++ b/__graft_entry__.py
@@ -93,6 +93,8 @@
                 sources.append(device_ops.unit_source(device_ops.unit_solver(unit, dtkey)))
         for seed in device_ops.WIDE_SEEDS:
             sources.append(device_ops.wide_model(seed)[0]._kernel_plan()['source'])
+        import test_gpu_uniform_bound
+        sources += test_gpu_uniform_bound.units()
     finally:
         sys.path.remove(os.path.join(ROOT, 'tests'))
         sys.dont_write_bytecode = dont_write
diff --git a/stodynprog_amd/codegen.py b/stodynprog_amd/codegen.py
--- a/stodynprog_amd/codegen.py
+++ b/stodynprog_amd/codegen.py
@@ -18,7 +18,7 @@
     'SDP_STAMP', 'SDP_NO_POW2', 'SDP_EXTRA_DEFINES', 'SDP_COL_FILTER_SCALE', 'SDP_LEAD_FILTER_SCALE',
     'SDP_LEAD_UNROLL', 'SDP_COL_A_LW', 'SDP_COL_FILTER', 'SDP_COL_SHIFT', 'SDP_COL_UTAB', 'SDP_LEAD_FILTER',
     'SDP_COL_THREADS', 'SDP_COL_WCHUNK', 'SDP_STG_CU', 'SDP_COL_WPAIR', 'SDP_COL_WRES', 'SDP_COL_LEAN2', 'SDP_COL_BNB',
-    'SDP_LINE_FILTER', 'SDP_LINE_FILTER_SCALE', 'SDP_LINE_TOP2'))
+    'SDP_LINE_FILTER', 'SDP_LINE_FILTER_SCALE', 'SDP_LINE_TOP2', 'SDP_BNB_UNIFORM'))
 
 
 def check_debug(debug):
@@ -392,7 +392,86 @@
     return lines
 
 
-def _column_lines(model, dtype, column, col_cfg, window, per_control, filtered, utab, debug, wres=0):
+def uniform_rows_axis(axis, dtype, n0=None):
+    from fractions import Fraction
+    if np.dtype(dtype).itemsize != 8:
+        return False
+    x = np.asarray(axis, dtype=np.float64).ravel()
+    n = x.size
+    if n < 2 or (n0 is not None and n != int(n0)) or not np.all(np.isfinite(x)):
+        return False
+    span = x[-1] - x[0]
+    if not (span > 0):
+        return False
+    k = Fraction(float(np.float64(n - 1) / span))
+    smin, tol, u2 = Fraction(float(x[0])), Fraction(1, 2 ** 23), Fraction(1, 2 ** 51)
+    for r in range(n):
+        p = (Fraction(float(x[r])) - smin) * k
+        if abs(p - r) + u2 * (abs(p) + 1) > tol:
+            return False
+    return True
+
+
+def uniform_stage_model(model, frontier):
+    sp = model.additive_control_split(frontier) if frontier is not None else None
+    if sp is None:
+        return False
+    x_node, _, a_form = sp['lead']
+    return bool(a_form in ('add', 'sub') and x_node is not None and x_node.op == 'var' and x_node.value == 'x0')
+
+
+uniform_define = ('\n#define SDP_BNB_UNIFORM 1      // node r of a column sits at row r of the stock axis: the block ends of the '
+                  'branch and bound at the same offsets in every lane')
+
+
+def uniform_stage_reach(model, frontier, lattice, k_rows):
+    from . import trace
+    a_node = frontier[int(model.additive_control_split(frontier)['lead'][1])]
+    mesh = np.meshgrid(*[np.asarray(v, dtype=float) for v in lattice], indexing='ij')
+    env = {}
+    with np.errstate(all='ignore'):
+        for n in model.slice_nodes([a_node]):
+            if n.op == 'var':
+                if not (isinstance(n.value, str) and n.value[0] == 'u'):
+                    return None
+                env[n.id] = mesh[int(n.value[1:])]
+            elif n.op == 'const':
+                env[n.id] = np.float64(n.value)
+            elif n.op == 'bconst':
+                env[n.id] = np.bool_(n.value)
+            elif n.op == 'interp1':
+                xp, fp, left, right = model.graph.tables[n.value][:4]
+                env[n.id] = np.interp(env[n.args[0].id], xp, fp, left, right)
+            else:
+                env[n.id] = trace._NP_EVAL[n.op](*[env[a.id] for a in n.args])
+    a = np.abs(np.asarray(env[a_node.id], dtype=float))
+    if not np.all(np.isfinite(a)):
+        return None
+    return float(a.max()) * abs(float(k_rows))
+
+
+def uniform_stage_pad(model, dtype, frontier, axis, n0, lattice, wres, shift, threads, lds, debug=None):
+    rs = np.dtype(dtype).itemsize
+    n0 = int(n0)
+    if not wres or shift or rs != 8 or frontier is None or model.cost_depends_on_w:
+        return 0
+    if _dbg(debug, 'SDP_COL_LEAN2') == '0' or _dbg(debug, 'SDP_COL_BNB') == '0':
+        return 0
+    if n0 < 2 or (n0 - 1) % 64 == 0 or not uniform_stage_model(model, frontier):
+        return 0
+    if not uniform_rows_axis(axis, dtype, n0):
+        return 0
+    x = np.asarray(axis, dtype=np.float64).ravel()
+    reach = uniform_stage_reach(model, frontier, lattice, np.float64(n0 - 1) / (x[-1] - x[0]))
+    if reach is None or not reach * (1.0 + 2.0 ** -30) + 2.0 ** -19 <= BNB_PAD - 3:
+        return 0
+    per_cu = lambda size: min(COLUMN_LDS_MAX // size, max(1, 2048 // int(threads)))
+    if per_cu(int(lds) + 2 * BNB_PAD * rs) != per_cu(int(lds)):
+        return 0
+    return BNB_PAD
+
+
+def _column_lines(model, dtype, column, col_cfg, window, per_control, filtered, utab, debug, wres=0, bnb_pad=0):
     rs = np.dtype(dtype).itemsize
     wpair = use_wpair(model, dtype, debug) and window is None
     shifted = bool(filtered and column_shift_applies(model, dtype, debug=debug))
@@ -463,6 +542,12 @@
                 if short and _dbg(debug, 'SDP_COL_BNB') != '0':
                     short += ('\n#define SDP_COL_BNB 1          // the short first pass as a certified branch and bound over '
                               'blocks of controls (sdp_lean2_bnb)')
+                    if bnb_pad:
+                        short += '\n#define SDP_BNB_PAD_ROWS {}    // the reduced table continued linearly on either side'.format(
+                            int(bnb_pad))
+                        if _dbg(debug, 'SDP_BNB_UNIFORM') != '0':
+                            short += uniform_define
+                        bnb_pad = 0
 
             elif rs == 4 and not wres and _dbg(debug, 'SDP_COL_FILTER_TOP2') in (None, '1'):
                 short = short_pass_source(model, utab[0], 'SDP_COL_WIDE2')
@@ -473,6 +558,8 @@
                         short += '\n#define SDP_BNB_CHUNK 4        // blocks whose bounds are evaluated together (see SDP_COL_A_GROUP above)'
         if short:
             lines += [short, '']
+    if bnb_pad:
+        raise ValueError('a padded reduced table was planned for a unit without the branch and bound of the short first pass')
     lines += ['#include "sdp_column_kernel.h"    // also brings in sdp_sweep_kernel.h', '']
     return lines
 
@@ -523,7 +610,7 @@
 
 def translation_unit(model, dtype, lanes, column=None, staged=None, window=None,
                      per_control=None, filtered=False, utab=None, lead_axes=0, col_cfg=None, debug=None, wres=0,
-                     lead_perm=None, line=0, peer_stores=False):
+                     lead_perm=None, line=0, peer_stores=False, bnb_pad=0):
     debug = check_debug(debug)
     real = {'float64': 'double', 'float32': 'float'}[np.dtype(dtype).name]
     head = _prologue_lines(model, real, lanes, debug, peer_stores)
@@ -544,7 +631,7 @@
         if col_cfg is None:
             raise ValueError('the column kernel does not fit this grid (its table exceeds the LDS of a CU)')
         head += _column_lines(model, dtype, column, col_cfg, window, per_control, filtered, utab, debug,
-                              wres if (window is None and per_control is None) else 0)
+                              wres if (window is None and per_control is None) else 0, bnb_pad=bnb_pad)
     elif staged is not None:
         tile = tuple(staged['tile']) + (1,) * (4 - len(staged['tile']))
         head += ['#define SDP_STG_THREADS {}'.format(int(staged['threads']))] + [
@@ -790,6 +877,11 @@
     return (best[0], best[1]) if best[2] >= 0.85 else (0, 0)
 
 
+BNB_PAD = 16
+
+
+
+
 def bnb_words(n_controls):
     n = max(int(n_controls), 1)
     block = 8
@@ -803,7 +895,7 @@
 
 
 def _column_lds(tw, w, rows, n_state, rs, threads, reduced=False, shift=False, shift_rows=0, utab_values=0,
-                partial_minima=False):
+                partial_minima=False, bnb_pad=False):
     dt = n_state - 1
     part = threads if partial_minima else 1
     members = [(rs, tw * rows, 16),
@@ -815,7 +907,7 @@
                (rs, 2 * (int(utab_values) + 4 if utab_values else 2), 16)]
     if reduced or shift:
         per_row = 4 if rs == 4 else (2 if shift else 1)
-        members.append((rs, per_row * int(shift_rows if shift else rows), 16))
+        members.append((rs, per_row * int(shift_rows if shift else rows) + (2 * BNB_PAD if bnb_pad and not shift else 0), 16))
     if shift:
         members += [(4, 2 * w, 4), (rs, 2 * w, rs), (rs, 2 * w, rs), (4, 8, 4)]
     off = 0
diff --git a/stodynprog_amd/csrc/sdp_colfilter_kernel.h b/stodynprog_amd/csrc/sdp_colfilter_kernel.h
--- a/stodynprog_amd/csrc/sdp_colfilter_kernel.h
+++ b/stodynprog_amd/csrc/sdp_colfilter_kernel.h
@@ -381,6 +381,9 @@
     const int lane_u = tid - first;
     bool bnb_fine = count == 64 && SDP_BNB_BLOCK <= 64;
     sdp_real bnb_prev_hi = -INFINITY, bnb_prev_lo = (sdp_real)NAN, bnb_between = (sdp_real)0, bnb_amax = (sdp_real)0;
+#if SDP_BNB_UNIFORM_ON
+    asm volatile("" : "+v"(bnb_prev_hi));
+#endif
     for (int c0 = 0; c0 < n_tab; c0 += 64) {
         int ci = c0 + lane_u;
         asm volatile("" : "+v"(ci));
@@ -437,7 +440,13 @@
                 hp = sdp_vmin(hp, __shfl_xor(hp, d, 64));
             }
         }
+#if SDP_BNB_UNIFORM_ON
+        const int next_at = (lane_u + SEG) << 2;
+        const sdp_real next_lo = (sdp_real)__hiloint2double(__builtin_amdgcn_ds_bpermute(next_at, __double2hiint((double)lo)),
+                                                            __builtin_amdgcn_ds_bpermute(next_at, __double2loint((double)lo)));
+#else
         const sdp_real next_lo = __shfl_down(lo, SEG, 64);
+#endif
         const bool has_next = lane_u + SEG < 64 && ci + SEG < n_tab;
         if (head) {
             const int b = ci / SDP_BNB_BLOCK;
@@ -466,6 +475,17 @@
         const bool sorted = __all(bnb_fine);
         bnb_between = sdp_wave_max(bnb_between);
         bnb_amax = sdp_wave_max(bnb_amax);
+        bool uni_fine = true;
+#if SDP_BNB_UNIFORM_ON
+        float uni_k = 0.0f;
+        for (int b = lane_u; b <= (n_tab + SDP_BNB_BLOCK - 1) / SDP_BNB_BLOCK; b += 64) {
+            const sdp_real st = rec[2 * b], kf = floor(st);
+            SDP_BNB_UNI_K(rec)[b] = (int)((unsigned)(int)kf << 3);
+            SDP_BNB_UNI_PHI(rec)[b] = st - kf;
+            uni_k = fmaxf(uni_k, fabsf((float)kf));
+        }
+        uni_fine = sorted && sdp_wave_max(uni_k) + 2.0f <= (float)SDP_BNB_PAD;
+#endif
         if (lane_u == 0) {
             const int n_blocks = (n_tab + SDP_BNB_BLOCK - 1) / SDP_BNB_BLOCK;
             const int extra = (bnb_between == bnb_between && bnb_between < (sdp_real)SDP_COL_N0)
@@ -474,7 +494,7 @@
             else rec[2 * n_blocks + 1] = (sdp_real)__hiloint2double(0, extra);
             sdp_real *st = utab + SDP_COL_UTAB * SDP_COL_UTAB_N;
             const sdp_real cap = x_cap - bnb_amax;
-            st[3] = (sorted && cap == cap && extra < SDP_COL_N0) ? cap : (sdp_real)-1;
+            st[3] = (sorted && uni_fine && cap == cap && extra < SDP_COL_N0) ? cap : (sdp_real)-1;
         }
     }
 #else
@@ -753,9 +773,9 @@
 template <int AXIS, bool WIDE, typename INSERT>
 SDP_DEV void sdp_short_bnb(const sdp_real *A, const sdp_real *utab, const SdpColFilter &f, const SdpLeadAxis &l,
                            sdp_real X, sdp_real k_rows, int c_lo, int n, int mask, double slack, int guess, INSERT &insert,
-                           sdp_real &sdp_diag_cnt, sdp_real *b_seen = nullptr)
-{
-    (void)sdp_diag_cnt; (void)c_lo; (void)b_seen;
+                           sdp_real &sdp_diag_cnt, sdp_real *b_seen = nullptr, int row_u = -1)
+{
+    (void)sdp_diag_cnt; (void)c_lo; (void)b_seen; (void)row_u;
     constexpr bool SHIFT = SDP_COL_SHIFT != 0;
     static_assert(!(SHIFT && WIDE), "branch and bound on the shifted lattice: 8-byte reals");
     constexpr double BSCALE = (double)(SDP_COL_FILTER_SCALE);
@@ -780,6 +800,7 @@
     const int g = guess < 0 ? (n >> 1) : min(guess, n - 1);
     const sdp_real ga = utab[g * SDP_COL_UTAB + SDP_LEAN2_A_SLOT];
     const sdp_real gh = SDP_LEAN2_H_SLOT < 0 ? (sdp_real)0 : utab[g * SDP_COL_UTAB + HS];
+    (void)k_rows;
     const sdp_real pX = (SDP_LEAN2_FORM == 2 ? -((X + l.smin) * k_rows) : (X - l.smin) * k_rows) - (SHIFT ? l.koff : (sdp_real)0);
     const int extra = __builtin_amdgcn_readfirstlane(WIDE ? __float_as_int((float)rec[4 * n_blocks + 1]) : __double2loint((double)rec[2 * n_blocks + 1]));
     int gq;
@@ -789,6 +810,49 @@
     unsigned long long need = 0ull;
     double thresh = 0.0;
     constexpr int CB = NB < SDP_BNB_CHUNK ? NB : SDP_BNB_CHUNK;
+#if SDP_BNB_UNIFORM_ON
+    {
+        const char *Ar = (const char *)(A + row_u);
+        auto at = [&](int off) -> double { return (double)*(const sdp_real *)(Ar + off); };
+        for (int b0 = 0; b0 < n_blocks; b0 += CB) {
+            int ko[CB + 1];
+            double P[CB + 1], hp[CB], Aq[CB + 1], Aq1[CB + 1], m[CB];
+#pragma unroll
+            for (int j = 0; j <= CB; ++j) {
+                const int b = min(b0 + j, n_blocks);
+                ko[j] = SDP_BNB_UNI_K(rec)[b];
+                P[j] = (double)SDP_BNB_UNI_PHI(rec)[b];
+                if (j < CB) hp[j] = least(min(b, n_blocks - 1));
+            }
+#pragma unroll
+            for (int j = 0; j <= CB; ++j) {
+                Aq[j] = at(ko[j]);
+                Aq1[j] = at(ko[j] + 8);
+            }
+            if (b0 == 0) {
+                const double h = fma((double)glam, gA1 - gA0, gA0);
+                const double Fg = pack(SDP_LEAN2_H_SLOT < 0 ? h : fma((double)(SDP_LEAN2_HNEG ? -gh : gh), psum, h), g);
+                thresh = Fg + slack;
+            }
+#pragma unroll
+            for (int j = 0; j <= CB; ++j) P[j] = fma(P[j], Aq1[j] - Aq[j], Aq[j]);
+#pragma unroll
+            for (int j = 0; j < CB; ++j) m[j] = sdp_vmin(sdp_vmin(P[j], P[j + 1]), sdp_vmin(Aq1[j], Aq[j + 1]));
+            for (int k = 0; k < extra; ++k) {
+                double more[CB];
+#pragma unroll
+                for (int j = 0; j < CB; ++j) more[j] = at(min(ko[j] + 16 + 8 * k, ko[j + 1] - 8));
+#pragma unroll
+                for (int j = 0; j < CB; ++j) m[j] = sdp_vmin(m[j], more[j]);
+            }
+#pragma unroll
+            for (int j = 0; j < CB; ++j) {
+                const double lbv = hp[j] + m[j];
+                if ((!(lbv > thresh) || b0 + j == g / BS) && b0 + j < n_blocks) need |= 1ull << (b0 + j);
+            }
+        }
+    }
+#else
     for (int b0 = 0; b0 < n_blocks; b0 += CB) {
         int q[CB + 1];
         double P[CB + 1], hp[CB], Aq[CB + 1], Aq1[CB + 1], m[CB], Bq[SHIFT ? CB + 1 : 1], bm[SHIFT ? CB : 1];
@@ -843,6 +907,7 @@
             if ((!(lbv > thresh) || b0 + j == g / BS) && b0 + j < n_blocks) need |= 1ull << (b0 + j);
         }
     }
+#endif
 #ifdef SDP_DIAG_BNB_COUNT
     sdp_diag_cnt = (sdp_real)(__popcll(need) + 100 * (g / BS));
 #endif
diff --git a/stodynprog_amd/csrc/sdp_colres_kernel.h b/stodynprog_amd/csrc/sdp_colres_kernel.h
--- a/stodynprog_amd/csrc/sdp_colres_kernel.h
+++ b/stodynprog_amd/csrc/sdp_colres_kernel.h
@@ -250,6 +250,7 @@
 
 #endif
 
+#define SDP_LDS_AD (sdp_lds.ad + SDP_BNB_PAD)
 extern "C" __global__ void __launch_bounds__(SDP_COL_THREADS, SDP_COL_MIN_WAVES) sdp_sweep_col(SdpSweepArgs a)
 {
     __shared__ SdpColLds sdp_lds;
@@ -388,6 +389,9 @@
 #else
         {
             sdp_real dmax = (sdp_real)0;
+#if SDP_BNB_UNIFORM_ON
+            sdp_real acc_row = (sdp_real)0;
+#endif
             if (r < N0) {
                 sdp_real acc = (sdp_real)0;
 #pragma unroll SDP_COL_FILTER_RUNROLL
@@ -398,8 +402,28 @@
                 }
                 acc = acc + acc_t;
                 dmax = acc == acc ? filt.pcap * big + filt.floor : (sdp_real)INFINITY;
-                sdp_lds.ad[r] = acc;
-            }
+                SDP_LDS_AD[r] = acc;
+#if SDP_BNB_UNIFORM_ON
+                acc_row = acc;
+#endif
+            }
+#if SDP_BNB_UNIFORM_ON
+            int pt = (int)threadIdx.x;
+            asm volatile("" : "+v"(pt));
+            const int pl = pt & 63, pw = __builtin_amdgcn_readfirstlane(pt >> 6);
+            auto row_of = [&](int l) -> sdp_real {
+                return (sdp_real)__hiloint2double(__builtin_amdgcn_readlane(__double2hiint((double)acc_row), l),
+                                                  __builtin_amdgcn_readlane(__double2loint((double)acc_row), l));
+            };
+            if (pw == 0) {
+                const sdp_real a0 = row_of(0), a1 = row_of(1);
+                if (pl < SDP_BNB_PAD) SDP_LDS_AD[-(pl + 1)] = fma(-(sdp_real)(pl + 1), a1 - a0, a0);
+            }
+            if (pw == ((N0 - 1) >> 6)) {
+                const sdp_real a0 = row_of((N0 - 1) & 63), a1 = row_of((N0 - 2) & 63);
+                if (pl < SDP_BNB_PAD) SDP_LDS_AD[N0 + pl] = fma((sdp_real)(pl + 1), a0 - a1, a0);
+            }
+#endif
             dmax = sdp_wave_max(dmax);
             if (lane == 0) atomicMax(&sdp_lds.dcol[parity], (unsigned long long)__double_as_longlong((double)dmax));
         }
@@ -482,15 +506,15 @@
                     bd.f2 = sdp_vmin(bd.f2, sdp_vmax(bd.f1, Fq));
                     bd.f1 = sdp_vmin(bd.f1, Fq);
                 };
-                if (axis_mode == 2) sdp_short_bnb<2, false>(sdp_lds.ad, utab, filt, lead1, X, k_rows, 0, box.total, mask, slack, guess, ins, diag_cnt, &b_max);
-                else if (axis_mode == 1) sdp_short_bnb<1, false>(sdp_lds.ad, utab, filt, lead1, X, k_rows, 0, box.total, mask, slack, guess, ins, diag_cnt, &b_max);
-                else sdp_short_bnb<0, false>(sdp_lds.ad, utab, filt, lead1, X, k_rows, 0, box.total, mask, slack, guess, ins, diag_cnt, &b_max);
+                if (axis_mode == 2) sdp_short_bnb<2, false>(SDP_LDS_AD, utab, filt, lead1, X, k_rows, 0, box.total, mask, slack, guess, ins, diag_cnt, &b_max);
+                else if (axis_mode == 1) sdp_short_bnb<1, false>(SDP_LDS_AD, utab, filt, lead1, X, k_rows, 0, box.total, mask, slack, guess, ins, diag_cnt, &b_max);
+                else sdp_short_bnb<0, false>(SDP_LDS_AD, utab, filt, lead1, X, k_rows, 0, box.total, mask, slack, guess, ins, diag_cnt, &b_max);
             } else
 #endif
             {
-                if (axis_mode == 2) sdp_lean2s_pass1<2>(sdp_lds.ad, utab, filt, lead1, X, box.total, mask, bd.f1, bd.f2, bd.f3, b_max);
-                else if (axis_mode == 1) sdp_lean2s_pass1<1>(sdp_lds.ad, utab, filt, lead1, X, box.total, mask, bd.f1, bd.f2, bd.f3, b_max);
-                else sdp_lean2s_pass1<0>(sdp_lds.ad, utab, filt, lead1, X, box.total, mask, bd.f1, bd.f2, bd.f3, b_max);
+                if (axis_mode == 2) sdp_lean2s_pass1<2>(SDP_LDS_AD, utab, filt, lead1, X, box.total, mask, bd.f1, bd.f2, bd.f3, b_max);
+                else if (axis_mode == 1) sdp_lean2s_pass1<1>(SDP_LDS_AD, utab, filt, lead1, X, box.total, mask, bd.f1, bd.f2, bd.f3, b_max);
+                else sdp_lean2s_pass1<0>(SDP_LDS_AD, utab, filt, lead1, X, box.total, mask, bd.f1, bd.f2, bd.f3, b_max);
             }
             const sdp_real radius = fma((sdp_real)(SDP_COL_FILTER_SCALE), b_max, radius0);
             bd.i1 = bd.f1 < (sdp_real)INFINITY ? (__double2loint(bd.f1) & mask) : INT_MAX;
@@ -522,22 +546,27 @@
                              bits > 24 || box.total > SDP_COL_UTAB_N;
             const sdp_real radius = (filt.cu + (sdp_real)(SDP_COL_FILTER_SCALE) * ldexp(SDP_COL_FILTER_EPS, bits + 1)) * s_node;
 #if SDP_COL_BNB
-            const sdp_real slack = fma((sdp_real)2, radius, ((sdp_real)8 * SDP_COL_FILTER_EPS) * s_node);
+            const sdp_real slack = fma((sdp_real)2, radius, ((sdp_real)(SDP_BNB_UNIFORM_ON ? 12 : 8) * SDP_COL_FILTER_EPS) * s_node);
+#if SDP_BNB_UNIFORM_ON
+            const bool bnb = fabs(X) < ust[3] && fabs((X - lead.smin) * k_rows - (sdp_real)i) <= (sdp_real)0x1p-22;
+#else
             const bool bnb = fabs(X) < ust[3];
+#endif
+            const int row_u = i;
             if (__all(bnb)) {
                 auto ins = [&](double Fq) {
                     bd.f2 = sdp_vmin(bd.f2, sdp_vmax(bd.f1, Fq));
                     bd.f1 = sdp_vmin(bd.f1, Fq);
                 };
-                if (axis_mode == 2) sdp_short_bnb<2, false>(sdp_lds.ad, utab, filt, lead, X, k_rows, 0, box.total, mask, slack, guess, ins, diag_cnt);
-                else if (axis_mode == 1) sdp_short_bnb<1, false>(sdp_lds.ad, utab, filt, lead, X, k_rows, 0, box.total, mask, slack, guess, ins, diag_cnt);
-                else sdp_short_bnb<0, false>(sdp_lds.ad, utab, filt, lead, X, k_rows, 0, box.total, mask, slack, guess, ins, diag_cnt);
+                if (axis_mode == 2) sdp_short_bnb<2, false>(SDP_LDS_AD, utab, filt, lead, X, k_rows, 0, box.total, mask, slack, guess, ins, diag_cnt, nullptr, row_u);
+                else if (axis_mode == 1) sdp_short_bnb<1, false>(SDP_LDS_AD, utab, filt, lead, X, k_rows, 0, box.total, mask, slack, guess, ins, diag_cnt, nullptr, row_u);
+                else sdp_short_bnb<0, false>(SDP_LDS_AD, utab, filt, lead, X, k_rows, 0, box.total, mask, slack, guess, ins, diag_cnt, nullptr, row_u);
             } else
 #endif
             {
-                if (axis_mode == 2) sdp_lean2_pass1<2>(sdp_lds.ad, utab, filt, lead, X, box.total, mask, bd.f1, bd.f2);
-                else if (axis_mode == 1) sdp_lean2_pass1<1>(sdp_lds.ad, utab, filt, lead, X, box.total, mask, bd.f1, bd.f2);
-                else sdp_lean2_pass1<0>(sdp_lds.ad, utab, filt, lead, X, box.total, mask, bd.f1, bd.f2);
+                if (axis_mode == 2) sdp_lean2_pass1<2>(SDP_LDS_AD, utab, filt, lead, X, box.total, mask, bd.f1, bd.f2);
+                else if (axis_mode == 1) sdp_lean2_pass1<1>(SDP_LDS_AD, utab, filt, lead, X, box.total, mask, bd.f1, bd.f2);
+                else sdp_lean2_pass1<0>(SDP_LDS_AD, utab, filt, lead, X, box.total, mask, bd.f1, bd.f2);
             }
             bd.i1 = bd.f1 < (sdp_real)INFINITY ? (__double2loint(bd.f1) & mask) : INT_MAX;
 #else
@@ -548,13 +577,13 @@
             const sdp_real *utab = sdp_lds.utab[upar];
             const bool plain = SDP_NU == 1 && box.n[0] > 1 && box.step[0] != (sdp_real)0;
             if (plain) {
-                if (axis_mode == 2) sdp_col_filter_pass1<true, 2>(sdp_lds.ad, utab, filt, lead1, box, x, t, 0, box.total, bd);
-                else if (axis_mode == 1) sdp_col_filter_pass1<true, 1>(sdp_lds.ad, utab, filt, lead1, box, x, t, 0, box.total, bd);
-                else sdp_col_filter_pass1<true, 0>(sdp_lds.ad, utab, filt, lead1, box, x, t, 0, box.total, bd);
+                if (axis_mode == 2) sdp_col_filter_pass1<true, 2>(SDP_LDS_AD, utab, filt, lead1, box, x, t, 0, box.total, bd);
+                else if (axis_mode == 1) sdp_col_filter_pass1<true, 1>(SDP_LDS_AD, utab, filt, lead1, box, x, t, 0, box.total, bd);
+                else sdp_col_filter_pass1<true, 0>(SDP_LDS_AD, utab, filt, lead1, box, x, t, 0, box.total, bd);
             } else {
-                if (axis_mode == 2) sdp_col_filter_pass1<false, 2>(sdp_lds.ad, utab, filt, lead1, box, x, t, 0, box.total, bd);
-                else if (axis_mode == 1) sdp_col_filter_pass1<false, 1>(sdp_lds.ad, utab, filt, lead1, box, x, t, 0, box.total, bd);
-                else sdp_col_filter_pass1<false, 0>(sdp_lds.ad, utab, filt, lead1, box, x, t, 0, box.total, bd);
+                if (axis_mode == 2) sdp_col_filter_pass1<false, 2>(SDP_LDS_AD, utab, filt, lead1, box, x, t, 0, box.total, bd);
+                else if (axis_mode == 1) sdp_col_filter_pass1<false, 1>(SDP_LDS_AD, utab, filt, lead1, box, x, t, 0, box.total, bd);
+                else sdp_col_filter_pass1<false, 0>(SDP_LDS_AD, utab, filt, lead1, box, x, t, 0, box.total, bd);
             }
 #if SDP_COL_SHIFT
             const sdp_real h_cap = (((sdp_real)1 + (sdp_real)2 * (bd.p_max + shc.lc)) * ((sdp_real)3 + shc.es)) * dcol;
@@ -596,15 +625,15 @@
                     if (!cand) {
 #if SDP_COL_LEAN2 && SDP_COL_SHIFT
                         sdp_real b_unused = (sdp_real)0;
-                        const sdp_real F = lead.pow2 ? sdp_lean2s_value<1>(sdp_lds.ad, utab, filt, lead1, X, ci, b_unused)
-                                                     : sdp_lean2s_value<0>(sdp_lds.ad, utab, filt, lead1, X, ci, b_unused);
+                        const sdp_real F = lead.pow2 ? sdp_lean2s_value<1>(SDP_LDS_AD, utab, filt, lead1, X, ci, b_unused)
+                                                     : sdp_lean2s_value<0>(SDP_LDS_AD, utab, filt, lead1, X, ci, b_unused);
 #elif SDP_COL_LEAN2
-                        const sdp_real F = lead.pow2 ? sdp_lean2_value<1>(sdp_lds.ad, utab, filt, lead, X, ci)
-                                                     : sdp_lean2_value<0>(sdp_lds.ad, utab, filt, lead, X, ci);
+                        const sdp_real F = lead.pow2 ? sdp_lean2_value<1>(SDP_LDS_AD, utab, filt, lead, X, ci)
+                                                     : sdp_lean2_value<0>(SDP_LDS_AD, utab, filt, lead, X, ci);
 #else
                         sdp_real F, pm = (sdp_real)0, gm = (sdp_real)0, bm = (sdp_real)0;
-                        if (lead.pow2) sdp_col_lean_eval<1>(sdp_lds.ad, filt, lead1, x, u, t, F, pm, gm, bm);
-                        else sdp_col_lean_eval<0>(sdp_lds.ad, filt, lead1, x, u, t, F, pm, gm, bm);
+                        if (lead.pow2) sdp_col_lean_eval<1>(SDP_LDS_AD, filt, lead1, x, u, t, F, pm, gm, bm);
+                        else sdp_col_lean_eval<0>(SDP_LDS_AD, filt, lead1, x, u, t, F, pm, gm, bm);
 #endif
                         cand = !(F - radius > m_hi);
                     }
diff --git a/stodynprog_amd/csrc/sdp_column_kernel.h b/stodynprog_amd/csrc/sdp_column_kernel.h
--- a/stodynprog_amd/csrc/sdp_column_kernel.h
+++ b/stodynprog_amd/csrc/sdp_column_kernel.h
@@ -105,6 +105,20 @@
 #define SDP_COL_SHORT (SDP_COL_LEAN2 || SDP_COL_WIDE2)
 #ifndef SDP_COL_BNB
 #define SDP_COL_BNB 0
+#endif
+#ifndef SDP_BNB_UNIFORM
+#define SDP_BNB_UNIFORM 0
+#endif
+#define SDP_BNB_UNI_K(rec) ((int *)((rec) + 2 * (SDP_BNB_BLOCKS + 1)))
+#define SDP_BNB_UNI_PHI(rec) ((rec) + 2 * (SDP_BNB_BLOCKS + 1) + (SDP_BNB_BLOCKS + 2) / 2)
+#ifndef SDP_BNB_PAD_ROWS
+#define SDP_BNB_PAD_ROWS 0
+#endif
+#if SDP_BNB_UNIFORM && SDP_BNB_PAD_ROWS > 0 && SDP_COL_LEAN2 && SDP_COL_BNB && !SDP_COL_SHIFT && SDP_LEAN2_FORM != 2 && \
+    SDP_COL_WRES < SDP_COL_W && SDP_COL_N0 >= 2 && (SDP_COL_N0 - 1) % 64 != 0
+#define SDP_BNB_UNIFORM_ON 1
+#else
+#define SDP_BNB_UNIFORM_ON 0
 #endif
 #ifndef SDP_LEAN2_A_FIXED
 #define SDP_LEAN2_A_FIXED 0
@@ -159,6 +173,7 @@
 #define SDP_AD_A(ad, r) (SDP_COL_WIDE2 ? ((double *)(ad))[(r)] : *(double *)((ad) + 4 * (r)))
 #define SDP_AD_A_CONST(ad, r) (SDP_COL_WIDE2 ? ((const double *)(ad))[(r)] : *(const double *)((ad) + 4 * (r)))
 constexpr int SDP_COL_LDS_AD = sizeof(SDP_REAL) == 4 ? 4 : (!SDP_COL_SHIFT ? 1 : 2);
+constexpr int SDP_BNB_PAD = (SDP_COL_FILTER && !SDP_COL_SHIFT) ? SDP_BNB_PAD_ROWS : 0;
 struct __attribute__((aligned(16))) SdpColLds {
     sdp_real T[(SDP_TRAIL_HAS_U ? SDP_COL_WCHUNK : (SDP_COL_WRES < SDP_COL_W ? SDP_COL_WRES : SDP_COL_TW)) * SDP_COL_ROWS];
     sdp_real w_lam[SDP_COL_W * SDP_DT];
@@ -172,7 +187,7 @@
     unsigned long long dcol[2];
     sdp_real utab[2][SDP_COL_UTAB ? SDP_COL_UTAB * SDP_COL_UTAB_N + 4 + SDP_BNB_WORDS : 2] __attribute__((aligned(16)));
 #if SDP_COL_FILTER
-    sdp_real ad[SDP_COL_LDS_AD * (SDP_COL_SHIFT ? SDP_COL_SHIFT_ROWS : SDP_COL_ROWS)] __attribute__((aligned(16)));
+    sdp_real ad[SDP_COL_LDS_AD * (SDP_COL_SHIFT ? SDP_COL_SHIFT_ROWS : SDP_COL_ROWS) + 2 * SDP_BNB_PAD] __attribute__((aligned(16)));
 #endif
 #if SDP_COL_SHIFT
     int sh_q[2][SDP_COL_W];
diff --git a/stodynprog_amd/solver.py b/stodynprog_amd/solver.py
--- a/stodynprog_amd/solver.py
+++ b/stodynprog_amd/solver.py
@@ -572,7 +572,7 @@
         may_filter = (getattr(self, 'certified_filter', True)
                       and codegen.column_filter_applies(model, dtype=dt, table=(shape[0], W, len(shape)), debug=debug))
         n_controls = bp['max_u'] if box_t is None else 1 << max(int(bp['max_u']) - 1, 0).bit_length()
-        col_cfg, utab, wres = None, None, 0
+        col_cfg, utab, wres, bnb_pad = None, None, 0, 0
         if self.kernel in ('auto', 'column') and model.storage_separable:
             wpair = codegen.use_wpair(model, dt, debug)
             shift = bool(may_filter and codegen.column_shift_applies(model, dt, debug=debug))
@@ -587,6 +587,13 @@
                                                           col_cfg[0], kw['utab_values'], debug)
                     if wres:
                         col_cfg = codegen.column_config(shape[0], W, len(shape), dt, wpair, may_filter, wres=wres, **kw)
+                        if col_cfg is not None and not bp['per_node']:
+                            lattice = [np.linspace(float(bp['lo'][c, 0]), float(bp['hi'][c, 0]), int(bp['n'][c, 0]))
+                                       for c in range(bp['lo'].shape[0])]
+                            bnb_pad = codegen.uniform_stage_pad(model, dt, frontier, self.state_grid[0], shape[0], lattice,
+                                                                wres, shift, col_cfg[0], col_cfg[1], debug)
+                            if bnb_pad:
+                                col_cfg = (col_cfg[0], col_cfg[1] + 2 * bnb_pad * np.dtype(dt).itemsize) + tuple(col_cfg[2:])
                     break
         column = col_cfg is not None
         lead_axes = 0
@@ -670,7 +677,8 @@
                                           window=window, per_control=per_control_cfg if per_control else None,
                                           filtered=filtered, utab=utab, lead_axes=lead_axes,
                                           col_cfg=col_cfg, debug=debug, wres=wres if filtered else 0,
-                                          lead_perm=lead_perm, line=line, peer_stores=self._plans_direct_exchange())
+                                          lead_perm=lead_perm, line=line, peer_stores=self._plans_direct_exchange(),
+                                          bnb_pad=bnb_pad if (filtered and wres and utab is not None) else 0)
         filtered = filtered or bool(lead_axes) or bool(line)
         return dict(model=model, source=source, column=column, lanes=lanes, staged=staged, filtered=filtered,
                     lead_axes=lead_axes, lead_perm=lead_perm, line=bool(line),
```

Result: faster. 982.1 (median of 6 runs) (+4.1%).
